# jyf588/SimGAN

Hardware: AMD Instinct MI355X
Metric: env-steps/sec of GAIL-dyn PPO update (higher is better)
Workload: dtype f32; 1 GPU; northstar: GAIL-dyn update, T=128 N=512/GPU obs=47 act=12 D-in=86 policy=mlp h64 D h100 ppo_epoch=10 num_mini_batch=1...; optimizer_steps_per_update=2720, parallelism=single GPU

## Files before the change

### include/simgan_hip.h

```cpp
#ifndef SIMGAN_HIP_H
#define SIMGAN_HIP_H

#include <stdint.h>

#define SG_API __attribute__((visibility("default")))

#ifdef __cplusplus
extern "C" {
#endif

typedef struct sg_ctx sg_ctx;
typedef struct sg_policy sg_policy;
typedef struct sg_rollout sg_rollout;
typedef struct sg_ppo sg_ppo;
typedef struct sg_disc sg_disc;

SG_API const char *sg_last_error(void);
SG_API const char *sg_version(void);
SG_API int sg_ctx_create(int device, sg_ctx **out);
SG_API int sg_ctx_destroy(sg_ctx *ctx);
SG_API int sg_ctx_synchronize(sg_ctx *ctx);
SG_API int sg_ctx_device_info(sg_ctx *ctx, char *name, int name_len, int *num_cu, int64_t *hbm_bytes);

SG_API int sg_comm_unique_id(uint8_t id[128]);
SG_API int sg_comm_loopback_id(uint8_t id[128]);
SG_API int sg_ctx_comm_init(sg_ctx *ctx, const uint8_t id[128], int rank, int world);
SG_API int sg_ctx_comm_kind(sg_ctx *ctx, int *kind);
SG_API int sg_ctx_comm_set_peer(sg_ctx *ctx, int enable);
SG_API int sg_ctx_comm_info(sg_ctx *ctx, int *rank, int *world);
SG_API int sg_ctx_set_disc_dp(sg_ctx *ctx, int sharded);

enum { SG_POLICY_MLP = 0, SG_POLICY_SPLIT = 1, SG_POLICY_GRU = 2 };
SG_API int sg_policy_create(sg_ctx *ctx, int kind, int obs_dim, int act_dim, int hidden, int num_feet,
                     sg_policy **out);
SG_API int sg_policy_create2(sg_ctx *ctx, int kind, int obs_dim, int act_dim, int hidden, int num_feet, int critic_hidden,
                             sg_policy **out);
SG_API int sg_policy_destroy(sg_policy *p);
SG_API int sg_policy_num_params(const sg_policy *p, int64_t *n);
SG_API int sg_policy_set_params(sg_policy *p, const float *flat, int64_t n);
SG_API int sg_policy_get_params(sg_policy *p, float *flat, int64_t n);
SG_API int sg_policy_act(sg_policy *p, const float *obs, int n, const float *noise, uint64_t seed,
                  int deterministic, float *value, float *action, float *logp);
SG_API int sg_policy_get_value(sg_policy *p, const float *obs, int n, float *value);
SG_API int sg_policy_evaluate(sg_policy *p, const float *obs, const float *action, int n, float *value,
                       float *logp, float *entropy);
SG_API int sg_policy_act_rnn(sg_policy *p, const float *obs, const float *hxs, const float *masks, int n, const float *noise,
                      uint64_t seed, int deterministic, float *value, float *action, float *logp, float *hxs_out);
SG_API int sg_policy_get_value_rnn(sg_policy *p, const float *obs, const float *hxs, const float *masks, int n, float *value);
SG_API int sg_policy_evaluate_rnn(sg_policy *p, const float *obs, const float *hxs, const float *masks, const float *action,
                           int T, int n, float *value, float *logp, float *entropy, float *hxs_out);
#define SG_ENSEMBLE_MAX 8
SG_API int sg_policy_act_ensemble(sg_policy *const *policies, int n_policies, const int32_t *idx, const float *obs,
                           int n, const float *noise, uint64_t seed, int deterministic, float *value,
                           float *action, float *logp);

enum {
    SG_F_OBS = 0,
    SG_F_OBS_FEAT = 1,
    SG_F_ACTIONS = 2,
    SG_F_REWARDS = 3,
    SG_F_VALUE_PREDS = 4,
    SG_F_RETURNS = 5,
    SG_F_LOGP = 6,
    SG_F_MASKS = 7,
    SG_F_BAD_MASKS = 8,
    SG_F_ADVANTAGES = 9,
    SG_F_COUNT = 10
};
SG_API int sg_rollout_create(sg_ctx *ctx, int T, int N, int obs_dim, int act_dim, int feat_dim,
                      sg_rollout **out);
SG_API int sg_rollout_destroy(sg_rollout *r);
SG_API int sg_rollout_upload(sg_rollout *r, int field, const float *host, int64_t count);
SG_API int sg_rollout_download(sg_rollout *r, int field, float *host, int64_t count);
SG_API int sg_rollout_upload_step(sg_rollout *r, int field, int t, const float *host, int64_t count);
SG_API int sg_rollout_download_step(sg_rollout *r, int field, int t, float *host, int64_t count);
SG_API int sg_rollout_after_update(sg_rollout *r);
SG_API int sg_rollout_compute_returns(sg_rollout *r, const float *next_value, int use_gae, float gamma,
                               float gae_lambda, int use_proper_time_limits);
SG_API int sg_rollout_compute_returns_policy(sg_rollout *r, sg_policy *p, int use_gae, float gamma,
                                      float gae_lambda, int use_proper_time_limits);
SG_API int sg_rollout_fill_synthetic(sg_rollout *r, sg_policy *p, uint64_t seed, float p_done);

typedef struct {
    float clip_param;
    int ppo_epoch;
    int num_mini_batch;
    float value_loss_coef;
    float entropy_coef;
    float lr;
    float eps;
    float max_grad_norm;
    int use_clipped_value_loss;
} sg_ppo_config;
SG_API int sg_ppo_create(sg_ctx *ctx, sg_policy *p, const sg_ppo_config *cfg, sg_ppo **out);
SG_API int sg_ppo_destroy(sg_ppo *a);
SG_API int sg_ppo_set_lr(sg_ppo *a, float lr);
SG_API int sg_ppo_update(sg_ppo *a, sg_rollout *r, const int64_t *perms, int64_t n_perms, uint64_t seed, float out3[3]);
SG_API int sg_results_publish(sg_ctx *ctx, sg_disc *d, sg_ppo *a, int slot);
SG_API int sg_results_fetch(sg_ctx *ctx, int slot, double out13[13]);
SG_API int sg_ppo_last_perms(sg_ppo *a, int64_t *perms, int64_t count);
SG_API int sg_ppo_get_adam(sg_ppo *a, float *m, float *v, int64_t n, int64_t *step);
SG_API int sg_ppo_set_adam(sg_ppo *a, const float *m, const float *v, int64_t n, int64_t step);
SG_API int sg_ppo_set_hidden_states(sg_ppo *a, const float *hxs0, int64_t count);
SG_API int sg_ppo_set_symmetry(sg_ppo *a, float coef, const float *m_obs, const float *m_act);
SG_API int sg_ppo_set_mirrored_obs(sg_ppo *a, const float *host, int64_t count);
SG_API int sg_ppo_last_symmetry_loss(sg_ppo *a, float *out);

typedef struct {
    float value_loss_coef;
    float entropy_coef;
    float lr;
    float eps;
    float alpha;
    float max_grad_norm;
} sg_a2c_config;
SG_API int sg_a2c_create(sg_ctx *ctx, sg_policy *p, const sg_a2c_config *cfg, sg_ppo **out);
SG_API int sg_a2c_get_rmsprop(sg_ppo *a, float *square_avg, int64_t n, int64_t *step);
SG_API int sg_a2c_set_rmsprop(sg_ppo *a, const float *square_avg, int64_t n, int64_t step);

typedef struct {
    float value_loss_coef;
    float entropy_coef;
    float lr;
    float momentum;
    float stat_decay;
    float kl_clip;
    float damping;
    int Tf;
} sg_acktr_config;
SG_API int sg_acktr_create(sg_ctx *ctx, sg_policy *p, const sg_acktr_config *cfg, sg_ppo **out);
SG_API int sg_acktr_set_value_noise(sg_ppo *a, const float *eps, int64_t n);
SG_API int sg_acktr_get_state(sg_ppo *a, float *m_aa, int64_t n_aa, float *m_gg, int64_t n_gg, float *momentum_buf, int64_t n,
                              int64_t *steps);

SG_API int sg_disc_create(sg_ctx *ctx, int input_dim, int hidden_dim, sg_disc **out);
SG_API int sg_disc_destroy(sg_disc *d);
SG_API int sg_disc_num_params(const sg_disc *d, int64_t *n);
SG_API int sg_disc_set_params(sg_disc *d, const float *flat, int64_t n);
SG_API int sg_disc_get_params(sg_disc *d, float *flat, int64_t n);
SG_API int sg_disc_get_adam(sg_disc *d, float *m, float *v, int64_t n, int64_t *step);
SG_API int sg_disc_set_adam(sg_disc *d, const float *m, const float *v, int64_t n, int64_t step);
SG_API int sg_disc_set_expert(sg_disc *d, const float *expert, int64_t n_rows);
SG_API int sg_disc_update_gail_dyn(sg_disc *d, sg_rollout *r, int batch_size, const int64_t *expert_perm, int64_t n_expert_perm,
                            const int64_t *policy_perm, int64_t n_policy_perm, const float *alpha, int64_t n_alpha,
                            uint64_t seed, float out3[3], int *n_steps);
SG_API int sg_disc_update_rows(sg_disc *d, const float *policy_rows, int64_t n_rows, int n_cols, int batch_size,
                        const int64_t *expert_perm, int64_t n_expert_perm, const int64_t *policy_perm, int64_t n_policy_perm,
                        const float *alpha, int64_t n_alpha, uint64_t seed, float out3[3], int *n_steps);
SG_API int sg_disc_predict_reward(sg_disc *d, const float *x, int n, float gamma, const float *masks,
                           float offset, float *reward, float *returns);
SG_API int sg_disc_predict_reward_steps(sg_disc *d, sg_rollout *r, float gamma, float offset, float *reward, float *returns);
SG_API int sg_disc_predict_prob(sg_disc *d, const float *x, int n, float *prob);
SG_API int sg_disc_grad_pen(sg_disc *d, const float *expert_rows, const float *policy_rows, const float *alpha, int n,
                     uint64_t seed, float *pen);
SG_API int sg_disc_last_draws(sg_disc *d, int64_t *expert_perm, int64_t *policy_perm, float *alpha, int64_t counts3[3]);
SG_API int sg_disc_reset_returns(sg_disc *d);
SG_API int sg_disc_get_returns(sg_disc *d, float *returns, int n, int *is_none);
SG_API int sg_disc_set_returns(sg_disc *d, const float *returns, int n);
SG_API int sg_disc_relabel_rewards(sg_disc *d, sg_rollout *r, float gamma, float offset,
                            double rms_state[3]);
SG_API int sg_disc_relabel_rewards_auto(sg_disc *d, sg_rollout *r, float gamma, double gail_tar_length, int no_alive_bonus);
SG_API int sg_disc_set_rms(sg_disc *d, const double rms_state[3]);
SG_API int sg_disc_get_scalars(sg_disc *d, double out5[5]);
SG_API int sg_rollout_count_dones(sg_rollout *r, double *dones);

SG_API int sg_host_alloc(int64_t bytes, void **out);
SG_API int sg_host_free(void *p);

SG_API int sg_ctx_profile(sg_ctx *ctx, int enable);
SG_API int sg_ctx_profile_read(sg_ctx *ctx, int which, double *total_ms, int64_t *launches);
SG_API int sg_ctx_profile_reset(sg_ctx *ctx);
SG_API int sg_ctx_mark(sg_ctx *ctx, int *id);
SG_API int sg_ctx_mark_elapsed(sg_ctx *ctx, int from, int to, double *ms);

#ifdef __cplusplus
}
#endif
#endif
```

### simgan_amd/_lib.py

```python
import ctypes as C
import os

import numpy as np

_HERE = os.path.dirname(os.path.abspath(__file__))
LIB_PATH = os.path.join(_HERE, "libsimgan_hip.so")

c_float_p = C.POINTER(C.c_float)
c_i64_p = C.POINTER(C.c_int64)
c_double_p = C.POINTER(C.c_double)
c_u8_p = C.POINTER(C.c_uint8)
c_int_p = C.POINTER(C.c_int)
H = C.c_void_p

F_OBS, F_OBS_FEAT, F_ACTIONS, F_REWARDS, F_VALUE_PREDS, F_RETURNS, F_LOGP, F_MASKS, F_BAD_MASKS, \
    F_ADVANTAGES = range(10)
POLICY_MLP, POLICY_SPLIT, POLICY_GRU = 0, 1, 2
PROF_DISC_CHAIN, PROF_DISC_WGRAD, PROF_PPO_FWD, PROF_PPO_BWD, PROF_PPO_REDUCE, PROF_RELABEL, PROF_PPO_ADAM = range(7)


class PPOConfig(C.Structure):
    _fields_ = [("clip_param", C.c_float), ("ppo_epoch", C.c_int), ("num_mini_batch", C.c_int),
                ("value_loss_coef", C.c_float), ("entropy_coef", C.c_float), ("lr", C.c_float),
                ("eps", C.c_float), ("max_grad_norm", C.c_float),
                ("use_clipped_value_loss", C.c_int)]


class A2CConfig(C.Structure):
    _fields_ = [("value_loss_coef", C.c_float), ("entropy_coef", C.c_float), ("lr", C.c_float), ("eps", C.c_float),
                ("alpha", C.c_float), ("max_grad_norm", C.c_float)]


class ACKTRConfig(C.Structure):
    _fields_ = [("value_loss_coef", C.c_float), ("entropy_coef", C.c_float), ("lr", C.c_float), ("momentum", C.c_float),
                ("stat_decay", C.c_float), ("kl_clip", C.c_float), ("damping", C.c_float), ("Tf", C.c_int)]


PROTOTYPES = {
    "sg_last_error": (C.c_char_p, []),
    "sg_version": (C.c_char_p, []),
    "sg_ctx_create": (C.c_int, [C.c_int, C.POINTER(H)]),
    "sg_ctx_destroy": (C.c_int, [H]),
    "sg_ctx_synchronize": (C.c_int, [H]),
    "sg_ctx_device_info": (C.c_int, [H, C.c_char_p, C.c_int, c_int_p, c_i64_p]),
    "sg_comm_unique_id": (C.c_int, [c_u8_p]),
    "sg_comm_loopback_id": (C.c_int, [c_u8_p]),
    "sg_ctx_comm_init": (C.c_int, [H, c_u8_p, C.c_int, C.c_int]),
    "sg_ctx_comm_kind": (C.c_int, [H, c_int_p]),
    "sg_ctx_comm_set_peer": (C.c_int, [H, C.c_int]),
    "sg_ctx_comm_info": (C.c_int, [H, c_int_p, c_int_p]),
    "sg_ctx_set_disc_dp": (C.c_int, [H, C.c_int]),
    "sg_policy_create": (C.c_int, [H, C.c_int, C.c_int, C.c_int, C.c_int, C.c_int, C.POINTER(H)]),
    "sg_policy_create2": (C.c_int, [H, C.c_int, C.c_int, C.c_int, C.c_int, C.c_int, C.c_int, C.POINTER(H)]),
    "sg_policy_destroy": (C.c_int, [H]),
    "sg_policy_num_params": (C.c_int, [H, c_i64_p]),
    "sg_policy_set_params": (C.c_int, [H, c_float_p, C.c_int64]),
    "sg_policy_get_params": (C.c_int, [H, c_float_p, C.c_int64]),
    "sg_policy_act": (C.c_int, [H, c_float_p, C.c_int, c_float_p, C.c_uint64, C.c_int, c_float_p, c_float_p, c_float_p]),
    "sg_policy_get_value": (C.c_int, [H, c_float_p, C.c_int, c_float_p]),
    "sg_policy_evaluate": (C.c_int, [H, c_float_p, c_float_p, C.c_int, c_float_p, c_float_p, c_float_p]),
    "sg_policy_act_rnn": (C.c_int, [H, c_float_p, c_float_p, c_float_p, C.c_int, c_float_p, C.c_uint64, C.c_int, c_float_p, c_float_p,
                                    c_float_p, c_float_p]),
    "sg_policy_get_value_rnn": (C.c_int, [H, c_float_p, c_float_p, c_float_p, C.c_int, c_float_p]),
    "sg_policy_evaluate_rnn": (C.c_int, [H, c_float_p, c_float_p, c_float_p, c_float_p, C.c_int, C.c_int, c_float_p, c_float_p,
                                         c_float_p, c_float_p]),
    "sg_policy_act_ensemble": (C.c_int, [C.POINTER(H), C.c_int, C.POINTER(C.c_int32), c_float_p, C.c_int, c_float_p, C.c_uint64,
                                         C.c_int, c_float_p, c_float_p, c_float_p]),
    "sg_rollout_create": (C.c_int, [H, C.c_int, C.c_int, C.c_int, C.c_int, C.c_int, C.POINTER(H)]),
    "sg_rollout_destroy": (C.c_int, [H]),
    "sg_rollout_upload": (C.c_int, [H, C.c_int, c_float_p, C.c_int64]),
    "sg_rollout_download": (C.c_int, [H, C.c_int, c_float_p, C.c_int64]),
    "sg_rollout_upload_step": (C.c_int, [H, C.c_int, C.c_int, c_float_p, C.c_int64]),
    "sg_rollout_download_step": (C.c_int, [H, C.c_int, C.c_int, c_float_p, C.c_int64]),
    "sg_rollout_after_update": (C.c_int, [H]),
    "sg_rollout_compute_returns": (C.c_int, [H, c_float_p, C.c_int, C.c_float, C.c_float, C.c_int]),
    "sg_rollout_compute_returns_policy": (C.c_int, [H, H, C.c_int, C.c_float, C.c_float, C.c_int]),
    "sg_rollout_fill_synthetic": (C.c_int, [H, H, C.c_uint64, C.c_float]),
    "sg_rollout_count_dones": (C.c_int, [H, c_double_p]),
    "sg_ppo_create": (C.c_int, [H, H, C.POINTER(PPOConfig), C.POINTER(H)]),
    "sg_ppo_destroy": (C.c_int, [H]),
    "sg_ppo_set_lr": (C.c_int, [H, C.c_float]),
    "sg_ppo_update": (C.c_int, [H, H, c_i64_p, C.c_int64, C.c_uint64, c_float_p]),
    "sg_ppo_last_perms": (C.c_int, [H, c_i64_p, C.c_int64]),
    "sg_ppo_set_hidden_states": (C.c_int, [H, c_float_p, C.c_int64]),
    "sg_ppo_get_adam": (C.c_int, [H, c_float_p, c_float_p, C.c_int64, c_i64_p]),
    "sg_ppo_set_adam": (C.c_int, [H, c_float_p, c_float_p, C.c_int64, C.c_int64]),
    "sg_ppo_set_symmetry": (C.c_int, [H, C.c_float, c_float_p, c_float_p]),
    "sg_ppo_set_mirrored_obs": (C.c_int, [H, c_float_p, C.c_int64]),
    "sg_ppo_last_symmetry_loss": (C.c_int, [H, c_float_p]),
    "sg_a2c_create": (C.c_int, [H, H, C.POINTER(A2CConfig), C.POINTER(H)]),
    "sg_a2c_get_rmsprop": (C.c_int, [H, c_float_p, C.c_int64, c_i64_p]),
    "sg_a2c_set_rmsprop": (C.c_int, [H, c_float_p, C.c_int64, C.c_int64]),
    "sg_acktr_create": (C.c_int, [H, H, C.POINTER(ACKTRConfig), C.POINTER(H)]),
    "sg_acktr_set_value_noise": (C.c_int, [H, c_float_p, C.c_int64]),
    "sg_acktr_get_state": (C.c_int, [H, c_float_p, C.c_int64, c_float_p, C.c_int64, c_float_p, C.c_int64, c_i64_p]),
    "sg_disc_create": (C.c_int, [H, C.c_int, C.c_int, C.POINTER(H)]),
    "sg_disc_destroy": (C.c_int, [H]),
    "sg_disc_num_params": (C.c_int, [H, c_i64_p]),
    "sg_disc_set_params": (C.c_int, [H, c_float_p, C.c_int64]),
    "sg_disc_get_params": (C.c_int, [H, c_float_p, C.c_int64]),
    "sg_disc_get_adam": (C.c_int, [H, c_float_p, c_float_p, C.c_int64, c_i64_p]),
    "sg_disc_set_adam": (C.c_int, [H, c_float_p, c_float_p, C.c_int64, C.c_int64]),
    "sg_disc_set_expert": (C.c_int, [H, c_float_p, C.c_int64]),
    "sg_disc_update_gail_dyn": (C.c_int, [H, H, C.c_int, c_i64_p, C.c_int64, c_i64_p, C.c_int64, c_float_p, C.c_int64, C.c_uint64,
                                          c_float_p, c_int_p]),
    "sg_disc_update_rows": (C.c_int, [H, c_float_p, C.c_int64, C.c_int, C.c_int, c_i64_p, C.c_int64, c_i64_p, C.c_int64, c_float_p,
                                      C.c_int64, C.c_uint64, c_float_p, c_int_p]),
    "sg_disc_predict_reward": (C.c_int, [H, c_float_p, C.c_int, C.c_float, c_float_p, C.c_float, c_float_p, c_float_p]),
    "sg_disc_predict_prob": (C.c_int, [H, c_float_p, C.c_int, c_float_p]),
    "sg_disc_predict_reward_steps": (C.c_int, [H, H, C.c_float, C.c_float, c_float_p, c_float_p]),
    "sg_disc_grad_pen": (C.c_int, [H, c_float_p, c_float_p, c_float_p, C.c_int, C.c_uint64, c_float_p]),
    "sg_disc_last_draws": (C.c_int, [H, c_i64_p, c_i64_p, c_float_p, c_i64_p]),
    "sg_disc_reset_returns": (C.c_int, [H]),
    "sg_disc_get_returns": (C.c_int, [H, c_float_p, C.c_int, c_int_p]),
    "sg_disc_set_returns": (C.c_int, [H, c_float_p, C.c_int]),
    "sg_disc_relabel_rewards": (C.c_int, [H, H, C.c_float, C.c_float, c_double_p]),
    "sg_disc_relabel_rewards_auto": (C.c_int, [H, H, C.c_float, C.c_double, C.c_int]),
    "sg_disc_set_rms": (C.c_int, [H, c_double_p]),
    "sg_disc_get_scalars": (C.c_int, [H, c_double_p]),
    "sg_results_publish": (C.c_int, [H, H, H, C.c_int]),
    "sg_results_fetch": (C.c_int, [H, C.c_int, c_double_p]),
    "sg_ctx_profile": (C.c_int, [H, C.c_int]),
    "sg_ctx_profile_read": (C.c_int, [H, C.c_int, c_double_p, c_i64_p]),
    "sg_ctx_profile_reset": (C.c_int, [H]),
    "sg_host_alloc": (C.c_int, [C.c_int64, C.POINTER(C.c_void_p)]),
    "sg_host_free": (C.c_int, [C.c_void_p]),
    "sg_ctx_mark": (C.c_int, [H, c_int_p]),
    "sg_ctx_mark_elapsed": (C.c_int, [H, C.c_int, C.c_int, c_double_p]),
}

TEST_LIB_PATH = os.path.join(_HERE, "libsimgan_hip_test.so")
c_ll_p = C.POINTER(C.c_longlong)
TEST_PROTOTYPES = {
    "sg_test_last_error": (C.c_char_p, []),
    "sg_test_gemm": (C.c_int, [H, C.c_int, C.c_int, C.c_int, C.c_int, c_float_p, c_float_p, c_float_p]),
    "sg_test_gemm_bench": (C.c_int, [H, C.c_int, C.c_int, C.c_int, C.c_int, C.c_int, C.c_int, C.c_int, c_ll_p]),
    "sg_test_mfma_probe": (C.c_int, [H, C.c_int, c_float_p, c_float_p, c_float_p]),
    "sg_test_flag_probe": (C.c_int, [H, C.c_int, C.c_int, C.c_int, C.c_int, c_ll_p, c_float_p]),
    "sg_test_fetch_probe": (C.c_int, [H, C.c_int, C.c_int, C.c_int, c_ll_p]),
    "sg_test_pmc_calibrate": (C.c_int, [H, C.c_int64]),
    "sg_test_pstep_probe": (C.c_int, [H, C.c_int, C.c_int, C.c_int, C.c_int, C.c_int, c_ll_p, c_int_p]),
    "sg_test_graph_state": (C.c_int, [H, H, c_int_p]),
    "sg_test_disc_phase_times": (C.c_int, [H, C.c_int, c_ll_p, C.c_int]),
    "sg_test_disc_step4_times": (C.c_int, [H, C.c_int, c_ll_p, C.c_int]),
    "sg_test_disc_gathers": (C.c_int, [H, c_ll_p]),
    "sg_test_ppo_phase_times": (C.c_int, [H, C.c_int, c_ll_p, C.c_int]),
    "sg_test_rng": (C.c_int, [H, C.c_int, C.c_int64, C.c_uint64, C.c_void_p]),
    "sg_test_kfac_eig": (C.c_int, [H, C.c_int, c_float_p, c_float_p, c_float_p, C.POINTER(C.c_int)]),
    "sg_test_acktr_noise": (C.c_int, [H, C.c_int64, C.c_uint64, C.c_int64, c_float_p]),
    "sg_test_raise_kfac_error": (C.c_int, [H]),
    "sg_test_tear_probe": (C.c_int, [H, C.c_int, C.c_int, C.c_int, c_ll_p]),
    "sg_test_raise_handoff_error": (C.c_int, [H, H]),
}
_TEST_LIB = None

_LIB = None


class SimganHipError(RuntimeError):
    pass


def load():
    global _LIB
    if _LIB is not None:
        return _LIB
    if not os.path.exists(LIB_PATH):
        raise SimganHipError(
            f"{LIB_PATH} not found: the HIP extension is not built. There is no CPU fallback; "
            "run `make -C simgan_amd/csrc` (hipcc, gfx950).")
    lib = C.CDLL(LIB_PATH)
    for name, (res, args) in PROTOTYPES.items():
        fn = getattr(lib, name)
        fn.restype = res
        fn.argtypes = args
    _LIB = lib
    return lib


def check(rc):
    if rc != 0:
        raise SimganHipError(load().sg_last_error().decode(errors="replace"))


def load_test():
    global _TEST_LIB
    if _TEST_LIB is not None:
        return _TEST_LIB
    load()
    if not os.path.exists(TEST_LIB_PATH):
        raise SimganHipError(f"{TEST_LIB_PATH} not found: run `make -C simgan_amd/csrc`")
    lib = C.CDLL(TEST_LIB_PATH)
    for name, (res, args) in TEST_PROTOTYPES.items():
        fn = getattr(lib, name)
        fn.restype = res
        fn.argtypes = args
    _TEST_LIB = lib
    return lib


def check_test(rc):
    if rc != 0:
        raise SimganHipError(load_test().sg_test_last_error().decode(errors="replace"))


def fptr(a):
    assert isinstance(a, np.ndarray) and a.dtype == np.float32 and a.flags["C_CONTIGUOUS"], (type(a), getattr(a, "dtype", None))
    return a.ctypes.data_as(c_float_p)


def i64ptr(a):
    assert isinstance(a, np.ndarray) and a.dtype == np.int64 and a.flags["C_CONTIGUOUS"]
    return a.ctypes.data_as(c_i64_p)


def as_f32(x):
    if hasattr(x, "detach"):
        x = x.detach().cpu().numpy()
    return np.ascontiguousarray(x, dtype=np.float32)


def as_i64(x):
    if hasattr(x, "detach"):
        x = x.detach().cpu().numpy()
    return np.ascontiguousarray(x, dtype=np.int64)


class _PinnedBlock(object):

    def __init__(self, nbytes):
        self.lib = load()
        p = C.c_void_p()
        check(self.lib.sg_host_alloc(int(nbytes), C.byref(p)))
        self.ptr = p.value

    def __del__(self):
        try:
            if self.ptr:
                self.lib.sg_host_free(C.c_void_p(self.ptr))
                self.ptr = None
        except Exception:
            pass


_PINNED_WARNED = False


def pinned_array(shape, fill=0.0):
    n = int(np.prod(shape)) * 4
    if n == 0:
        return np.full(shape, fill, np.float32)
    try:
        blk = _PinnedBlock(n)
    except SimganHipError as exc:
        global _PINNED_WARNED
        if not _PINNED_WARNED:
            _PINNED_WARNED = True
            import warnings
            warnings.warn(f"simgan_amd: page-locked host allocation of {n} bytes failed ({exc}); the rollout's host tensors fall back to "
                          "pageable memory (uploads are staged and slower)", RuntimeWarning, stacklevel=3)
        return np.full(shape, fill, np.float32)
    buf = (C.c_char * n).from_address(blk.ptr)
    buf._owner = blk
    a = np.frombuffer(buf, dtype=np.float32).reshape(shape)
    a[...] = fill
    return a


_CTX = {}


class Context:

    def __init__(self, device=0):
        self.lib = load()
        h = H()
        check(self.lib.sg_ctx_create(int(device), C.byref(h)))
        self.h = h
        self.device = int(device)
        self.rank, self.world = 0, 1
        self.disc_sharded = False

    @staticmethod
    def default():
        dev = int(os.environ.get("LOCAL_RANK", "0"))
        if dev not in _CTX:
            try:
                _CTX[dev] = Context(dev)
            except SimganHipError as exc:
                if dev == 0 or "out of range (1 visible)" not in str(exc):
                    raise
                _CTX[dev] = Context(0)
        return _CTX[dev]

    def make_default(self):
        _CTX[int(os.environ.get("LOCAL_RANK", "0"))] = self
        return self

    def synchronize(self):
# ... 74 lines not shown
```

### simgan_amd/csrc/sg_common.h

```cpp
#pragma once
#include <hip/hip_runtime.h>
#include <stdint.h>

#include <string>
#include <atomic>
#include <vector>
#include <mutex>
inline std::recursive_mutex& sg_capture_mutex() { static std::recursive_mutex m; return m; }
struct SgDeviceWideGuard {
    std::lock_guard<std::recursive_mutex> l{sg_capture_mutex()};
    ~SgDeviceWideGuard() { (void)hipGetLastError(); }
};
#define SG_DEVICE_WIDE() SgDeviceWideGuard _sg_device_wide_guard
static inline hipError_t sg_dev_malloc(void** p, size_t n) { std::lock_guard<std::recursive_mutex> l(sg_capture_mutex()); return hipMalloc(p, n); }
static inline hipError_t sg_dev_free(void* p) { std::lock_guard<std::recursive_mutex> l(sg_capture_mutex()); return hipFree(p); }
static inline hipError_t sg_host_malloc(void** p, size_t n) { std::lock_guard<std::recursive_mutex> l(sg_capture_mutex()); return hipHostMalloc(p, n, hipHostMallocDefault); }
static inline hipError_t sg_host_release(void* p) { std::lock_guard<std::recursive_mutex> l(sg_capture_mutex()); return hipHostFree(p); }

#include "../../include/simgan_hip.h"
#include "sg_gemm.hpp"

void sg_set_error(const char* fmt, ...);

#define SG_CHECK(expr)                                                                      \
// ... 45 lines not shown
    int total;
    int nc, na;
};

struct SgDiscDesc {
    int F, Hd, Fp, ldF, Hp, ldH;
    int w1, b1, w2, b2, w3, b3;
    int total;
};

SgPolicyDesc sg_make_policy_desc(int kind, int O, int A, int H, int num_feet, int Hc = 0);
int64_t sg_policy_flat_count(const SgPolicyDesc& d);
void sg_policy_pad(const SgPolicyDesc& d, const float* flat, float* padded);
void sg_policy_unpad(const SgPolicyDesc& d, const float* padded, float* flat);
struct sg_ctx;
bool sg_policy_needs_gw(const sg_ctx* ctx, const SgPolicyDesc& d);
SgDiscDesc sg_make_disc_desc(int F, int Hd);
int64_t sg_disc_flat_count(const SgDiscDesc& d);
void sg_disc_pad(const SgDiscDesc& d, const float* flat, float* padded);
void sg_disc_unpad(const SgDiscDesc& d, const float* padded, float* flat);

enum { SG_PROF_DISC_CHAIN = 0, SG_PROF_DISC_WGRAD, SG_PROF_PPO_FWD, SG_PROF_PPO_BWD,
       SG_PROF_PPO_REDUCE, SG_PROF_RELABEL, SG_PROF_PPO_ADAM, SG_PROF_DISC_STEP, SG_PROF_COMM_F32, SG_PROF_COUNT };

struct SgProfSlot {
    double total_ms = 0.0;
    int64_t launches = 0;
    std::vector<std::pair<hipEvent_t, hipEvent_t>> pending;
};

struct SgComm;

struct sg_ctx {
    int device = 0;
    hipStream_t stream = nullptr;
    int num_cu = 0;
    int lds_bytes = 0;
    bool profile = false;
    SgProfSlot prof[SG_PROF_COUNT];
    std::vector<hipEvent_t> event_pool;
    std::vector<hipEvent_t> marks;
    SgComm* comm = nullptr;
    int rank = 0, world = 1;
    bool disc_sharded = false;
    bool use_comm = false;
    std::atomic<int> n_learners{0};
    float* d_scratch = nullptr;
    size_t scratch_bytes = 0;
    void* h_pinned = nullptr;
    size_t pinned_bytes = 0;
    double* mailbox = nullptr;
    double* results = nullptr;
    hipEvent_t res_ev[8] = {nullptr};
    struct sg_disc* res_d[8] = {nullptr};
    struct sg_ppo* res_a[8] = {nullptr};
};
#define SG_RESULT_SLOTS 8

bool sg_ctx_exclusive(const sg_ctx* ctx);
void sg_ctx_learner_born(sg_ctx* ctx);
void sg_ctx_learner_gone(sg_ctx* ctx);
int sg_ctx_scratch(sg_ctx* ctx, size_t bytes, float** out);
int sg_ctx_pinned(sg_ctx* ctx, size_t bytes, void** out);
int sg_ctx_fetch_f64(sg_ctx* ctx, const double* dev, double* host, int n);
int sg_ctx_put_f64(sg_ctx* ctx, double* dev, const double* host, int n);
struct SgEv { hipEvent_t a = nullptr, b = nullptr; };
SgEv sg_prof_events(sg_ctx* ctx, int which);
#ifdef __HIPCC__
#include <hip/hip_ext.h>
#define SG_LAUNCH(ctx, which, kernel, grid, block, lds, ...)                                                  \
    do {                                                                                                      \
        if ((ctx)->profile) {                                                                                 \
            SgEv _ev = sg_prof_events(ctx, which);                                                            \
            hipExtLaunchKernelGGL(kernel, grid, block, lds, (ctx)->stream, _ev.a, _ev.b, 0, __VA_ARGS__);     \
        } else {                                                                                              \
            hipLaunchKernelGGL(kernel, grid, block, lds, (ctx)->stream, __VA_ARGS__);                         \
        }                                                                                                     \
    } while (0)
#endif

struct SgGruDesc {
    int O, H, Op, ldO, Hp, ldH;
    int off;
    int wih, whh, bih, bhh;
    int total;
};
SgGruDesc sg_make_gru_desc(int O, int H, int off);
int64_t sg_gru_flat_count(const SgGruDesc& g);
void sg_gru_pad(const SgGruDesc& g, const float* flat, float* padded);
void sg_gru_unpad(const SgGruDesc& g, const float* padded, float* flat);

struct sg_policy {
    sg_ctx* ctx;
    SgPolicyDesc desc;
    bool recurrent = false;
    SgGruDesc gru;
    float* d_params = nullptr;
    float* d_io = nullptr;
    size_t io_bytes = 0;
};

size_t sg_policy_padded_count(const sg_policy* p);
bool sg_gru_fits(const sg_ctx* ctx, const SgGruDesc& g);

#define SG_STEP4_FLAG_WORD0 64
#define SG_STEP4_MAX_FLAGS 1024
#ifndef SG_STEP4_FLAG_STRIDE
#define SG_STEP4_FLAG_STRIDE 32
#endif
#define SG_STEP4_ERR_WORD (SG_STEP4_FLAG_WORD0 + SG_STEP4_MAX_FLAGS * SG_STEP4_FLAG_STRIDE)
#define SG_STEP4_STATE_BYTES (4 * (SG_STEP4_ERR_WORD + 16))
#define SG_PAIR_ERR_WORD 0
unsigned* sg_comm_peer_err_word(struct sg_ctx* ctx);
bool sg_comm_peer_on(const struct sg_ctx* ctx);
uint32_t sg_comm_peer_generation(const struct sg_ctx* ctx);
unsigned* sg_disc_err_word(struct sg_disc* d);
uint64_t sg_next_feat_version();
struct sg_rollout {
    sg_ctx* ctx;
    int T, N, O, A, F;
    float* d_field[SG_F_COUNT] = {nullptr};
    int64_t field_count[SG_F_COUNT] = {0};
    int field_slots[SG_F_COUNT] = {0};
    int field_width[SG_F_COUNT] = {0};
    int64_t* d_perm = nullptr;
    uint64_t feat_version = sg_next_feat_version();
};

#define SG_H0_SLOTS 8
struct sg_ppo {
    int64_t opt_t = 0;
    uint64_t scratch_key = 0;
    hipGraphExec_t steps_graph = nullptr;
    bool graph_refused = false;
    uint64_t steps_graph_key[18] = {0};
    sg_ctx* ctx;
    sg_policy* policy;
    sg_ppo_config cfg;
    float *d_m = nullptr, *d_v = nullptr, *d_grad = nullptr;
    float* d_slabs = nullptr;
    size_t slabs_cap = 0;
    float* d_stacks = nullptr;
    size_t stacks_cap = 0;
    float* d_state = nullptr;
    int64_t* d_perms = nullptr;
    int64_t perms_cap = 0;
    int64_t last_perm_count = 0;
    double* d_loss_acc = nullptr;
    float* d_part = nullptr;
    long long* d_dbg = nullptr;
    unsigned* d_pair = nullptr;
    bool self_wait_failed = false;
    bool pair_primed = false;
    float sym_coef = 0.f;
    float* d_mobs_mat = nullptr;
    float* d_mact = nullptr;
    float* d_mrows = nullptr;
    int64_t mrows_cap = 0;
    int64_t mrows_host = 0;
    float* d_h0 = nullptr;
    int64_t h0_cap = 0, h0_count = 0;
    float* h_h0 = nullptr;
    hipEvent_t h0_ev[8] = {nullptr};
    uint64_t h0_calls = 0;
    float* d_gru = nullptr;
    size_t gru_cap = 0;
    int64_t gru_layout[8] = {0};
    bool a2c = false;
    float alpha = 0.f;
    struct SgKfac* kfac = nullptr;
};

struct sg_disc {
    sg_ctx* ctx;
    SgDiscDesc desc;
    bool self_wait_failed = false;
    float *d_params = nullptr, *d_m = nullptr, *d_v = nullptr;
    float* d_slabs = nullptr;
    int n_slabs = 0;
    float* d_state = nullptr;
    float* d_expert = nullptr;
    int64_t n_expert = 0;
    int64_t *d_eperm = nullptr, *d_pperm = nullptr;
    int64_t eperm_cap = 0, pperm_cap = 0;
    float* d_alpha = nullptr;
    int64_t alpha_cap = 0;
    int64_t last_draws[3] = {0, 0, 0};
    float* d_feat_all = nullptr;
    int64_t feat_all_cap = 0;
    const float* gather_src = nullptr;
    int64_t gather_rows = 0;
    uint64_t gather_version = 0;
    int64_t n_gathers = 0;
    int64_t opt_t = 0;
    hipGraphExec_t epoch_graph = nullptr;
    bool graph_refused = false;
    uint64_t epoch_graph_key[12] = {0};
    float* d_wT = nullptr;
    float *d_erows = nullptr, *d_prows = nullptr;
    int64_t erows_cap = 0, prows_cap = 0;
    float* d_rows = nullptr;
    int64_t rows_cap = 0;
    double* d_loss_acc = nullptr;
    double* d_scal = nullptr;
    int last_n_d = 0;
    float* d_returns = nullptr;
    int returns_n = 0;
    bool returns_none = true;
    uint64_t rng_calls = 0;
    long long* d_dbg_step4 = nullptr;
    long long* d_dbg = nullptr;
};

struct SgOptState {
    float lr;
    float reserved[3];
    float step_size2[2];
    float bc2_sqrt2[2];
    int t0;
    int pad[3];
};

#ifdef __HIPCC__
__attribute__((unused)) static __global__ void k_zero_f64(double* p, int n) {
    if ((int)threadIdx.x < n) p[threadIdx.x] = 0.0;
}
__attribute__((unused)) static __global__ void k_opt_commit(SgOptState* st, int n_steps) { st->t0 += n_steps; }
__device__ __forceinline__ void sg_opt_prepare(SgOptState* st, int t) {
    const double bc1 = 1.0 - pow(0.9, (double)t), bc2 = 1.0 - pow(0.999, (double)t);
    st->step_size2[t & 1] = (float)((double)st->lr / bc1);
    st->bc2_sqrt2[t & 1] = (float)sqrt(bc2);
}
#endif

#include <stdio.h>

template <typename F>
static inline int sg_try_capture(sg_ctx* ctx, hipGraphExec_t* exec, F&& enqueue) {
    std::lock_guard<std::recursive_mutex> lock(sg_capture_mutex());
    hipGraph_t graph = nullptr;
    auto refuse = [&](const char* what, hipError_t e, int rc) {
        static bool told = false;
        if (!told) {
            fprintf(stderr, "[simgan_hip] graph capture not used (%s: %s%s); falling back to direct launches\n", what,
                    e != hipSuccess ? hipGetErrorString(e) : "no HIP error", rc != 0 ? ", enqueue reported an error" : "");
            told = true;
        }
        (void)hipGetLastError();
        return 1;
    };
    hipError_t e = hipStreamBeginCapture(ctx->stream, hipStreamCaptureModeRelaxed);
    if (e != hipSuccess) return refuse("hipStreamBeginCapture", e, 0);
    const int rc = enqueue();
    e = hipStreamEndCapture(ctx->stream, &graph);
    if (rc != 0 || e != hipSuccess || !graph) {
        if (graph) (void)hipGraphDestroy(graph);
        return refuse("hipStreamEndCapture", e, rc);
    }
    e = hipGraphInstantiate(exec, graph, nullptr, nullptr, 0);
    (void)hipGraphDestroy(graph);
    if (e != hipSuccess) { *exec = nullptr; return refuse("hipGraphInstantiate", e, 0); }
    return 0;
}

int sg_comm_graph_ok(const sg_ctx* ctx);
void sg_comm_destroy(sg_ctx* ctx);
int sg_rollout_count_dones_dev(sg_rollout* r, double* d_out);
int sg_comm_allreduce_f32(sg_ctx* ctx, float* dev, int64_t n);
int sg_comm_allreduce_f64(sg_ctx* ctx, double* dev, int64_t n);
int sg_comm_allgather_f32(sg_ctx* ctx, const float* dev_in, float* dev_out, int64_t n_per_rank);
```

### simgan_amd/csrc/sg_gemm.hpp

```cpp
#pragma once
#include <hip/hip_runtime.h>

typedef float f32x4 __attribute__((ext_vector_type(4)));

#define SG_PAD16(x) (((x) + 15) & ~15)
#define SG_LD(x) (SG_PAD16(x) + 4)

__device__ __forceinline__ f32x4 sg_mfma(float a, float b, f32x4 c) {
    return __builtin_amdgcn_mfma_f32_16x16x4f32(a, b, c, 0, 0, 0);
}

__device__ __forceinline__ float2 sg_lds_read_b64(const float* p) {
    typedef float v2f __attribute__((ext_vector_type(2)));
    typedef const volatile v2f __attribute__((address_space(3))) * lds_v2f_ptr;
    const v2f v = *(lds_v2f_ptr)(p);
    return float2{v.x, v.y};
}

__device__ __forceinline__ float sg_tanh(float x) {
    const float x2 = x * x;
    const float poly = x * (1.f + x2 * (-0.33333334f + x2 * (0.13333334f + x2 * (-0.053968254f + x2 * 0.021869488f))));
    const float t = __expf(2.f * x);
    const float big = 1.f - 2.f * __builtin_amdgcn_rcpf(t + 1.f);
    return fabsf(x) < 0.1f ? poly : big;
// ... 129 lines not shown
    for (int c = 0; c < KC; ++c)
#pragma unroll
        for (int s = 0; s < 4; ++s)
#pragma unroll
            for (int i = 0; i < MT; ++i) {
                const float av = s == 0 ? a[c][i].x : s == 1 ? a[c][i].y : s == 2 ? a[c][i].z : a[c][i].w;
#pragma unroll
                for (int j = 0; j < NT; ++j) {
                    if (DUAL && (s & 1)) alt = sg_mfma(av, b[c][s][j], alt);
                    else acc[i][j] = sg_mfma(av, b[c][s][j], acc[i][j]);
                }
            }
    ap += 16 * KC;
    bp += 16 * KC * ldb;
}

template <int MT, int NT>
__device__ __forceinline__ void sg_mma_nn(const float* A, int lda, const float* B, int ldb, int K,
                                          f32x4 (&acc)[MT][NT]) {
    const int lane = threadIdx.x & 63, li = lane & 15, lq = lane >> 4;
    const float* ap = A + li * lda + 4 * lq;
    const float* bp = B + (4 * lq) * ldb + li;
    f32x4 alt = f32x4{0.f, 0.f, 0.f, 0.f};
#define SG_BODY(N) sg_mma_nn_blk<MT, NT, N>(ap, lda, bp, ldb, acc, alt)
    SG_KC_DISPATCH(K >> 4, SG_BODY);
#undef SG_BODY
    if (MT * NT == 1) acc[0][0] += alt;
}

template <int MT, int NT, int KC>
__device__ __forceinline__ void sg_mma_tn_blk(const float*& ap, int lda, const float*& bp, int ldb,
                                              f32x4 (&acc)[MT][NT], f32x4& alt) {
    constexpr bool DUAL = (MT * NT == 1);
    float a[KC][4][MT], b[KC][4][NT];
#pragma unroll
    for (int c = 0; c < KC; ++c)
#pragma unroll
        for (int s = 0; s < 4; ++s) {
#pragma unroll
            for (int i = 0; i < MT; ++i) a[c][s][i] = ap[(16 * c + s) * lda + i * 16];
#pragma unroll
            for (int j = 0; j < NT; ++j) b[c][s][j] = bp[(16 * c + s) * ldb + j * 16];
        }
#pragma unroll
    for (int c = 0; c < KC; ++c)
#pragma unroll
        for (int s = 0; s < 4; ++s)
#pragma unroll
            for (int i = 0; i < MT; ++i)
#pragma unroll
                for (int j = 0; j < NT; ++j) {
                    if (DUAL && (s & 1)) alt = sg_mfma(a[c][s][i], b[c][s][j], alt);
                    else acc[i][j] = sg_mfma(a[c][s][i], b[c][s][j], acc[i][j]);
                }
    ap += 16 * KC * lda;
    bp += 16 * KC * ldb;
}

template <int MT, int NT>
__device__ __forceinline__ void sg_mma_tn(const float* A, int lda, const float* B, int ldb, int K,
                                          f32x4 (&acc)[MT][NT]) {
    const int lane = threadIdx.x & 63, li = lane & 15, lq = lane >> 4;
    const float* ap = A + (4 * lq) * lda + li;
    const float* bp = B + (4 * lq) * ldb + li;
    f32x4 alt = f32x4{0.f, 0.f, 0.f, 0.f};
#define SG_BODY(N) sg_mma_tn_blk<MT, NT, N>(ap, lda, bp, ldb, acc, alt)
    SG_KC_DISPATCH(K >> 4, SG_BODY);
#undef SG_BODY
    if (MT * NT == 1) acc[0][0] += alt;
}

template <typename F>
__device__ __forceinline__ void sg_tile_foreach(const f32x4& acc, int row0, int col0, F&& f) {
    const int lane = threadIdx.x & 63, li = lane & 15, lq = lane >> 4;
#pragma unroll
    for (int r = 0; r < 4; ++r) f(row0 + 4 * lq + r, col0 + li, acc[r]);
}

template <int MT>
__device__ __forceinline__ float sg_tile_colsum(const float (&v)[MT][4]) {
    float s = 0.f;
#pragma unroll
    for (int i = 0; i < MT; ++i) s += (v[i][0] + v[i][1]) + (v[i][2] + v[i][3]);
    s += __shfl_xor(s, 16);
    s += __shfl_xor(s, 32);
    return s;
}


template <int MT, bool GW = false, typename EP>
__device__ __forceinline__ void sg_layer_nt_t(const float* in, int ldi, const float* W, int ldw,
                                              int K, int Np, EP&& ep) {
    const int wave = threadIdx.x >> 6, nw = blockDim.x >> 6;
    for (int tn = wave; tn * 16 < Np; tn += nw) {
        f32x4 acc[MT][1];
        sg_acc_zero(acc);
        if (GW) sg_mma_nt_g<MT, 1>(in, ldi, W + (size_t)tn * 16 * ldw, ldw, K, acc);
        else sg_mma_nt<MT, 1>(in, ldi, W + tn * 16 * ldw, ldw, K, acc);
        ep(tn, acc);
    }
}

template <int MT, typename EP>
__device__ __forceinline__ void sg_layer_nn_t(const float* dY, int ldy, const float* W, int ldw,
                                              int K, int Np, EP&& ep) {
    const int wave = threadIdx.x >> 6, nw = blockDim.x >> 6;
    for (int tn = wave; tn * 16 < Np; tn += nw) {
        f32x4 acc[MT][1];
        sg_acc_zero(acc);
        sg_mma_nn<MT, 1>(dY, ldy, W + tn * 16, ldw, K, acc);
        ep(tn, acc);
    }
}

template <int MT, bool GW = false, typename EP>
__device__ __forceinline__ void sg_layer_nt(const float* in, int ldi, const float* W, int ldw,
                                            int K, int Np, EP&& ep) {
    sg_layer_nt_t<MT, GW>(in, ldi, W, ldw, K, Np, [&](int tn, f32x4 (&acc)[MT][1]) {
#pragma unroll
        for (int i = 0; i < MT; ++i) sg_tile_foreach(acc[i][0], i * 16, tn * 16, ep);
    });
}

template <int MT, typename EP>
__device__ __forceinline__ void sg_layer_nn(const float* dY, int ldy, const float* W, int ldw,
                                            int K, int Np, EP&& ep) {
    sg_layer_nn_t<MT>(dY, ldy, W, ldw, K, Np, [&](int tn, f32x4 (&acc)[MT][1]) {
#pragma unroll
        for (int i = 0; i < MT; ++i) sg_tile_foreach(acc[i][0], i * 16, tn * 16, ep);
    });
}

template <int MT, bool GW = false, typename EP>
__device__ __forceinline__ void sg_layer_nt_u(const float* in, int ldi, const float* W, int ldw, int K, int Np, EP&& ep) {
    const int wave = threadIdx.x >> 6, nw = blockDim.x >> 6, ntl = Np >> 4;
    for (int u = wave; u < MT * ntl; u += nw) {
        const int i = u / ntl, tn = u - i * ntl;
        f32x4 acc[1][1];
        sg_acc_zero(acc);
        if (GW) sg_mma_nt_g<1, 1>(in + i * 16 * ldi, ldi, W + (size_t)tn * 16 * ldw, ldw, K, acc);
        else sg_mma_nt<1, 1>(in + i * 16 * ldi, ldi, W + tn * 16 * ldw, ldw, K, acc);
        sg_tile_foreach(acc[0][0], i * 16, tn * 16, ep);
    }
}
template <int MT, typename EP>
__device__ __forceinline__ void sg_layer_nn_u(const float* dY, int ldy, const float* W, int ldw, int K, int Np, EP&& ep) {
    const int wave = threadIdx.x >> 6, nw = blockDim.x >> 6, ntl = Np >> 4;
    for (int u = wave; u < MT * ntl; u += nw) {
        const int i = u / ntl, tn = u - i * ntl;
        f32x4 acc[1][1];
        sg_acc_zero(acc);
        sg_mma_nn<1, 1>(dY + i * 16 * ldy, ldy, W + tn * 16, ldw, K, acc);
        sg_tile_foreach(acc[0][0], i * 16, tn * 16, ep);
    }
}

template <int KC, int NTN, bool TWO, bool NT = true>
__device__ __forceinline__ void sg_tn_panel(const float* ap, const float* ap2, int lda, const float* bp,
                                            const float* bp2, int ldb, float* G, int ldg, bool accumulate) {
    float a[TWO ? 2 : 1][KC][4], b[TWO ? 2 : 1][KC][4][NTN];
#pragma unroll
    for (int c = 0; c < KC; ++c)
#pragma unroll
        for (int s = 0; s < 4; ++s) {
            a[0][c][s] = ap[(16 * c + s) * lda];
#pragma unroll
            for (int j = 0; j < NTN; ++j) b[0][c][s][j] = bp[(16 * c + s) * ldb + 16 * j];
            if (TWO) {
                a[TWO ? 1 : 0][c][s] = ap2[(16 * c + s) * lda];
#pragma unroll
                for (int j = 0; j < NTN; ++j) b[TWO ? 1 : 0][c][s][j] = bp2[(16 * c + s) * ldb + 16 * j];
            }
        }
    f32x4 acc[NTN];
#pragma unroll
    for (int j = 0; j < NTN; ++j) acc[j] = f32x4{0.f, 0.f, 0.f, 0.f};
#pragma unroll
    for (int src = 0; src < (TWO ? 2 : 1); ++src)
#pragma unroll
        for (int c = 0; c < KC; ++c)
#pragma unroll
            for (int s = 0; s < 4; ++s)
#pragma unroll
                for (int j = 0; j < NTN; ++j) acc[j] = sg_mfma(b[src][c][s][j], a[src][c][s], acc[j]);
    const int lane = threadIdx.x & 63, li = lane & 15, lq = lane >> 4;
    typedef float sg_f4 __attribute__((ext_vector_type(4)));
#pragma unroll
    for (int j = 0; j < NTN; ++j) {
        sg_f4* p = reinterpret_cast<sg_f4*>(G + li * ldg + 16 * j + 4 * lq);
        sg_f4 v = sg_f4{acc[j][0], acc[j][1], acc[j][2], acc[j][3]};
        if (accumulate) *p = *p + v;
        else if (NT) __builtin_nontemporal_store(v, p);
        else {
            float* q = G + li * ldg + 16 * j + 4 * lq;
            q[0] = acc[j][0]; q[1] = acc[j][1]; q[2] = acc[j][2]; q[3] = acc[j][3];
        }
    }
}

template <int KC, int NW_HINT = 0, bool NT = true>
__device__ __forceinline__ void sg_grad_tn2(const float* dY, int ldy, const float* X, int ldx,
                                            const float* dY2, const float* X2, int Mp, int Np,
                                            float* G, int ldg, bool accumulate) {
    const int wave = threadIdx.x >> 6, nw = blockDim.x >> 6;
    const int lane = threadIdx.x & 63, li = lane & 15, lq = lane >> 4;
    const int tm_n = Mp >> 4, tn_n = Np >> 4;
    int bw = 8;
    if (NW_HINT > 4) while (bw > 1 && tm_n * ((tn_n + bw - 1) / bw) < NW_HINT) bw >>= 1;
    const int blocks_n = (tn_n + bw - 1) / bw;
    for (int t = wave; t < tm_n * blocks_n; t += nw) {
        const int tm = t / blocks_n, tb = t % blocks_n;
        const int ntn = tn_n - bw * tb < bw ? tn_n - bw * tb : bw;
        const float* ap = dY + (4 * lq) * ldy + tm * 16 + li;
        const float* bp = X + (4 * lq) * ldx + tb * bw * 16 + li;
        const float* ap2 = dY2 ? dY2 + (4 * lq) * ldy + tm * 16 + li : ap;
        const float* bp2 = X2 ? X2 + (4 * lq) * ldx + tb * bw * 16 + li : bp;
        float* g = G + (size_t)(tm * 16) * ldg + tb * bw * 16;
#define SG_PANEL(N)                                                                              \
    do {                                                                                         \
        if (dY2) sg_tn_panel<KC, N, true, NT>(ap, ap2, ldy, bp, bp2, ldx, g, ldg, accumulate);   \
        else sg_tn_panel<KC, N, false, NT>(ap, ap2, ldy, bp, bp2, ldx, g, ldg, accumulate);      \
    } while (0)
        switch (ntn) {
            case 8: SG_PANEL(8); break; case 7: SG_PANEL(7); break; case 6: SG_PANEL(6); break;
            case 5: SG_PANEL(5); break; case 4: SG_PANEL(4); break; case 3: SG_PANEL(3); break;
            case 2: SG_PANEL(2); break; case 1: SG_PANEL(1); break; default: break;
        }
#undef SG_PANEL
    }
}

template <int KC, int NW_HINT = 0, bool NT = true>
__device__ __forceinline__ void sg_grad_tn(const float* dY, int ldy, const float* X, int ldx, int Mp,
                                           int Np, float* G, int ldg, bool accumulate) {
    sg_grad_tn2<KC, NW_HINT, NT>(dY, ldy, X, ldx, nullptr, nullptr, Mp, Np, G, ldg, accumulate);
}

template <int CTRL>
__device__ __forceinline__ float sg_dpp_add(float v) {
    return v + __int_as_float(__builtin_amdgcn_update_dpp(0, __float_as_int(v), CTRL, 0xF, 0xF, true));
}
__device__ __forceinline__ float sg_rowsum16(float v) {
    v = sg_dpp_add<0xB1>(v);
    v = sg_dpp_add<0x4E>(v);
    v = sg_dpp_add<0x141>(v);
    v = sg_dpp_add<0x140>(v);
    return v;
}

__device__ __forceinline__ void sg_colsum(const float* M, int ldm, int R, int Np, float* g,
                                          bool accumulate) {
    const int sub = threadIdx.x & 15;
    for (int c = threadIdx.x >> 4; c < Np; c += blockDim.x >> 4) {
        float s = 0.f;
        for (int r = sub; r < R; r += 16) s += M[r * ldm + c];
        s = sg_rowsum16(s);
        if (sub == 0) g[c] = accumulate ? g[c] + s : s;
    }
}

typedef unsigned int sg_u32x4 __attribute__((ext_vector_type(4)));
__device__ __forceinline__ float4 sg_buffer_load4(__amdgpu_buffer_rsrc_t rsrc, int byte_offset) {
    const sg_u32x4 r = __builtin_amdgcn_raw_buffer_load_b128(rsrc, byte_offset, 0, 0);
    return float4{__uint_as_float(r.x), __uint_as_float(r.y), __uint_as_float(r.z), __uint_as_float(r.w)};
}
__device__ __forceinline__ void sg_stage(float* lds, const float* __restrict__ g, int n4) {
    const __amdgpu_buffer_rsrc_t rsrc = __builtin_amdgcn_make_buffer_rsrc(const_cast<float*>(g), 0, n4 * 16, 0x00020000);
    float4* dst = reinterpret_cast<float4*>(lds);
    const int nt = blockDim.x;
#pragma unroll 2
    for (int base = threadIdx.x; base < n4; base += 8 * nt) {
        float4 v[8];
#pragma unroll
        for (int u = 0; u < 8; ++u) v[u] = sg_buffer_load4(rsrc, (base + u * nt) * 16);
#pragma unroll
        for (int u = 0; u < 8; ++u) {
            const int i = base + u * nt;
            if (i < n4) dst[i] = v[u];
        }
    }
}

template <int U>
__device__ __forceinline__ void sg_stage_issue(float4 (&v)[U], const float* __restrict__ g, int n4) {
    const __amdgpu_buffer_rsrc_t rsrc = __builtin_amdgcn_make_buffer_rsrc(const_cast<float*>(g), 0, n4 * 16, 0x00020000);
#pragma unroll
    for (int u = 0; u < U; ++u) v[u] = sg_buffer_load4(rsrc, (int)(threadIdx.x + u * blockDim.x) * 16);
}
template <int U>
__device__ __forceinline__ void sg_stage_commit(float* lds, const float4 (&v)[U], const float* __restrict__ g, int n4) {
    float4* dst = reinterpret_cast<float4*>(lds);
#pragma unroll
    for (int u = 0; u < U; ++u) {
        const int i = threadIdx.x + u * blockDim.x;
        if (i < n4) dst[i] = v[u];
    }
    const int done = U * blockDim.x;
    if (n4 > done) sg_stage(lds + 4 * done, g + 4 * done, n4 - done);
}

__device__ __forceinline__ float sg_wave_sum(float v) {
#pragma unroll
    for (int o = 32; o > 0; o >>= 1) v += __shfl_xor(v, o);
    return v;
}
__device__ __forceinline__ double sg_wave_sum(double v) {
// ... 5 lines not shown
```

### simgan_amd/csrc/sg_layout.cpp

```cpp
#include <string.h>

#include <functional>

#include "sg_common.h"

static SgTrunk make_trunk(int& cursor, int H, int ldO, int P, int EX) {
    SgTrunk t;
    const int Hp = SG_PAD16(H), ldH = SG_LD(H);
    t.H = H; t.Hp = Hp; t.ldH = ldH;
    t.off = cursor;
    int o = 0;
    t.w1 = o; o += Hp * ldO;
    t.b1 = o; o += Hp;
    t.w2 = o; o += Hp * ldH;
    t.b2 = o; o += Hp;
    t.P = P;
    t.Pp = SG_PAD16(P);
    t.ldP = SG_LD(P);
    t.wh = o; o += t.Pp * ldH;
    t.bh = o; o += t.Pp;
    t.EX = EX;
    t.ex = o; o += EX ? SG_PAD16(EX) : 0;
    t.size = o;
    cursor += o;
    return t;
}

SgPolicyDesc sg_make_policy_desc(int kind, int O, int A, int H, int num_feet, int Hc) {
    SgPolicyDesc d;
    memset(&d, 0, sizeof d);
    if (Hc <= 0) Hc = H;
    d.kind = kind; d.O = O; d.A = A; d.H = H; d.num_feet = num_feet; d.Hc = Hc;
    d.Op = SG_PAD16(O); d.ldO = SG_LD(O);
    const int Hmax = H > Hc ? H : Hc;
    d.Hp = SG_PAD16(Hmax); d.ldH = SG_LD(Hmax);
    int cur = 0;
    if (kind == SG_POLICY_MLP) {
        d.n_trunks = 2;
        d.trunk[0] = make_trunk(cur, H, d.ldO, A, A);
        d.trunk[1] = make_trunk(cur, Hc, d.ldO, 1, 0);
    } else {
        d.n_trunks = 3;
        d.nc = 4 * num_feet; d.na = 3 * num_feet;
        d.trunk[0] = make_trunk(cur, H, d.ldO, 2 * d.nc, 0);
        d.trunk[1] = make_trunk(cur, H, d.ldO, 2 * d.na, 0);
        d.trunk[2] = make_trunk(cur, Hc, d.ldO, 1, 0);
    }
    d.total = cur;
    return d;
}

typedef std::function<void(int64_t, int64_t, int, int, int)> SegFn;

static int64_t policy_segments(const SgPolicyDesc& d, const SegFn& f) {
    int64_t fo = 0;
    const int O = d.O, H = d.H, A = d.A;
    auto mat = [&](int64_t po, int rows, int cols, int ld) { f(fo, po, rows, cols, ld); fo += (int64_t)rows * cols; };
    for (int t = 0; t < d.n_trunks; ++t) {
        const SgTrunk& tr = d.trunk[t];
        mat(tr.off + tr.w1, tr.H, O, d.ldO);
        mat(tr.off + tr.b1, 1, tr.H, tr.H);
        mat(tr.off + tr.w2, tr.H, tr.H, tr.ldH);
        mat(tr.off + tr.b2, 1, tr.H, tr.H);
    }
    const SgTrunk& cr = d.trunk[d.n_trunks - 1];
    mat(cr.off + cr.wh, 1, cr.H, cr.ldH);
    mat(cr.off + cr.bh, 1, 1, 1);
    if (d.kind == SG_POLICY_MLP) {
        const SgTrunk& ac = d.trunk[0];
        mat(ac.off + ac.wh, A, H, ac.ldH);
        mat(ac.off + ac.bh, 1, A, A);
        mat(ac.off + ac.ex, 1, A, A);
    } else {
        const SgTrunk& c = d.trunk[0];
        const SgTrunk& a = d.trunk[1];
        mat(c.off + c.wh, d.nc, H, c.ldH);
        mat(c.off + c.bh, 1, d.nc, d.nc);
        mat(a.off + a.wh, d.na, H, a.ldH);
        mat(a.off + a.bh, 1, d.na, d.na);
        mat(c.off + c.wh + d.nc * c.ldH, d.nc, H, c.ldH);
        mat(c.off + c.bh + d.nc, 1, d.nc, d.nc);
        mat(a.off + a.wh + d.na * a.ldH, d.na, H, a.ldH);
        mat(a.off + a.bh + d.na, 1, d.na, d.na);
    }
    return fo;
}

int64_t sg_policy_flat_count(const SgPolicyDesc& d) {
    return policy_segments(d, [](int64_t, int64_t, int, int, int) {});
}

void sg_policy_pad(const SgPolicyDesc& d, const float* flat, float* padded) {
    policy_segments(d, [&](int64_t fo, int64_t po, int rows, int cols, int ld) {
        for (int r = 0; r < rows; ++r) memcpy(padded + po + (int64_t)r * ld, flat + fo + (int64_t)r * cols, sizeof(float) * cols);
    });
}

void sg_policy_unpad(const SgPolicyDesc& d, const float* padded, float* flat) {
    policy_segments(d, [&](int64_t fo, int64_t po, int rows, int cols, int ld) {
        for (int r = 0; r < rows; ++r) memcpy(flat + fo + (int64_t)r * cols, padded + po + (int64_t)r * ld, sizeof(float) * cols);
    });
}

SgGruDesc sg_make_gru_desc(int O, int H, int off) {
    SgGruDesc g;
    memset(&g, 0, sizeof g);
    g.O = O; g.H = H; g.Op = SG_PAD16(O); g.ldO = SG_LD(O); g.Hp = SG_PAD16(H); g.ldH = SG_LD(H);
    g.off = off;
    int o = 0;
    g.wih = o; o += 3 * g.Hp * g.ldO;
    g.whh = o; o += 3 * g.Hp * g.ldH;
    g.bih = o; o += 3 * g.Hp;
    g.bhh = o; o += 3 * g.Hp;
    g.total = o;
    return g;
}

static int64_t gru_segments(const SgGruDesc& g, const SegFn& f) {
    int64_t fo = 0;
    auto mat = [&](int64_t po, int rows, int cols, int ld) { f(fo, po, rows, cols, ld); fo += (int64_t)rows * cols; };
    for (int k = 0; k < 3; ++k) mat(g.wih + (int64_t)k * g.Hp * g.ldO, g.H, g.O, g.ldO);
    for (int k = 0; k < 3; ++k) mat(g.whh + (int64_t)k * g.Hp * g.ldH, g.H, g.H, g.ldH);
    for (int k = 0; k < 3; ++k) mat(g.bih + k * g.Hp, 1, g.H, g.H);
    for (int k = 0; k < 3; ++k) mat(g.bhh + k * g.Hp, 1, g.H, g.H);
    return fo;
}

int64_t sg_gru_flat_count(const SgGruDesc& g) {
    return gru_segments(g, [](int64_t, int64_t, int, int, int) {});
}

void sg_gru_pad(const SgGruDesc& g, const float* flat, float* padded) {
    gru_segments(g, [&](int64_t fo, int64_t po, int rows, int cols, int ld) {
        for (int r = 0; r < rows; ++r) memcpy(padded + po + (int64_t)r * ld, flat + fo + (int64_t)r * cols, sizeof(float) * cols);
    });
}

void sg_gru_unpad(const SgGruDesc& g, const float* padded, float* flat) {
    gru_segments(g, [&](int64_t fo, int64_t po, int rows, int cols, int ld) {
        for (int r = 0; r < rows; ++r) memcpy(flat + fo + (int64_t)r * cols, padded + po + (int64_t)r * ld, sizeof(float) * cols);
    });
}

SgDiscDesc sg_make_disc_desc(int F, int Hd) {
    SgDiscDesc d;
    d.F = F; d.Hd = Hd;
    d.Fp = SG_PAD16(F); d.ldF = SG_LD(F);
    d.Hp = SG_PAD16(Hd); d.ldH = SG_LD(Hd);
    int o = 0;
    d.w1 = o; o += d.Hp * d.ldF;
    d.b1 = o; o += d.Hp;
    d.w2 = o; o += d.Hp * d.ldH;
    d.b2 = o; o += d.Hp;
    d.w3 = o; o += d.Hp;
    d.b3 = o; o += 16;
    d.total = o;
    return d;
}

static int64_t disc_segments(const SgDiscDesc& d, const SegFn& f) {
    int64_t fo = 0;
    auto mat = [&](int64_t po, int rows, int cols, int ld) { f(fo, po, rows, cols, ld); fo += (int64_t)rows * cols; };
    mat(d.w1, d.Hd, d.F, d.ldF);
    mat(d.b1, 1, d.Hd, d.Hd);
    mat(d.w2, d.Hd, d.Hd, d.ldH);
    mat(d.b2, 1, d.Hd, d.Hd);
    mat(d.w3, 1, d.Hd, d.Hd);
    mat(d.b3, 1, 1, 1);
    return fo;
}

int64_t sg_disc_flat_count(const SgDiscDesc& d) {
    return disc_segments(d, [](int64_t, int64_t, int, int, int) {});
}

void sg_disc_pad(const SgDiscDesc& d, const float* flat, float* padded) {
    disc_segments(d, [&](int64_t fo, int64_t po, int rows, int cols, int ld) {
        for (int r = 0; r < rows; ++r) memcpy(padded + po + (int64_t)r * ld, flat + fo + (int64_t)r * cols, sizeof(float) * cols);
    });
}

void sg_disc_unpad(const SgDiscDesc& d, const float* padded, float* flat) {
    disc_segments(d, [&](int64_t fo, int64_t po, int rows, int cols, int ld) {
        for (int r = 0; r < rows; ++r) memcpy(flat + fo + (int64_t)r * cols, padded + po + (int64_t)r * ld, sizeof(float) * cols);
    });
}
```

### simgan_amd/csrc/sg_ppo.hip

```cpp
#include <math.h>
#include <stdlib.h>
#include <string.h>

#include <algorithm>
#include <vector>

#include "sg_common.h"
#include "sg_rng.hpp"
#include "sg_ppo_kernels.hpp"
#include "sg_kfac.hpp"
#include "sg_gru_kernels.hpp"

__global__ void k_fill_perm(int64_t* perm, int64_t n, int half_bits, uint64_t key) {
    const int64_t i = (int64_t)blockIdx.x * blockDim.x + threadIdx.x;
    if (i < n) perm[i] = sg_perm_at(i, n, half_bits, key);
}

int sg_fill_perm(sg_ctx* ctx, int64_t* d_perm, int64_t n, uint64_t seed, uint64_t stream_id) {
    const uint64_t key = sg_key(seed, 0x5045524Dull, stream_id);
    hipLaunchKernelGGL(k_fill_perm, dim3((unsigned)((n + 255) / 256)), dim3(256), 0, ctx->stream, d_perm, n,
                       sg_perm_half_bits((uint64_t)n), key);
    SG_CHECK(hipGetLastError());
    return 0;
}

static int max_trunk_floats(const SgPolicyDesc& d) {
    int m = 0;
    for (int t = 0; t < d.n_trunks; ++t) m = d.trunk[t].size > m ? d.trunk[t].size : m;
    return m;
}
static int max_bwd_floats(const SgPolicyDesc& d) {
    int m = 0;
    for (int t = 0; t < d.n_trunks; ++t) { const int s = d.trunk[t].size - d.trunk[t].w2; m = s > m ? s : m; }
    return m;
}
static int stack_ldP(const SgPolicyDesc& d) {
    int m = 0;
    for (int t = 0; t < d.n_trunks; ++t) m = d.trunk[t].ldP > m ? d.trunk[t].ldP : m;
    return m;
}
static size_t ppo_fwd_lds(const SgPolicyDesc& d, int MT, bool gw) {
    const int R = 16 * MT;
    return sizeof(float) * ((gw ? 0 : (size_t)max_trunk_floats(d)) + R * d.ldO + 2 * R * d.ldH);
}
static bool ppo_fused(const SgPolicyDesc& d, int MT) {
    const char* e = getenv("SG_PPO_FUSED");
    return d.kind == SG_POLICY_MLP && MT <= 2 && !(e && !strcmp(e, "0"));
}
static size_t ppo_bwd_lds(const SgPolicyDesc& d, int MT, bool gw) {
    const int R = 16 * MT;
    return sizeof(float) * ((gw ? 0 : (size_t)(ppo_fused(d, MT) ? max_trunk_floats(d) : max_bwd_floats(d))) + R * d.ldO + 2 * R * d.ldH + 2 * R * stack_ldP(d) +
                            ((R * d.A + 3) & ~3) + 7 * R);
}
static size_t ppo_bwd_sym_lds(const SgPolicyDesc& d, int MT, bool gw) {
    const int R = 16 * MT;
    return sizeof(float) * ((gw ? 0 : (size_t)max_bwd_floats(d)) + R * d.ldO + 2 * R * d.ldH + 3 * R * stack_ldP(d) +
                            ((R * d.A + 3) & ~3) + 7 * R + ((d.A * d.A + 3) & ~3));
}

static size_t a2c_bwd_lds(const SgPolicyDesc& d, int MT, bool gw) {
    const int R = 16 * MT;
    return sizeof(float) * ((gw ? 0 : (size_t)max_bwd_floats(d)) + R * d.ldO + 2 * R * d.ldH + 2 * R * stack_ldP(d) +
                            ((R * d.A + 3) & ~3) + 7 * R);
}
#define SG_A2C_CHUNK_ROWS 4096

#define SG_PPO_SHAPES(X) X(1, 3, 4) X(2, 3, 4)  X(2, 1, 7)  \
                         X(2, 4, 7)  X(2, 7, 4)

static int ppo_block_threads(int MT) {
    const char* we = getenv("SG_PPO_WAVES");
    return (MT >= 2 && !(we && atoi(we) == 4)) ? 512 : 256;
}

static void launch_ppo_fwd(sg_ctx* ctx, int MT, const SgPolicyDesc& d, dim3 grid, size_t lds, const PpoArgs& pa, bool gw) {
    const int ko = d.Op / 16, kh = d.Hc == d.H ? d.Hp / 16 : 0;
    const dim3 block(ppo_block_threads(MT));
    if (gw) {
        if (MT == 2) SG_LAUNCH(ctx, SG_PROF_PPO_FWD, (k_ppo_fwd<2, 0, 0, true>), grid, block, lds, pa);
        else SG_LAUNCH(ctx, SG_PROF_PPO_FWD, (k_ppo_fwd<1, 0, 0, true>), grid, block, lds, pa);
        return;
    }
#define SG_CASE(mt, o, h) \
    if (MT == mt && ko == o && kh == h) { SG_LAUNCH(ctx, SG_PROF_PPO_FWD, (k_ppo_fwd<mt, o, h>), grid, block, lds, pa); return; }
    SG_PPO_SHAPES(SG_CASE)
#undef SG_CASE
    if (MT == 4) SG_LAUNCH(ctx, SG_PROF_PPO_FWD, (k_ppo_fwd<4, 0, 0>), grid, block, lds, pa);
    else if (MT == 2) SG_LAUNCH(ctx, SG_PROF_PPO_FWD, (k_ppo_fwd<2, 0, 0>), grid, block, lds, pa);
    else SG_LAUNCH(ctx, SG_PROF_PPO_FWD, (k_ppo_fwd<1, 0, 0>), grid, block, lds, pa);
}
static void launch_ppo_fwd_critic(sg_ctx* ctx, int MT, const SgPolicyDesc& d, dim3 grid, size_t lds, const PpoArgs& pa) {
    const int ko = d.Op / 16, kh = d.Hc == d.H ? d.Hp / 16 : 0;
    const dim3 block(ppo_block_threads(MT));
    if (MT == 2 && ko == 4 && kh == 7) { SG_LAUNCH(ctx, SG_PROF_PPO_FWD, (k_ppo_fwd_critic<2, 4, 7>), grid, block, lds, pa); return; }
    if (MT == 2 && ko == 1 && kh == 7) { SG_LAUNCH(ctx, SG_PROF_PPO_FWD, (k_ppo_fwd_critic<2, 1, 7>), grid, block, lds, pa); return; }
    if (MT == 2) SG_LAUNCH(ctx, SG_PROF_PPO_FWD, (k_ppo_fwd_critic<2, 0, 0>), grid, block, lds, pa);
    else SG_LAUNCH(ctx, SG_PROF_PPO_FWD, (k_ppo_fwd_critic<1, 0, 0>), grid, block, lds, pa);
}
static void launch_ppo_pair(sg_ctx* ctx, int MT, const SgPolicyDesc& d, int G, size_t lds, const PpoArgs& pa) {
    const int ko = d.Op / 16, kh = d.Hc == d.H ? d.Hp / 16 : 0;
    const dim3 block(ppo_block_threads(MT)), grid(3 * G);
    if (MT == 2 && ko == 1 && kh == 7) { SG_LAUNCH(ctx, SG_PROF_PPO_BWD, (k_ppo_pair<2, 1, 7>), grid, block, lds, pa); return; }
    if (MT == 2 && ko == 4 && kh == 7) { SG_LAUNCH(ctx, SG_PROF_PPO_BWD, (k_ppo_pair<2, 4, 7>), grid, block, lds, pa); return; }
    if (MT == 2) SG_LAUNCH(ctx, SG_PROF_PPO_BWD, (k_ppo_pair<2, 0, 0>), grid, block, lds, pa);
    else SG_LAUNCH(ctx, SG_PROF_PPO_BWD, (k_ppo_pair<1, 0, 0>), grid, block, lds, pa);
}
static void launch_ppo_bwd(sg_ctx* ctx, int MT, const SgPolicyDesc& d, dim3 grid, size_t lds, const PpoArgs& pa, bool fused, bool gw) {
    const int ko = d.Op / 16, kh = d.Hc == d.H ? d.Hp / 16 : 0;
    const dim3 block(ppo_block_threads(MT));
    if (gw) {
        if (fused && MT == 2) SG_LAUNCH(ctx, SG_PROF_PPO_BWD, (k_ppo_bwd<2, 0, 0, true, true>), grid, block, lds, pa);
        else if (fused) SG_LAUNCH(ctx, SG_PROF_PPO_BWD, (k_ppo_bwd<1, 0, 0, true, true>), grid, block, lds, pa);
        else if (MT == 2) SG_LAUNCH(ctx, SG_PROF_PPO_BWD, (k_ppo_bwd<2, 0, 0, false, true>), grid, block, lds, pa);
        else SG_LAUNCH(ctx, SG_PROF_PPO_BWD, (k_ppo_bwd<1, 0, 0, false, true>), grid, block, lds, pa);
        return;
    }
    if (fused) {
        if (MT == 1 && ko == 3 && kh == 4) { SG_LAUNCH(ctx, SG_PROF_PPO_BWD, (k_ppo_bwd<1, 3, 4, true>), grid, block, lds, pa); return; }
        if (MT == 2 && ko == 3 && kh == 4) { SG_LAUNCH(ctx, SG_PROF_PPO_BWD, (k_ppo_bwd<2, 3, 4, true>), grid, block, lds, pa); return; }
        if (MT == 2 && ko == 7 && kh == 4) { SG_LAUNCH(ctx, SG_PROF_PPO_BWD, (k_ppo_bwd<2, 7, 4, true>), grid, block, lds, pa); return; }
        if (MT == 2) SG_LAUNCH(ctx, SG_PROF_PPO_BWD, (k_ppo_bwd<2, 0, 0, true>), grid, block, lds, pa);
        else SG_LAUNCH(ctx, SG_PROF_PPO_BWD, (k_ppo_bwd<1, 0, 0, true>), grid, block, lds, pa);
        return;
    }
#define SG_CASE(mt, o, h) \
    if (MT == mt && ko == o && kh == h) { SG_LAUNCH(ctx, SG_PROF_PPO_BWD, (k_ppo_bwd<mt, o, h>), grid, block, lds, pa); return; }
    SG_PPO_SHAPES(SG_CASE)
#undef SG_CASE
    if (MT == 4) SG_LAUNCH(ctx, SG_PROF_PPO_BWD, (k_ppo_bwd<4, 0, 0>), grid, block, lds, pa);
    else if (MT == 2) SG_LAUNCH(ctx, SG_PROF_PPO_BWD, (k_ppo_bwd<2, 0, 0>), grid, block, lds, pa);
    else SG_LAUNCH(ctx, SG_PROF_PPO_BWD, (k_ppo_bwd<1, 0, 0>), grid, block, lds, pa);
}

static void launch_ppo_fwd_sym(sg_ctx* ctx, int MT, const SgPolicyDesc& d, dim3 grid, size_t lds, const PpoArgs& pa, bool gw) {
    const int ko = d.Op / 16, kh = d.Hc == d.H ? d.Hp / 16 : 0;
    const dim3 block(ppo_block_threads(MT));
    if (gw) {
        if (MT == 2) SG_LAUNCH(ctx, SG_PROF_PPO_FWD, (k_ppo_fwd_sym<2, 0, 0, true>), grid, block, lds, pa);
        else SG_LAUNCH(ctx, SG_PROF_PPO_FWD, (k_ppo_fwd_sym<1, 0, 0, true>), grid, block, lds, pa);
    } else if (MT == 2 && ko == 7 && kh == 4) {
        SG_LAUNCH(ctx, SG_PROF_PPO_FWD, (k_ppo_fwd_sym<2, 7, 4>), grid, block, lds, pa);
    } else if (MT == 2) {
        SG_LAUNCH(ctx, SG_PROF_PPO_FWD, (k_ppo_fwd_sym<2, 0, 0>), grid, block, lds, pa);
    } else {
        SG_LAUNCH(ctx, SG_PROF_PPO_FWD, (k_ppo_fwd_sym<1, 0, 0>), grid, block, lds, pa);
    }
}
static void launch_ppo_bwd_sym(sg_ctx* ctx, int MT, const SgPolicyDesc& d, dim3 grid, size_t lds, const PpoArgs& pa, bool gw) {
    const int ko = d.Op / 16, kh = d.Hc == d.H ? d.Hp / 16 : 0;
    const dim3 block(ppo_block_threads(MT));
    if (gw) {
        if (MT == 2) SG_LAUNCH(ctx, SG_PROF_PPO_BWD, (k_ppo_bwd_sym<2, 0, 0, true>), grid, block, lds, pa);
        else SG_LAUNCH(ctx, SG_PROF_PPO_BWD, (k_ppo_bwd_sym<1, 0, 0, true>), grid, block, lds, pa);
    } else if (MT == 2 && ko == 7 && kh == 4) {
        SG_LAUNCH(ctx, SG_PROF_PPO_BWD, (k_ppo_bwd_sym<2, 7, 4>), grid, block, lds, pa);
    } else if (MT == 2) {
        SG_LAUNCH(ctx, SG_PROF_PPO_BWD, (k_ppo_bwd_sym<2, 0, 0>), grid, block, lds, pa);
    } else {
        SG_LAUNCH(ctx, SG_PROF_PPO_BWD, (k_ppo_bwd_sym<1, 0, 0>), grid, block, lds, pa);
    }
}

static void launch_a2c_bwd(sg_ctx* ctx, int MT, const SgPolicyDesc& d, dim3 grid, size_t lds, const PpoArgs& pa, bool gw) {
    const int ko = d.Op / 16, kh = d.Hc == d.H ? d.Hp / 16 : 0;
    const dim3 block(ppo_block_threads(MT));
    if (gw) {
        if (MT == 2) SG_LAUNCH(ctx, SG_PROF_PPO_BWD, (k_a2c_bwd<2, 0, 0, true>), grid, block, lds, pa);
        else SG_LAUNCH(ctx, SG_PROF_PPO_BWD, (k_a2c_bwd<1, 0, 0, true>), grid, block, lds, pa);
    } else if (MT == 2 && ko == 3 && kh == 4) {
        SG_LAUNCH(ctx, SG_PROF_PPO_BWD, (k_a2c_bwd<2, 3, 4>), grid, block, lds, pa);
    } else if (MT == 1 && ko == 3 && kh == 4) {
        SG_LAUNCH(ctx, SG_PROF_PPO_BWD, (k_a2c_bwd<1, 3, 4>), grid, block, lds, pa);
    } else if (MT == 2) {
        SG_LAUNCH(ctx, SG_PROF_PPO_BWD, (k_a2c_bwd<2, 0, 0>), grid, block, lds, pa);
    } else {
        SG_LAUNCH(ctx, SG_PROF_PPO_BWD, (k_a2c_bwd<1, 0, 0>), grid, block, lds, pa);
    }
}

static void kfac_free(sg_ppo* a) {
    SgKfac* k = a->kfac;
    if (!k) return;
    void* ptrs[] = {k->d_acc, k->d_m, k->d_Q, k->d_d, k->d_work, k->d_ks, k->d_vec, k->d_t0, k->d_t1, k->d_one, k->d_vpart,
                    k->d_jobs, k->d_tiles, k->d_eps, k->d_fish};
    for (void* q : ptrs) if (q) (void)sg_dev_free(q);
    delete k;
    a->kfac = nullptr;
}

static int kfac_setup(sg_ctx* ctx, SgKfac* k, const SgPolicyDesc& d, float* d_grad) {
    const SgTrunk& ac = d.trunk[0];
    const SgTrunk& cr = d.trunk[1];
    const int O = d.O, A = d.A, H = ac.H, Hc = cr.H;
    const int nf[SG_KFAC_NF] = {O, H, H, Hc, Hc, H, H, Hc, Hc, 1, A, A};
    int fo = 0, vo = 0;
    int64_t wo = 0;
    k->lds_n = 0;
    while (16 * (k->lds_n + 1) * (k->lds_n + 1) + 8192 <= ctx->lds_bytes) ++k->lds_n;
    for (int f = 0; f < SG_KFAC_NF; ++f) {
        if (f == SG_KFAC_NA) k->g_start = fo;
        k->n[f] = nf[f]; k->off[f] = fo; k->voff[f] = vo; k->woff[f] = wo;
        fo += nf[f] * nf[f]; vo += nf[f];
        if (nf[f] > k->lds_n) wo += 2 * (int64_t)nf[f] * nf[f];
        SG_REQUIRE(nf[f] <= 512, "sg_acktr_create: a %d-wide Kronecker factor is larger than the eigensolver's 512", nf[f]);
    }
    k->fac_total = fo; k->vec_total = vo; k->work_doubles = wo;
    const KfacModule mods[SG_KFAC_MODULES] = {
        {0, 5, ac.off + ac.w1, d.ldO, H, O, 0},     {-1, 5, ac.off + ac.b1, 1, H, 1, 0},
        {1, 6, ac.off + ac.w2, ac.ldH, H, H, 0},    {-1, 6, ac.off + ac.b2, 1, H, 1, 0},
        {0, 7, cr.off + cr.w1, d.ldO, Hc, O, 0},    {-1, 7, cr.off + cr.b1, 1, Hc, 1, 0},
        {3, 8, cr.off + cr.w2, cr.ldH, Hc, Hc, 0},  {-1, 8, cr.off + cr.b2, 1, Hc, 1, 0},
        {4, 9, cr.off + cr.wh, cr.ldH, 1, Hc, 0},   {-1, 9, cr.off + cr.bh, 1, 1, 1, 0},
        {2, 10, ac.off + ac.wh, ac.ldH, A, H, 0},   {-1, 10, ac.off + ac.bh, 1, A, 1, 0},
        {-1, 11, ac.off + ac.ex, 1, A, 1, 0}};
    int to = 0;
    k->max_tiles = 0;
    for (int m = 0; m < SG_KFAC_MODULES; ++m) {
        k->mod[m] = mods[m];
        k->mod[m].toff = to;
        to += mods[m].out * mods[m].in;
        k->max_tiles = std::max(k->max_tiles, ((mods[m].out + 31) / 32) * ((mods[m].in + 31) / 32));
    }
    k->tmp_total = to;
    SG_CHECK(sg_dev_malloc((void**)&k->d_acc, sizeof(float) * fo));
    SG_CHECK(sg_dev_malloc((void**)&k->d_m, sizeof(float) * fo));
    SG_CHECK(sg_dev_malloc((void**)&k->d_Q, sizeof(float) * fo));
    SG_CHECK(sg_dev_malloc((void**)&k->d_d, sizeof(float) * vo));
    if (wo) SG_CHECK(sg_dev_malloc((void**)&k->d_work, sizeof(double) * wo));
    SG_CHECK(sg_dev_malloc((void**)&k->d_ks, sizeof(KfacDevState)));
    SG_CHECK(sg_dev_malloc((void**)&k->d_vec, sizeof(float) * (d.total + 8)));
    SG_CHECK(sg_dev_malloc((void**)&k->d_t0, sizeof(float) * to));
    SG_CHECK(sg_dev_malloc((void**)&k->d_t1, sizeof(float) * to));
    SG_CHECK(sg_dev_malloc((void**)&k->d_one, sizeof(float) * 4));
    SG_CHECK(sg_dev_malloc((void**)&k->d_vpart, sizeof(float) * SG_KFAC_MODULES * k->max_tiles));
    SG_CHECK(hipMemsetAsync(k->d_m, 0, sizeof(float) * fo, ctx->stream));
    SG_CHECK(hipMemsetAsync(k->d_Q, 0, sizeof(float) * fo, ctx->stream));
    SG_CHECK(hipMemsetAsync(k->d_d, 0, sizeof(float) * vo, ctx->stream));
    SG_CHECK(hipMemsetAsync(k->d_ks, 0, sizeof(KfacDevState), ctx->stream));
    SG_CHECK(hipMemsetAsync(k->d_vec, 0, sizeof(float) * (d.total + 8), ctx->stream));
    const float one[4] = {1.f, 1.f, 1.f, 1.f};
    SG_COPY_SYNC(ctx, k->d_one, one, sizeof one, hipMemcpyHostToDevice);
    std::vector<KfacJob> jobs(4 * SG_KFAC_MODULES);
    for (int m = 0; m < SG_KFAC_MODULES; ++m) {
        const KfacModule& md = k->mod[m];
        const float* Qa = md.a_f >= 0 ? k->d_Q + k->off[md.a_f] : k->d_one;
        const float* da = md.a_f >= 0 ? k->d_d + k->voff[md.a_f] : k->d_one;
        const float* Qg = k->d_Q + k->off[md.g_f];
        const float* dg = k->d_d + k->voff[md.g_f];
        float* t0 = k->d_t0 + md.toff;
        float* t1 = k->d_t1 + md.toff;
        const int M = md.out, N = md.in;
        KfacJob j;
        memset(&j, 0, sizeof j);
        j.M = M; j.N = N;
        KfacJob s1 = j, s2 = j, s3 = j, s4 = j;
        s1.K = M; s1.A = Qg; s1.lda = M; s1.ta = 1; s1.B = d_grad + md.goff; s1.ldb = md.gld; s1.C = t0; s1.ldc = N;
        s2.K = N; s2.A = t0; s2.lda = N; s2.B = Qa; s2.ldb = N; s2.C = t1; s2.ldc = N; s2.epi = 1; s2.dg = dg; s2.da = da;
        s3.K = M; s3.A = Qg; s3.lda = M; s3.B = t1; s3.ldb = N; s3.C = t0; s3.ldc = N;
        s4.K = N; s4.A = t0; s4.lda = N; s4.B = Qa; s4.ldb = N; s4.tb = 1; s4.C = k->d_vec + md.goff; s4.ldc = md.gld; s4.epi = 2;
        s4.G = d_grad + md.goff; s4.ldg = md.gld;
        jobs[0 * SG_KFAC_MODULES + m] = s1;
        jobs[1 * SG_KFAC_MODULES + m] = s2;
        jobs[2 * SG_KFAC_MODULES + m] = s3;
        jobs[3 * SG_KFAC_MODULES + m] = s4;
    }
    SG_CHECK(sg_dev_malloc((void**)&k->d_jobs, sizeof(KfacJob) * jobs.size()));
    SG_COPY_SYNC(ctx, k->d_jobs, jobs.data(), sizeof(KfacJob) * jobs.size(), hipMemcpyHostToDevice);
    std::vector<int4> tiles;
    for (int f = 0; f < SG_KFAC_NF; ++f) {
        const int T = (k->n[f] + 15) / 16;
        for (int ti = 0; ti < T; ++ti)
            for (int tj = ti; tj < T; ++tj) tiles.push_back(make_int4(f, ti, tj, 0));
    }
    k->n_tiles = (int)tiles.size();
    SG_CHECK(sg_dev_malloc((void**)&k->d_tiles, sizeof(int4) * tiles.size()));
    SG_COPY_SYNC(ctx, k->d_tiles, tiles.data(), sizeof(int4) * tiles.size(), hipMemcpyHostToDevice);
    return 0;
}

static KfacEigArgs kfac_eig_args(const SgKfac* k) {
    KfacEigArgs e;
    memset(&e, 0, sizeof e);
    e.m = k->d_m; e.Q = k->d_Q; e.dv = k->d_d; e.work = k->d_work;
    for (int f = 0; f < SG_KFAC_NF; ++f) { e.n[f] = k->n[f]; e.off[f] = k->off[f]; e.voff[f] = k->voff[f]; e.woff[f] = k->woff[f]; }
    e.lds_n = k->lds_n; e.tf = k->cfg.Tf; e.ks = k->d_ks;
    return e;
}

static size_t kfac_eig_lds(const SgKfac* k) {
    int nl = 0;
    for (int f = 0; f < SG_KFAC_NF; ++f) if (k->n[f] <= k->lds_n) nl = std::max(nl, k->n[f]);
    return sizeof(double) * 2 * (size_t)nl * nl;
}

extern "C" int sg_ppo_create(sg_ctx* ctx, sg_policy* p, const sg_ppo_config* cfg, sg_ppo** out) {
    SG_DEVICE_WIDE();
    SG_REQUIRE(ctx && p && cfg && out, "sg_ppo_create: NULL argument");
    SG_REQUIRE(!(p->recurrent && ctx->use_comm && ctx->world > 1), "sg_ppo_create: PPO with a recurrent policy runs on one rank: this "
               "context has a communicator of world %d (data-parallel PPO through time is not implemented)", ctx->world);
    SG_REQUIRE(cfg->ppo_epoch > 0 && cfg->num_mini_batch > 0, "sg_ppo_create: ppo_epoch and num_mini_batch must be positive");
    SG_REQUIRE(ppo_fwd_lds(p->desc, 1, true) <= (size_t)ctx->lds_bytes && ppo_bwd_lds(p->desc, 1, true) <= (size_t)ctx->lds_bytes,
               "sg_ppo_create: the 16-row activation tiles of this policy do not fit LDS (%zu / %zu > %d bytes)",
               ppo_fwd_lds(p->desc, 1, true), ppo_bwd_lds(p->desc, 1, true), ctx->lds_bytes);
    SG_CHECK(hipSetDevice(ctx->device));
    sg_ppo* a = new sg_ppo();
    a->ctx = ctx; a->policy = p; a->cfg = *cfg;
    const size_t tot = sg_policy_padded_count(p) + 8;
    SG_CHECK(sg_dev_malloc((void**)&a->d_m, sizeof(float) * tot));
    SG_CHECK(sg_dev_malloc((void**)&a->d_v, sizeof(float) * tot));
    SG_CHECK(sg_dev_malloc((void**)&a->d_grad, sizeof(float) * tot));
    SG_CHECK(sg_dev_malloc((void**)&a->d_state, sizeof(SgOptState)));
    SG_CHECK(sg_dev_malloc((void**)&a->d_loss_acc, sizeof(double) * 8));
    SG_CHECK(sg_dev_malloc((void**)&a->d_part, sizeof(float) * ((tot + 8 + SG_PPO_REDUCE_PARAMS - 1) / SG_PPO_REDUCE_PARAMS + 8 +
                                                                 (p->recurrent ? (p->gru.total + 255) / 256 : 0))));
    SG_CHECK(hipMemsetAsync(a->d_m, 0, sizeof(float) * tot, ctx->stream));
    SG_CHECK(hipMemsetAsync(a->d_v, 0, sizeof(float) * tot, ctx->stream));
    SG_CHECK(hipMemsetAsync(a->d_loss_acc, 0, sizeof(double) * 8, ctx->stream));
    SG_CHECK(sg_dev_malloc((void**)&a->d_pair, SG_PAIR_BYTES));
    SG_CHECK(hipMemsetAsync(a->d_pair, 0, SG_PAIR_BYTES, ctx->stream));
    SgOptState st;
    memset(&st, 0, sizeof st);
    st.lr = cfg->lr;
    SG_CHECK(hipMemcpyAsync(a->d_state, &st, sizeof st, hipMemcpyHostToDevice, ctx->stream));
    SG_CHECK(hipStreamSynchronize(ctx->stream));
    sg_ctx_learner_born(ctx);
    *out = a;
    return 0;
}

extern "C" int sg_a2c_create(sg_ctx* ctx, sg_policy* p, const sg_a2c_config* cfg, sg_ppo** out) {
    SG_REQUIRE(ctx && p && cfg && out, "sg_a2c_create: NULL argument");
    SG_REQUIRE(!p->recurrent, "sg_a2c_create: A2C is implemented for feed-forward policies only, not for a recurrent Policy");
    SG_REQUIRE(p->desc.kind == SG_POLICY_MLP, "sg_a2c_create: A2C is implemented for Policy (MLP) only, not for SplitPolicy");
    SG_REQUIRE(!(ctx->use_comm && ctx->world > 1), "sg_a2c_create: A2C runs on one rank: this context has a communicator of "
               "world %d (data-parallel A2C is not implemented)", ctx->world);
    SG_REQUIRE(cfg->alpha >= 0.f && cfg->alpha <= 1.f && cfg->eps >= 0.f && cfg->max_grad_norm > 0.f,
               "sg_a2c_create: alpha must lie in [0, 1], eps >= 0 and max_grad_norm > 0 (got %g, %g, %g)", (double)cfg->alpha,
               (double)cfg->eps, (double)cfg->max_grad_norm);
    sg_ppo_config pc;
    memset(&pc, 0, sizeof pc);
    pc.ppo_epoch = 1; pc.num_mini_batch = 1;
    pc.value_loss_coef = cfg->value_loss_coef; pc.entropy_coef = cfg->entropy_coef;
    pc.lr = cfg->lr; pc.eps = cfg->eps; pc.max_grad_norm = cfg->max_grad_norm;
    sg_ppo* a = nullptr;
    SG_TRY(sg_ppo_create(ctx, p, &pc, &a));
    a->a2c = true;
    a->alpha = cfg->alpha;
    *out = a;
    return 0;
}

extern "C" int sg_acktr_create(sg_ctx* ctx, sg_policy* p, const sg_acktr_config* cfg, sg_ppo** out) {
    SG_DEVICE_WIDE();
    SG_REQUIRE(ctx && p && cfg && out, "sg_acktr_create: NULL argument");
    SG_REQUIRE(!p->recurrent, "sg_acktr_create: ACKTR is not defined for a recurrent Policy (the reference refuses it too: "
               "a2c/arguments.py:253-255)");
    SG_REQUIRE(p->desc.kind == SG_POLICY_MLP, "sg_acktr_create: ACKTR is implemented for Policy (MLP) only, not for SplitPolicy");
    SG_REQUIRE(!(ctx->use_comm && ctx->world > 1), "sg_acktr_create: ACKTR runs on one rank: this context has a communicator of "
               "world %d (data-parallel ACKTR is not implemented)", ctx->world);
    SG_REQUIRE(cfg->lr > 0.f && cfg->momentum >= 0.f && cfg->momentum < 1.f && cfg->stat_decay > 0.f && cfg->stat_decay < 1.f &&
               cfg->kl_clip > 0.f && cfg->damping >= 0.f && cfg->Tf >= 1,
               "sg_acktr_create: need lr > 0, momentum in [0, 1), stat_decay in (0, 1), kl_clip > 0, damping >= 0 and Tf >= 1");
    sg_a2c_config ac;
    memset(&ac, 0, sizeof ac);
    ac.value_loss_coef = cfg->value_loss_coef; ac.entropy_coef = cfg->entropy_coef;
    ac.lr = cfg->lr; ac.eps = 1.f; ac.alpha = 0.f; ac.max_grad_norm = 1.f;
    sg_ppo* a = nullptr;
    SG_TRY(sg_a2c_create(ctx, p, &ac, &a));
    a->kfac = new SgKfac();
    a->kfac->cfg = *cfg;
    const int rc = kfac_setup(ctx, a->kfac, p->desc, a->d_grad);
    if (rc != 0) {
        const std::string err = sg_last_error();
        sg_ppo_destroy(a);
        sg_set_error("%s", err.c_str());
        return rc;
    }
    *out = a;
    return 0;
}

extern "C" int sg_acktr_set_value_noise(sg_ppo* a, const float* eps, int64_t n) {
    SG_REQUIRE(a, "sg_acktr_set_value_noise: NULL argument");
    SG_REQUIRE(a->kfac, "sg_acktr_set_value_noise: not an ACKTR handle");
    SgKfac* k = a->kfac;
    if (!eps) {
        k->eps_pending = false;
        k->eps_host.clear();
        return 0;
    }
    SG_REQUIRE(n > 0 && n < (1ll << 30), "sg_acktr_set_value_noise: %lld values", (long long)n);
    k->eps_host.assign(eps, eps + n);
    k->eps_pending = true;
    return 0;
}

extern "C" int sg_acktr_get_state(sg_ppo* a, float* m_aa, int64_t n_aa, float* m_gg, int64_t n_gg, float* momentum_buf,
                                  int64_t n, int64_t* steps) {
    SG_REQUIRE(a && m_aa && m_gg && momentum_buf && steps, "sg_acktr_get_state: NULL argument");
    SG_REQUIRE(a->kfac, "sg_acktr_get_state: not an ACKTR handle");
    const SgKfac* k = a->kfac;
    const SgPolicyDesc& d = a->policy->desc;
    SG_REQUIRE(n == sg_policy_flat_count(d), "sg_acktr_get_state: bad momentum length");
    int64_t want_aa = 0, want_gg = 0;
    for (int m = 0; m < SG_KFAC_MODULES; ++m) {
        want_aa += (int64_t)k->mod[m].in * k->mod[m].in;
        want_gg += (int64_t)k->mod[m].out * k->mod[m].out;
    }
    SG_REQUIRE(n_aa == want_aa && n_gg == want_gg, "sg_acktr_get_state: m_aa / m_gg take %lld / %lld floats", (long long)want_aa,
               (long long)want_gg);
    std::vector<float> fac(k->fac_total), buf(d.total);
    KfacDevState ks;
    SG_CHECK(hipSetDevice(a->ctx->device));
    SG_CHECK(hipStreamSynchronize(a->ctx->stream));
    SG_COPY_SYNC(a->ctx, fac.data(), k->d_m, sizeof(float) * k->fac_total, hipMemcpyDeviceToHost);
    SG_COPY_SYNC(a->ctx, buf.data(), a->d_m, sizeof(float) * d.total, hipMemcpyDeviceToHost);
    SG_COPY_SYNC(a->ctx, &ks, k->d_ks, sizeof ks, hipMemcpyDeviceToHost);
    SG_REQUIRE(!ks.err, "sg_acktr_get_state: k_kfac_eig hit its sweep cap (%d) on an earlier update", SG_KFAC_SWEEPS);
    float *pa = m_aa, *pg = m_gg;
    for (int m = 0; m < SG_KFAC_MODULES; ++m) {
        const KfacModule& md = k->mod[m];
        if (md.a_f >= 0) {
            memcpy(pa, fac.data() + k->off[md.a_f], sizeof(float) * md.in * md.in);
        } else {
            pa[0] = ks.steps > 0 ? 1.f : 0.f;
        }
        pa += (int64_t)md.in * md.in;
        memcpy(pg, fac.data() + k->off[md.g_f], sizeof(float) * md.out * md.out);
        pg += (int64_t)md.out * md.out;
    }
    sg_policy_unpad(d, buf.data(), momentum_buf);
    *steps = ks.steps;
    return 0;
}

extern "C" int sg_ppo_destroy(sg_ppo* a) {
    SG_DEVICE_WIDE();
    if (!a) return 0;
    (void)hipStreamSynchronize(a->ctx->stream);
    sg_ctx_learner_gone(a->ctx);
    for (auto& q : a->ctx->res_a) if (q == a) q = nullptr;
    float* ptrs[] = {a->d_m, a->d_v, a->d_grad, a->d_slabs, a->d_state, a->d_part, a->d_stacks, a->d_mobs_mat, a->d_mact, a->d_mrows,
                     a->d_h0, a->d_gru};
    for (float* q : ptrs) if (q) (void)sg_dev_free(q);
    if (a->d_perms) (void)sg_dev_free(a->d_perms);
    if (a->d_loss_acc) (void)sg_dev_free(a->d_loss_acc);
    if (a->d_dbg) (void)sg_dev_free(a->d_dbg);
    if (a->d_pair) (void)sg_dev_free(a->d_pair);
    if (a->h_h0) (void)sg_host_release(a->h_h0);
    for (hipEvent_t ev : a->h0_ev) if (ev) (void)hipEventDestroy(ev);
    if (a->steps_graph) (void)hipGraphExecDestroy(a->steps_graph);
    kfac_free(a);
    delete a;
    return 0;
}

__global__ void k_set_lr(SgOptState* st, float lr) { st->lr = lr; }

extern "C" int sg_ppo_set_lr(sg_ppo* a, float lr) {
    SG_REQUIRE(a, "sg_ppo_set_lr: NULL argument");
    SG_CHECK(hipSetDevice(a->ctx->device));
    a->cfg.lr = lr;
    hipLaunchKernelGGL(k_set_lr, dim3(1), dim3(1), 0, a->ctx->stream, reinterpret_cast<SgOptState*>(a->d_state), lr);
    SG_CHECK(hipGetLastError());
    return 0;
}

extern "C" int sg_ppo_set_symmetry(sg_ppo* a, float coef, const float* m_obs, const float* m_act) {
    SG_REQUIRE(a, "sg_ppo_set_symmetry: NULL argument");
    SG_REQUIRE(!a->a2c, "sg_ppo_set_symmetry: the mirror-symmetry loss is a PPO option; this is an A2C / ACKTR handle");
    SG_REQUIRE(coef >= 0.f && coef < INFINITY, "sg_ppo_set_symmetry: symmetry_coef must be finite and >= 0 (got %g)", (double)coef);
    sg_ctx* ctx = a->ctx;
    const SgPolicyDesc& d = a->policy->desc;
    SG_CHECK(hipSetDevice(ctx->device));
    SG_CHECK(hipStreamSynchronize(ctx->stream));
    if (coef == 0.f) { a->sym_coef = 0.f; return 0; }
    SG_REQUIRE(m_act, "sg_ppo_set_symmetry: symmetry_coef > 0 needs the action mirror m_act");
    SG_REQUIRE(d.kind == SG_POLICY_MLP, "sg_ppo_set_symmetry: the mirror-symmetry loss is implemented for Policy (MLP) only, "
               "not for SplitPolicy");
    SG_REQUIRE(!a->policy->recurrent, "sg_ppo_set_symmetry: the mirror-symmetry loss is implemented for feed-forward policies only, "
               "not for a recurrent Policy");
    SG_REQUIRE(ppo_bwd_sym_lds(d, 1, true) <= (size_t)ctx->lds_bytes,
               "sg_ppo_set_symmetry: the 16-row tiles of the symmetric step do not fit LDS (%zu > %d bytes)", ppo_bwd_sym_lds(d, 1, true),
               ctx->lds_bytes);
    if (!a->d_mact) SG_CHECK(sg_dev_malloc((void**)&a->d_mact, sizeof(float) * d.A * d.A));
    SG_COPY_SYNC(ctx, a->d_mact, m_act, sizeof(float) * d.A * d.A, hipMemcpyHostToDevice);
    if (m_obs) {
        if (!a->d_mobs_mat) SG_CHECK(sg_dev_malloc((void**)&a->d_mobs_mat, sizeof(float) * d.O * d.O));
        SG_COPY_SYNC(ctx, a->d_mobs_mat, m_obs, sizeof(float) * d.O * d.O, hipMemcpyHostToDevice);
    } else if (a->d_mobs_mat) {
        SG_CHECK(sg_dev_free(a->d_mobs_mat));
        a->d_mobs_mat = nullptr;
    }
    a->sym_coef = coef;
    return 0;
}

extern "C" int sg_ppo_set_mirrored_obs(sg_ppo* a, const float* host, int64_t count) {
    SG_REQUIRE(a && host, "sg_ppo_set_mirrored_obs: NULL argument");
    SG_REQUIRE(!a->a2c, "sg_ppo_set_mirrored_obs: the mirror-symmetry loss is a PPO option; this is an A2C / ACKTR handle");
    SG_REQUIRE(count > 0 && count % a->policy->desc.O == 0, "sg_ppo_set_mirrored_obs: %lld floats is not a whole number of %d-float rows",
               (long long)count, a->policy->desc.O);
    sg_ctx* ctx = a->ctx;
    SG_CHECK(hipSetDevice(ctx->device));
    SG_CHECK(hipStreamSynchronize(ctx->stream));
    if (a->mrows_cap < count) {
        if (a->d_mrows) SG_CHECK(sg_dev_free(a->d_mrows));
        SG_CHECK(sg_dev_malloc((void**)&a->d_mrows, sizeof(float) * count));
        a->mrows_cap = count;
    }
    SG_COPY_SYNC(ctx, a->d_mrows, host, sizeof(float) * count, hipMemcpyHostToDevice);
    a->mrows_host = count;
    return 0;
}

extern "C" int sg_ppo_last_symmetry_loss(sg_ppo* a, float* out) {
    SG_REQUIRE(a && out, "sg_ppo_last_symmetry_loss: NULL argument");
    SG_CHECK(hipSetDevice(a->ctx->device));
    double acc = 0.0;
    SG_TRY(sg_ctx_fetch_f64(a->ctx, a->d_loss_acc + 3, &acc, 1));
    *out = (float)(acc / ((double)a->cfg.ppo_epoch * a->cfg.num_mini_batch));
    return 0;
}

extern "C" int sg_ppo_last_perms(sg_ppo* a, int64_t* perms, int64_t count) {
    SG_REQUIRE(a && perms, "sg_ppo_last_perms: NULL argument");
    SG_REQUIRE(a->last_perm_count > 0, "sg_ppo_last_perms: no update has run on this agent");
    SG_REQUIRE(count == a->last_perm_count, "sg_ppo_last_perms: the last update used %lld indices, asked for %lld",
               (long long)a->last_perm_count, (long long)count);
    SG_CHECK(hipSetDevice(a->ctx->device));
    SG_CHECK(hipStreamSynchronize(a->ctx->stream));
    SG_COPY_SYNC(a->ctx, perms, a->d_perms, sizeof(int64_t) * count, hipMemcpyDeviceToHost);
    return 0;
}

extern "C" int sg_ppo_get_adam(sg_ppo* a, float* m, float* v, int64_t n, int64_t* step) {
    SG_REQUIRE(a && m && v && step, "sg_ppo_get_adam: NULL argument");
    SG_REQUIRE(!a->kfac, "sg_ppo_get_adam: an ACKTR handle has K-FAC state, not Adam's (sg_acktr_get_state)");
    SG_REQUIRE(!a->a2c, "sg_ppo_get_adam: an A2C handle has RMSprop state, not Adam's (sg_a2c_get_rmsprop)");
    const SgPolicyDesc& d = a->policy->desc;
    const sg_policy* pol = a->policy;
    const int64_t n_gru = pol->recurrent ? sg_gru_flat_count(pol->gru) : 0;
    SG_REQUIRE(n == sg_policy_flat_count(d) + n_gru, "sg_ppo_get_adam: bad length");
    const size_t ptot = sg_policy_padded_count(pol);
    std::vector<float> pm(ptot), pv(ptot);
    SG_CHECK(hipStreamSynchronize(a->ctx->stream));
    SG_COPY_SYNC(a->ctx, pm.data(), a->d_m, sizeof(float) * ptot, hipMemcpyDeviceToHost);
    SG_COPY_SYNC(a->ctx, pv.data(), a->d_v, sizeof(float) * ptot, hipMemcpyDeviceToHost);
    if (pol->recurrent) {
        sg_gru_unpad(pol->gru, pm.data() + pol->gru.off, m);
        sg_gru_unpad(pol->gru, pv.data() + pol->gru.off, v);
    }
    sg_policy_unpad(d, pm.data(), m + n_gru);
    sg_policy_unpad(d, pv.data(), v + n_gru);
    *step = a->opt_t;
    return 0;
}

extern "C" int sg_ppo_set_adam(sg_ppo* a, const float* m, const float* v, int64_t n, int64_t step) {
    SG_REQUIRE(a && m && v, "sg_ppo_set_adam: NULL argument");
    SG_REQUIRE(!a->kfac, "sg_ppo_set_adam: an ACKTR handle has K-FAC state, not Adam's (sg_acktr_get_state)");
    SG_REQUIRE(!a->a2c, "sg_ppo_set_adam: an A2C handle has RMSprop state, not Adam's (sg_a2c_set_rmsprop)");
    const SgPolicyDesc& d = a->policy->desc;
    const sg_policy* pol = a->policy;
    const int64_t n_gru = pol->recurrent ? sg_gru_flat_count(pol->gru) : 0;
    SG_REQUIRE(n == sg_policy_flat_count(d) + n_gru, "sg_ppo_set_adam: bad length");
    const size_t ptot = sg_policy_padded_count(pol);
    std::vector<float> pm(ptot, 0.f), pv(ptot, 0.f);
    if (pol->recurrent) {
        sg_gru_pad(pol->gru, m, pm.data() + pol->gru.off);
        sg_gru_pad(pol->gru, v, pv.data() + pol->gru.off);
    }
    sg_policy_pad(d, m + n_gru, pm.data());
    sg_policy_pad(d, v + n_gru, pv.data());
    SG_REQUIRE(step >= 0 && step < (1ll << 30), "sg_ppo_set_adam: step out of range");
    const int t0 = (int)step;
    SG_CHECK(hipStreamSynchronize(a->ctx->stream));
    SG_COPY_SYNC(a->ctx, a->d_m, pm.data(), sizeof(float) * ptot, hipMemcpyHostToDevice);
    SG_COPY_SYNC(a->ctx, a->d_v, pv.data(), sizeof(float) * ptot, hipMemcpyHostToDevice);
    SG_COPY_SYNC(a->ctx, &reinterpret_cast<SgOptState*>(a->d_state)->t0, &t0, sizeof t0, hipMemcpyHostToDevice);
    a->scratch_key = 0;
    a->pair_primed = false;
    a->opt_t = step;
    return 0;
}

extern "C" int sg_a2c_get_rmsprop(sg_ppo* a, float* square_avg, int64_t n, int64_t* step) {
    SG_REQUIRE(a && square_avg && step, "sg_a2c_get_rmsprop: NULL argument");
    SG_REQUIRE(!a->kfac, "sg_a2c_get_rmsprop: an ACKTR handle has K-FAC state, not RMSprop's (sg_acktr_get_state)");
    SG_REQUIRE(a->a2c, "sg_a2c_get_rmsprop: not an A2C handle (sg_ppo_get_adam)");
    const SgPolicyDesc& d = a->policy->desc;
    SG_REQUIRE(n == sg_policy_flat_count(d), "sg_a2c_get_rmsprop: bad length");
    std::vector<float> pv(d.total);
    SG_CHECK(hipSetDevice(a->ctx->device));
    SG_CHECK(hipStreamSynchronize(a->ctx->stream));
    SG_COPY_SYNC(a->ctx, pv.data(), a->d_v, sizeof(float) * d.total, hipMemcpyDeviceToHost);
    sg_policy_unpad(d, pv.data(), square_avg);
    *step = a->opt_t;
    return 0;
}

extern "C" int sg_a2c_set_rmsprop(sg_ppo* a, const float* square_avg, int64_t n, int64_t step) {
    SG_REQUIRE(a && square_avg, "sg_a2c_set_rmsprop: NULL argument");
    SG_REQUIRE(!a->kfac, "sg_a2c_set_rmsprop: an ACKTR handle has K-FAC state, not RMSprop's (sg_acktr_get_state)");
    SG_REQUIRE(a->a2c, "sg_a2c_set_rmsprop: not an A2C handle (sg_ppo_set_adam)");
    const SgPolicyDesc& d = a->policy->desc;
// ... 529 lines not shown
                step_off[(size_t)e * M + k] = (int)n_own;
                for (int64_t i = 0; i < mb_global; ++i) {
                    const int64_t g = perms[(size_t)e * TN_perm + (size_t)k * mb_global + i];
                    const int64_t t = g / Ng, c = g - t * Ng, owner = c / r->N;
                    if (owner == ctx->rank) {
                        SG_REQUIRE(n_own < TN, "sg_ppo_update: epoch %d hands this rank more than its %lld rows", e, (long long)TN);
                        own_perm[(size_t)e * TN + n_own++] = t * r->N + (c - owner * r->N);
                    }
                }
                const int cnt = (int)n_own - step_off[(size_t)e * M + k];
                step_cnt[(size_t)e * M + k] = cnt;
                if (cnt > mb) mb = cnt;
            }
            epoch_rows[e] = n_own;
        }
    } else {
        for (int e = 0; e < E; ++e)
            for (int k = 0; k < M; ++k) { step_cnt[(size_t)e * M + k] = mb; step_off[(size_t)e * M + k] = k * mb; }
    }

    const bool sym = a->sym_coef > 0.f;
    if (sym) {
        if (a->d_mobs_mat) {
            if (a->mrows_cap < TN * d.O) {
                SG_CHECK(hipStreamSynchronize(ctx->stream));
                if (a->d_mrows) SG_CHECK(sg_dev_free(a->d_mrows));
                SG_CHECK(sg_dev_malloc((void**)&a->d_mrows, sizeof(float) * TN * d.O));
                a->mrows_cap = TN * d.O;
            }
            hipLaunchKernelGGL(k_mirror_rows, dim3((unsigned)((TN * d.O + 255) / 256)), dim3(256), 0, ctx->stream,
                               r->d_field[SG_F_OBS], a->d_mobs_mat, a->d_mrows, TN, d.O);
            SG_CHECK(hipGetLastError());
        } else {
            SG_REQUIRE(a->mrows_host == TN * d.O, "sg_ppo_update: the symmetry loss takes its mirrored observations from the host: "
                       "sg_ppo_set_mirrored_obs must hand over %lld floats (T*N rows of %d) before every update (pending: %lld)",
                       (long long)(TN * d.O), d.O, (long long)a->mrows_host);
            a->mrows_host = 0;
        }
    }

    float* adv = r->d_field[SG_F_ADVANTAGES];
    double* stats = a->d_loss_acc + 4;
    hipLaunchKernelGGL(k_adv_stats, dim3(1), dim3(1024), 0, ctx->stream, r->d_field[SG_F_RETURNS],
                       r->d_field[SG_F_VALUE_PREDS], TN, adv, stats, 0);
    if (ctx->use_comm) SG_TRY(sg_comm_allreduce_f64(ctx, stats, 3));
    hipLaunchKernelGGL(k_adv_stats, dim3(1), dim3(1024), 0, ctx->stream, r->d_field[SG_F_RETURNS],
                       r->d_field[SG_F_VALUE_PREDS], TN, adv, stats, 1);
    if (ctx->use_comm) SG_TRY(sg_comm_allreduce_f64(ctx, stats + 1, 1));
    hipLaunchKernelGGL(k_adv_stats, dim3(64), dim3(1024), 0, ctx->stream, r->d_field[SG_F_RETURNS],
                       r->d_field[SG_F_VALUE_PREDS], TN, adv, stats, 2);
    SG_CHECK(hipGetLastError());

    if (a->perms_cap < (int64_t)E * TN) {
        SG_CHECK(hipStreamSynchronize(ctx->stream));
        if (a->d_perms) SG_CHECK(sg_dev_free(a->d_perms));
        SG_CHECK(sg_dev_malloc((void**)&a->d_perms, sizeof(int64_t) * (size_t)E * TN));
        a->perms_cap = (int64_t)E * TN;
    }
    a->last_perm_count = owned ? 0 : (int64_t)E * TN;
    if (owned) {
        SG_CHECK(hipMemcpyAsync(a->d_perms, own_perm.data(), sizeof(int64_t) * (size_t)E * TN, hipMemcpyHostToDevice, ctx->stream));
        SG_CHECK(hipStreamSynchronize(ctx->stream));
    } else if (perms) {
        SG_CHECK(hipMemcpyAsync(a->d_perms, perms, sizeof(int64_t) * (size_t)E * TN, hipMemcpyHostToDevice, ctx->stream));
        if (!out3) SG_CHECK(hipStreamSynchronize(ctx->stream));
    } else {
        for (int e = 0; e < E; ++e)
            SG_TRY(sg_fill_perm(ctx, a->d_perms + (size_t)e * TN, TN, seed, (uint64_t)e * 2654435761ull + (uint64_t)ctx->rank));
    }

    const int ncols = d.n_trunks + (sym ? 1 : 0);
    int MT = ((size_t)((mb + 15) / 16) * (size_t)(d.total + 8) * sizeof(float) > ((size_t)24 << 20) ||
              ((mb + 31) / 32) * ncols >= ctx->num_cu) ? 2 : 1;
    if (const char* e = getenv("SG_PPO_ROWS")) {
        const int v = atoi(e);
        if (v == 16 || v == 32 || v == 64) MT = v / 16;
    }
    const bool gw = sg_policy_needs_gw(ctx, d) || ppo_fwd_lds(d, 1, false) > (size_t)ctx->lds_bytes ||
                    ppo_bwd_lds(d, 1, false) > (size_t)ctx->lds_bytes || (sym && ppo_bwd_sym_lds(d, 1, false) > (size_t)ctx->lds_bytes);
    if ((gw || sym) && MT > 2) MT = 2;
    while (MT > 1 && (ppo_fwd_lds(d, MT, gw) > (size_t)ctx->lds_bytes || ppo_bwd_lds(d, MT, gw) > (size_t)ctx->lds_bytes ||
                      (sym && ppo_bwd_sym_lds(d, MT, gw) > (size_t)ctx->lds_bytes))) MT /= 2;
    const int R = 16 * MT;
    const int G = (mb + R - 1) / R;
    const int mbp = G * R;
    const int ldP = stack_ldP(d);
    const int slab_stride = (d.total + 8 + 63) & ~63;
    const int TNp = (int)TN + 64 + (owned ? mbp : 0);

    const size_t slab_f = (size_t)(sym ? 2 : 1) * G * slab_stride;
    const size_t xm_off = ((size_t)TNp * (d.ldO + d.A + 4) + 3) & ~(size_t)3;
    const size_t epoch_f = sym ? xm_off + (size_t)TNp * d.ldO : (size_t)TNp * (d.ldO + d.A + 4);
    const size_t stack_f = (size_t)ncols * mbp * (2 * (size_t)d.ldH + ldP);
    if (a->slabs_cap < slab_f || a->stacks_cap < epoch_f + stack_f) {
        SG_CHECK(hipStreamSynchronize(ctx->stream));
        if (a->d_slabs) SG_CHECK(sg_dev_free(a->d_slabs));
        if (a->d_stacks) SG_CHECK(sg_dev_free(a->d_stacks));
        SG_CHECK(sg_dev_malloc((void**)&a->d_slabs, sizeof(float) * slab_f));
        SG_CHECK(sg_dev_malloc((void**)&a->d_stacks, sizeof(float) * (epoch_f + stack_f)));
        a->slabs_cap = slab_f;
        a->stacks_cap = epoch_f + stack_f;
        a->scratch_key = 0;
    }
    const uint64_t key = ((uint64_t)G << 40) ^ ((uint64_t)slab_stride << 20) ^ ((uint64_t)mbp << 8) ^ (uint64_t)TNp ^ ((uint64_t)MT << 60) ^
                         ((uint64_t)sym << 63);
    if (a->scratch_key != key) {
        SG_CHECK(hipMemsetAsync(a->d_slabs, 0, sizeof(float) * slab_f, ctx->stream));
        SG_CHECK(hipMemsetAsync(a->d_stacks, 0, sizeof(float) * (epoch_f + stack_f), ctx->stream));
        a->scratch_key = key;
    }
    hipLaunchKernelGGL(k_zero_f64, dim3(1), dim3(64), 0, ctx->stream, a->d_loss_acc, 4);

    float* epX = a->d_stacks;
    float* epACT = epX + (size_t)TNp * d.ldO;
    float* epSC = epACT + (size_t)TNp * d.A;
    float* epXm = sym ? a->d_stacks + xm_off : nullptr;
    float* stk = a->d_stacks + epoch_f;

    EpochGatherArgs ga;
    ga.obs = r->d_field[SG_F_OBS]; ga.actions = r->d_field[SG_F_ACTIONS]; ga.old_logp = r->d_field[SG_F_LOGP];
    ga.adv = adv; ga.vpred = r->d_field[SG_F_VALUE_PREDS]; ga.ret = r->d_field[SG_F_RETURNS];
    ga.TN = TN; ga.O = d.O; ga.Op = d.Op; ga.ldO = d.ldO; ga.A = d.A; ga.sc_stride = TNp;
    ga.X = epX; ga.ACT = epACT; ga.SC = epSC;
    ga.mobs = sym ? a->d_mrows : nullptr; ga.Xm = epXm;

    PpoArgs pa;
    pa.d = d; pa.params = a->policy->d_params;
    pa.sc_stride = TNp; pa.mb = mb; pa.mbp = mbp; pa.inv_B = 1.0f / (float)mb_global;
    pa.clip = a->cfg.clip_param; pa.vcoef = a->cfg.value_loss_coef; pa.ecoef = a->cfg.entropy_coef;
    pa.use_clipped = a->cfg.use_clipped_value_loss;
    pa.slabs = a->d_slabs; pa.slab_stride = slab_stride; pa.ldP = ldP; pa.dbg = a->d_dbg;
    pa.st = reinterpret_cast<SgOptState*>(a->d_state); pa.G = G; pa.k1 = 0;
    pa.pair = a->d_pair;
    pa.Xm = nullptr; pa.MA = a->d_mact;
    pa.sym_c = sym ? (float)(2.0 * a->sym_coef / ((double)mb_global * d.A)) : 0.f;
    for (int t = 0; t < 3; ++t) {
        const bool on = t < ncols;
        pa.H1[t] = on ? stk : nullptr; if (on) stk += (size_t)mbp * d.ldH;
        pa.H2[t] = on ? stk : nullptr; if (on) stk += (size_t)mbp * d.ldH;
        pa.OUT[t] = on ? stk : nullptr; if (on) stk += (size_t)mbp * ldP;
    }
    const int wb_f = gw ? 0 : max_trunk_floats(d), wb_b = gw ? 0 : max_bwd_floats(d);
    const bool fused = !sym && ppo_fused(d, MT);
    const size_t lds_fc = sizeof(float) * ((size_t)wb_f + R * d.ldO + 2 * R * d.ldH + 2 * R * ldP + ((R * d.A + 3) & ~3) + 7 * R);
    const char* cfenv = getenv("SG_PPO_CRITIC_FIRST");
    const bool crit_first = !gw && !fused && d.kind == SG_POLICY_SPLIT && MT <= 2 && lds_fc <= (size_t)ctx->lds_bytes &&
                            (cfenv ? cfenv[0] == '1' : G * d.n_trunks > ctx->num_cu);
    const char* penv = getenv("SG_PPO_PAIR");
    const bool pair = !gw && !fused && !crit_first && d.kind == SG_POLICY_SPLIT && d.n_trunks == 3 && MT <= 2 &&
                      lds_fc <= (size_t)ctx->lds_bytes && 3 * G <= ctx->num_cu && 2 * ldP + 2 <= std::min(d.trunk[0].ldH, d.trunk[1].ldH) && !a->d_dbg &&
                      !a->self_wait_failed && (penv ? strcmp(penv, "0") != 0 : sg_ctx_exclusive(ctx));
    if (pair && !a->pair_primed) SG_CHECK(hipMemsetAsync(a->d_stacks, 0, sizeof(float) * (epoch_f + stack_f), ctx->stream));
    a->pair_primed = pair;
    const size_t lds_f = ppo_fwd_lds(d, MT, gw), lds_b = sym ? ppo_bwd_sym_lds(d, MT, gw) : ppo_bwd_lds(d, MT, gw);
    const int nblk = (d.total + 8 + 255) / 256;
    const int nblk_r = (d.total + 8 + SG_PPO_REDUCE_PARAMS - 1) / SG_PPO_REDUCE_PARAMS;
    SgOptState* st = reinterpret_cast<SgOptState*>(a->d_state);

    auto enqueue_steps = [&]() -> int {
        hipLaunchKernelGGL(k_opt_prepare_first, dim3(1), dim3(1), 0, ctx->stream, st);
        for (int e = 0; e < E; ++e) {
            ga.perm = a->d_perms + (size_t)e * TN;
            ga.TN = epoch_rows[e];
            if (ga.TN) hipLaunchKernelGGL(sym ? k_ppo_epoch_gather_sym : k_ppo_epoch_gather, dim3((unsigned)((ga.TN + 63) / 64)), dim3(256), 0,
                                          ctx->stream, ga);
            for (int k = 0; k < M; ++k) {
                const size_t rb = (size_t)step_off[(size_t)e * M + k];
                pa.mb = step_cnt[(size_t)e * M + k];
                pa.X = epX + rb * d.ldO; pa.ACT = epACT + rb * d.A; pa.SC = epSC + rb;
                if (sym) pa.Xm = epXm + rb * d.ldO;
                pa.k1 = e * M + k + 1;
                if (sym) {
                    pa.wbuf_floats = wb_f;
                    launch_ppo_fwd_sym(ctx, MT, d, dim3(G, 3), lds_f, pa, gw);
                    pa.wbuf_floats = wb_b;
                    launch_ppo_bwd_sym(ctx, MT, d, dim3(G, 3), lds_b, pa, gw);
                } else if (pair) {
                    pa.wbuf_floats = wb_f;
                    launch_ppo_pair(ctx, MT, d, G, lds_fc, pa);
                } else if (crit_first) {
                    pa.wbuf_floats = wb_f;
                    launch_ppo_fwd_critic(ctx, MT, d, dim3(G, d.n_trunks), lds_fc > lds_f ? lds_fc : lds_f, pa);
                    pa.wbuf_floats = wb_b;
                    launch_ppo_bwd(ctx, MT, d, dim3(G, d.n_trunks - 1), lds_b, pa, false, false);
                } else {
                    if (!fused) {
                        pa.wbuf_floats = wb_f;
                        launch_ppo_fwd(ctx, MT, d, dim3(G, d.n_trunks), lds_f, pa, gw);
                    }
                    pa.wbuf_floats = fused ? wb_f : wb_b;
                    launch_ppo_bwd(ctx, MT, d, dim3(G, d.n_trunks), lds_b, pa, fused, gw);
                }
                if (sym) SG_LAUNCH(ctx, SG_PROF_PPO_REDUCE, k_ppo_reduce_sym, dim3(nblk_r), dim3(256), 0, a->d_slabs, G, slab_stride,
                                   d.total, a->d_grad, a->d_part, d.trunk[0].off, d.trunk[0].off + d.trunk[0].ex);
                else SG_LAUNCH(ctx, SG_PROF_PPO_REDUCE, k_ppo_reduce, dim3(nblk_r), dim3(256), 0, a->d_slabs, G, slab_stride,
                               d.total, a->d_grad, a->d_part);
                if (ctx->use_comm) {
                    SG_TRY(sg_comm_allreduce_f32(ctx, a->d_grad, d.total + 8));
                    hipLaunchKernelGGL(k_sumsq, dim3(nblk), dim3(256), 0, ctx->stream, a->d_grad, d.total, a->d_part);
                }
                SG_LAUNCH(ctx, SG_PROF_PPO_ADAM, sym ? k_ppo_adam_sym : k_ppo_adam, dim3(nblk), dim3(256), 0, a->policy->d_params, a->d_m,
                          a->d_v, a->d_grad, a->d_part, ctx->use_comm ? nblk : nblk_r, d.total, st, e * M + k + 1, a->cfg.eps,
                          a->cfg.max_grad_norm, pa.inv_B, a->d_loss_acc);
            }
        }
        hipLaunchKernelGGL(k_opt_commit, dim3(1), dim3(1), 0, ctx->stream, st, E * M);
        return 0;
    };
    const char* genv = getenv("SG_PPO_GRAPH");
    const char* gcenv = getenv("SG_PPO_GRAPH_COMM");
    const bool comm_ok = !a->graph_refused && (!ctx->use_comm || (sg_comm_graph_ok(ctx) && !(gcenv && !strcmp(gcenv, "0"))));
    bool use_graph = comm_ok && !owned && !ctx->profile && !a->d_dbg && !(genv && !strcmp(genv, "0"));
    if (use_graph) {
        uint32_t fbits[6];
        const float fv[6] = {a->cfg.clip_param, a->cfg.value_loss_coef, a->cfg.entropy_coef, a->cfg.eps, a->cfg.max_grad_norm, pa.inv_B};
        memcpy(fbits, fv, sizeof fbits);
        uint32_t cbits;
        memcpy(&cbits, &a->sym_coef, sizeof cbits);
        const uint64_t key[18] = {(uint64_t)(uintptr_t)a->d_slabs, (uint64_t)(uintptr_t)a->d_stacks, (uint64_t)(uintptr_t)a->d_perms,
                                  (uint64_t)(uintptr_t)r->d_field[SG_F_OBS], (uint64_t)(uintptr_t)r->d_field[SG_F_ACTIONS],
                                  (uint64_t)(uintptr_t)r->d_field[SG_F_RETURNS], (uint64_t)(uintptr_t)a->policy->d_params,
                                  (uint64_t)TN, ((uint64_t)E << 32) | (uint64_t)M, ((uint64_t)MT << 32) | (uint64_t)G,
                                  ((uint64_t)fbits[0] << 32) | fbits[1], ((uint64_t)fbits[2] << 32) | fbits[3],
                                  ((uint64_t)fbits[4] << 32) | fbits[5], (uint64_t)a->cfg.use_clipped_value_loss,
                                  (uint64_t)(uintptr_t)r->d_field[SG_F_LOGP], 0x50504full + (fused ? 1 : 0) + (ctx->use_comm ? 2 : 0) + (crit_first ? 4 : 0) + (gw ? 8 : 0) + (pair ? 16 : 0) + (sg_comm_peer_on(ctx) ? 32 : 0) + (sym ? 64 : 0) + ((uint64_t)sg_comm_peer_generation(ctx) << 32),
                                  sym ? (uint64_t)(uintptr_t)a->d_mrows : 0, sym ? (uint64_t)cbits : 0};
        if (!a->steps_graph || memcmp(key, a->steps_graph_key, sizeof key) != 0) {
            if (a->steps_graph) { SG_CHECK(hipGraphExecDestroy(a->steps_graph)); a->steps_graph = nullptr; }
            if (sg_try_capture(ctx, &a->steps_graph, enqueue_steps) != 0) {
                a->graph_refused = true;
                use_graph = false;
            } else {
                memcpy(a->steps_graph_key, key, sizeof key);
            }
        }
        if (use_graph) SG_CHECK(hipGraphLaunch(a->steps_graph, ctx->stream));
    }
    if (!use_graph) SG_TRY(enqueue_steps());
    SG_CHECK(hipGetLastError());
    a->opt_t += (int64_t)E * M;
    if (!out3) return 0;
    double acc[3];
    SG_TRY(sg_ctx_fetch_f64(ctx, a->d_loss_acc, acc, 3));
    if (pair && (acc[0] != acc[0] || acc[1] != acc[1] || acc[2] != acc[2])) {
        unsigned err = 0;
        SG_COPY_SYNC(ctx, &err, a->d_pair + SG_PAIR_ERR_WORD, sizeof err, hipMemcpyDeviceToHost);
        if (err) {
            SG_CHECK(hipMemsetAsync(a->d_pair + SG_PAIR_ERR_WORD, 0, sizeof err, ctx->stream));
            a->self_wait_failed = true;
            SG_REQUIRE(false, "sg_ppo_update: a workgroup of k_ppo_pair waited %d s for its partner's words and gave "
                       "up (the policy's state is undefined; SG_PPO_PAIR=0 runs the multi-launch step)", (int)(SG_PAIR_TIMEOUT_TICKS / 100000000ll));
        }
    }
    const double nu = (double)E * M;
    for (int i = 0; i < 3; ++i) out3[i] = (float)(acc[i] / nu);
    return 0;
}

__global__ void k_publish(double* dst, const double* d_acc, const double* d_scal, const double* p_acc, double n_d, double n_p,
                          const unsigned* d_err, const unsigned* a_err, const unsigned* peer_err) {
    const int t = threadIdx.x;
    if (t < 3) dst[t] = d_acc ? d_acc[t] : 0.0;
    else if (t < 8) dst[t] = d_scal ? d_scal[t - 3] : 0.0;
    else if (t < 11) dst[t] = p_acc ? p_acc[t - 8] : 0.0;
    else if (t == 11) dst[t] = n_d;
    else if (t == 12) dst[t] = n_p;
    else if (t == 13) dst[t] = d_err ? (double)*d_err : 0.0;
    else if (t == 14) dst[t] = a_err ? (double)*a_err : 0.0;
    else if (t == 15) dst[t] = peer_err ? (double)__hip_atomic_load(peer_err, __ATOMIC_RELAXED, __HIP_MEMORY_SCOPE_AGENT) : 0.0;
}

extern "C" int sg_results_publish(sg_ctx* ctx, sg_disc* d, sg_ppo* a, int slot) {
    SG_REQUIRE(ctx && slot >= 0 && slot < SG_RESULT_SLOTS, "sg_results_publish: bad argument");
    SG_REQUIRE((!d || d->ctx == ctx) && (!a || a->ctx == ctx), "sg_results_publish: objects of another context");
    SG_CHECK(hipSetDevice(ctx->device));
    hipLaunchKernelGGL(k_publish, dim3(1), dim3(64), 0, ctx->stream, ctx->results + 16 * slot, d ? d->d_loss_acc : nullptr,
                       d ? d->d_scal : nullptr, a ? a->d_loss_acc : nullptr, d ? (double)d->last_n_d : 1.0,
                       a ? (double)a->cfg.ppo_epoch * a->cfg.num_mini_batch : 1.0,
                       d ? sg_disc_err_word(d) : nullptr,
                       (a && a->kfac) ? reinterpret_cast<const unsigned*>(&a->kfac->d_ks->err)
                                      : (a && a->d_pair) ? a->d_pair + SG_PAIR_ERR_WORD : nullptr,
                       sg_comm_peer_err_word(ctx));
    SG_CHECK(hipGetLastError());
    SG_CHECK(hipEventRecord(ctx->res_ev[slot], ctx->stream));
    ctx->res_d[slot] = d;
    ctx->res_a[slot] = a;
    return 0;
}

extern "C" int sg_results_fetch(sg_ctx* ctx, int slot, double out13[13]) {
    SG_REQUIRE(ctx && out13 && slot >= 0 && slot < SG_RESULT_SLOTS, "sg_results_fetch: bad argument");
    SG_CHECK(hipEventSynchronize(ctx->res_ev[slot]));
    const double* src = ctx->results + 16 * slot;
    memcpy(out13, src, sizeof(double) * 13);
    const bool d_err = src[13] != 0.0;
    const bool k_err = src[14] != 0.0 && ctx->res_a[slot] && ctx->res_a[slot]->kfac;
    const bool a_err = src[14] != 0.0 && !k_err;
    if (src[15] != 0.0) {
        SG_CHECK(hipSetDevice(ctx->device));
        if (unsigned* w = sg_comm_peer_err_word(ctx)) SG_CHECK(hipMemsetAsync(w, 0, sizeof(unsigned), ctx->stream));
        SG_REQUIRE(false, "sg_results_fetch: rank %d: a peer-mesh all-reduce (SG_COMM_PEER) waited 20 s for a peer's flags and gave up "
                   "during or before the update this slot reports; that step's gradient was NaN on this rank", ctx->rank);
    }
    if (d_err || a_err) {
        SG_CHECK(hipSetDevice(ctx->device));
        sg_disc* d = ctx->res_d[slot];
        sg_ppo* a = ctx->res_a[slot];
        if (d_err && d) {
            d->self_wait_failed = true;
            SG_CHECK(hipMemsetAsync(sg_disc_err_word(d), 0, sizeof(unsigned), ctx->stream));
        }
        if (a_err && a && a->d_pair) {
            a->self_wait_failed = true;
            SG_CHECK(hipMemsetAsync(a->d_pair + SG_PAIR_ERR_WORD, 0, sizeof(unsigned), ctx->stream));
        }
        SG_REQUIRE(false, "sg_results_fetch: %s%s%s waited for workgroups of its own launch and gave up during the update this slot reports "
                   "(another process on this GPU?): the %s undefined and the slot's losses are NaN; later updates of the object run the "
                   "multi-launch form", d_err ? "k_disc_step4" : "", d_err && a_err ? " and " : "", a_err ? "k_ppo_pair" : "",
                   d_err && a_err ? "discriminator's and the policy's state are" : d_err ? "discriminator's state is" : "policy's state is");
    }
    SG_REQUIRE(!k_err, "sg_results_fetch: k_kfac_eig hit its sweep cap (%d) during or before the ACKTR update this slot reports: "
               "the K-FAC eigenbases are not valid and the update stepped with them", SG_KFAC_SWEEPS);
    return 0;
}
```

### simgan_amd/csrc/sg_ppo_kernels.hpp

```cpp
#pragma once
#include "sg_common.h"
#include "sg_thin.hpp"

#define HALF_LOG_2PI 0.91893853320467274178f

struct PpoArgs {
    SgPolicyDesc d;
    const float* params;
    const float* X;
    const float* ACT;
    const float* SC;
    int sc_stride;
    int mb, mbp;
    float inv_B;
    float clip, vcoef, ecoef;
    int use_clipped;
    float* H1[3];
    float* H2[3];
    float* OUT[3];
    float* slabs;
    int slab_stride;
    int ldP;
    int wbuf_floats;
    long long* dbg;
    SgOptState* st;
    int k1, G;
    unsigned* pair;
    const float* Xm;
    const float* MA;
    float sym_c;
    float* DX[2] = {nullptr, nullptr};
};

#define SG_PAIR_BYTES 64
#define SG_PAIR_TIMEOUT_TICKS 300000000ll



#define SG_LDS_SYNC() asm volatile("s_waitcnt lgkmcnt(0)\n\ts_barrier" ::: "memory")

#define SG_PPO_STAMP(n) do { if (a.dbg && threadIdx.x == 0 && blockIdx.y == 0) a.dbg[blockIdx.x * 16 + (n)] = clock64(); } while (0)
#define SG_PPO_WALL(n) do { if (a.dbg && threadIdx.x == 0 && blockIdx.y < 2) a.dbg[(blockIdx.x + 512 * blockIdx.y) * 16 + (n)] = wall_clock64(); } while (0)

struct EpochGatherArgs {
    const float *obs, *actions, *old_logp, *adv, *vpred, *ret;
    const int64_t* perm;
    int64_t TN;
    int O, Op, ldO, A, sc_stride;
    float *X, *ACT, *SC;
    const float* mobs;
    float* Xm;
};

template <bool SYM = false, bool ROLLOUT_ORDER = false>
__device__ __forceinline__ void sg_ppo_epoch_gather_body(const EpochGatherArgs& a) {
    __shared__ int IDX[64];
    const int tid = threadIdx.x;
    const int64_t row0 = (int64_t)blockIdx.x * 64;
    if (tid < 64) {
        const int64_t rr = row0 + tid;
        const int idx = rr < a.TN ? (ROLLOUT_ORDER ? (int)rr : (int)a.perm[rr]) : -1;
        IDX[tid] = idx;
        if (ROLLOUT_ORDER) {
            if (idx >= 0) a.SC[3 * (size_t)a.sc_stride + rr] = a.ret[idx];
        } else if (idx >= 0) {
            a.SC[0 * (size_t)a.sc_stride + rr] = a.old_logp[idx];
            a.SC[1 * (size_t)a.sc_stride + rr] = a.adv[idx];
            a.SC[2 * (size_t)a.sc_stride + rr] = a.vpred[idx];
            a.SC[3 * (size_t)a.sc_stride + rr] = a.ret[idx];
        }
    }
    __syncthreads();
    for (int base = tid; base < 64 * a.Op; base += 8 * blockDim.x) {
        float v[8];
#pragma unroll
        for (int u = 0; u < 8; ++u) {
            const int i = base + u * blockDim.x;
            const int r = i / a.Op, c = i - r * a.Op;
            v[u] = (i < 64 * a.Op && IDX[r] >= 0 && c < a.O) ? a.obs[(size_t)IDX[r] * a.O + c] : 0.f;
        }
#pragma unroll
        for (int u = 0; u < 8; ++u) {
            const int i = base + u * blockDim.x;
            if (i < 64 * a.Op && IDX[i / a.Op] >= 0) a.X[(size_t)(row0 + i / a.Op) * a.ldO + (i % a.Op)] = v[u];
        }
        if (SYM) {
#pragma unroll
            for (int u = 0; u < 8; ++u) {
                const int i = base + u * blockDim.x;
                const int r = i / a.Op, c = i - r * a.Op;
                v[u] = (i < 64 * a.Op && IDX[r] >= 0 && c < a.O) ? a.mobs[(size_t)IDX[r] * a.O + c] : 0.f;
            }
#pragma unroll
            for (int u = 0; u < 8; ++u) {
                const int i = base + u * blockDim.x;
                if (i < 64 * a.Op && IDX[i / a.Op] >= 0) a.Xm[(size_t)(row0 + i / a.Op) * a.ldO + (i % a.Op)] = v[u];
            }
        }
    }
    for (int i = tid; i < 64 * a.A; i += blockDim.x) {
        const int r = i / a.A, c = i - r * a.A;
        if (IDX[r] >= 0) a.ACT[(size_t)(row0 + r) * a.A + c] = a.actions[(size_t)IDX[r] * a.A + c];
    }
}

__global__ __launch_bounds__(256) void k_ppo_epoch_gather(EpochGatherArgs a) { sg_ppo_epoch_gather_body<false>(a); }
__global__ __launch_bounds__(256) void k_ppo_epoch_gather_sym(EpochGatherArgs a) { sg_ppo_epoch_gather_body<true>(a); }
__global__ __launch_bounds__(256) void k_a2c_gather(EpochGatherArgs a) { sg_ppo_epoch_gather_body<false, true>(a); }

__global__ __launch_bounds__(256) void k_mirror_rows(const float* obs, const float* m, float* out, int64_t rows, int O) {
    const int64_t idx = (int64_t)blockIdx.x * blockDim.x + threadIdx.x;
    if (idx >= rows * O) return;
    const int64_t r = idx / O;
    const int i = (int)(idx - r * O);
    const float* x = obs + r * O;
    const float* mi = m + (size_t)i * O;
    double s = 0.0;
    for (int j = 0; j < O; ++j) {
        const float w = mi[j];
        if (w != 0.f) s += (double)w * (double)x[j];
    }
    out[idx] = (float)s;
}

template <int MT, int KO, int KH, bool GW = false, bool SYM = false>
__device__ __forceinline__ void sg_ppo_fwd_body(const PpoArgs& a, const int t, const int bx) {
    extern __shared__ __attribute__((aligned(16))) float smem[];
    constexpr int R = 16 * MT;
    const SgPolicyDesc& d = a.d;
    const int tid = threadIdx.x;
    const bool mirror = SYM && t == 2;
    const SgTrunk tr = d.trunk[mirror ? 0 : t];
    const int Op = (KO > 0 && KH > 0) ? 16 * KO : d.Op, Hp = (KO > 0 && KH > 0) ? 16 * KH : tr.Hp;
    const int ldO = Op + 4, ldH = Hp + 4, ldP = a.ldP;
    const float* W = GW ? a.params + tr.off : smem;
    float* X = smem + a.wbuf_floats;
    float* H1 = X + R * ldO;
    float* H2 = H1 + R * ldH;
    const int row0 = bx * R;

    SG_PPO_STAMP(0);
    float4 wv[12];
    if (!GW) sg_stage_issue<12>(wv, a.params + tr.off, tr.size / 4);
    {
        const float4* gx = reinterpret_cast<const float4*>((mirror ? a.Xm : a.X) + (size_t)row0 * ldO);
        float4* lx = reinterpret_cast<float4*>(X);
        for (int i = tid; i < R * ldO / 4; i += blockDim.x) lx[i] = gx[i];
    }
    SG_PPO_STAMP(1);
    if (!GW) sg_stage_commit<12>(smem, wv, a.params + tr.off, tr.size / 4);
    __syncthreads();
    SG_PPO_STAMP(2);
    const float* b1 = W + tr.b1;
    const float* b2 = W + tr.b2;
    const float* bh = W + tr.bh;
    float* gH1 = a.H1[t] + (size_t)row0 * ldH;
    float* gH2 = a.H2[t] + (size_t)row0 * ldH;
    float* gOUT = a.OUT[t] + (size_t)row0 * ldP;
    sg_layer_nt_u<MT, GW>(X, ldO, W + tr.w1, ldO, Op, Hp, [&](int r, int c, float v) {
        const float h = sg_tanh(v + b1[c]);
        H1[r * ldH + c] = h;
        gH1[r * ldH + c] = h;
    });
    __syncthreads();
    SG_PPO_STAMP(3);
    sg_layer_nt_u<MT, GW>(H1, ldH, W + tr.w2, ldH, Hp, Hp, [&](int r, int c, float v) {
        const float h = sg_tanh(v + b2[c]);
        H2[r * ldH + c] = h;
        gH2[r * ldH + c] = h;
    });
    __syncthreads();
    SG_PPO_STAMP(4);
    sg_layer_nt_u<MT, GW>(H2, ldH, W + tr.wh, ldH, Hp, tr.Pp, [&](int r, int c, float v) { gOUT[r * ldP + c] = v + bh[c]; });
    __syncthreads();
    SG_PPO_STAMP(5);
}

template <int MT, int KO, int KH, bool GW = false>
__global__ __launch_bounds__(512) void k_ppo_fwd(PpoArgs a) {
    sg_ppo_fwd_body<MT, KO, KH, GW>(a, blockIdx.y, blockIdx.x);
}
template <int MT, int KO, int KH, bool GW = false>
__global__ __launch_bounds__(512) void k_ppo_fwd_sym(PpoArgs a) {
    sg_ppo_fwd_body<MT, KO, KH, GW, true>(a, blockIdx.y, blockIdx.x);
}

template <int MT, int KO, int KH, bool FUSED, bool GW = false, bool PAIR = false, bool SYM = false, bool A2C = false, bool DX = false>
__device__ __forceinline__ void sg_ppo_bwd_body(const PpoArgs& a, const int t, const int bx) {
    static_assert(!(SYM && (FUSED || PAIR)), "the symmetric step runs the two-launch form");
    static_assert(!DX || ((FUSED || GW) && !PAIR && !SYM && !A2C), "d loss / d X needs w1 at hand: the fused or the global-weight form");
    static_assert(!(A2C && (FUSED || PAIR || SYM)), "the A2C step runs the two-launch form");
    extern __shared__ __attribute__((aligned(16))) float smem[];
    constexpr int R = 16 * MT;
    const SgPolicyDesc& d = a.d;
    const int tid = threadIdx.x;
    const bool mirror = SYM && t == 2;
    const SgTrunk tr = d.trunk[mirror ? 0 : t];
    const int Op = (KO > 0 && KH > 0) ? 16 * KO : d.Op, Hp = (KO > 0 && KH > 0) ? 16 * KH : tr.Hp;
    const bool critic = t == d.n_trunks - 1;
    const bool mlp = d.kind == SG_POLICY_MLP;
    const int ldO = Op + 4, ldH = Hp + 4, ldP = a.ldP, A = d.A;
    float* Wimg = smem;
    const int w_first = FUSED ? 0 : tr.w2;
    const float* W = GW ? a.params + tr.off : Wimg - w_first;
    const int wfl = tr.size - w_first;
    float* X = Wimg + a.wbuf_floats;
    float* H1 = X + R * ldO;
    float* H2 = H1 + R * ldH;
    float* O0 = H2 + R * ldH;
    float* O1 = O0 + R * ldP;
    float* ACT = O1 + R * ldP;
    float* SC = ACT + ((R * A + 3) & ~3);
    float* ROWL = SC + 4 * R;
    int* VALID = reinterpret_cast<int*>(ROWL + 2 * R);
    float* OM = reinterpret_cast<float*>(VALID + R);
    float* MA = OM + R * ldP;
    const int row0 = bx * R;
    float* slab = a.slabs + (size_t)(mirror ? a.G + bx : bx) * a.slab_stride;

    SG_PPO_STAMP(8);
    SG_PPO_WALL(6);
    unsigned pair_tag = 0;
    bool pair_failed = false;
    if (PAIR && !critic) pair_tag = (unsigned)(a.st->t0 + a.k1);
    float4 wv[12];
    if (!GW) sg_stage_issue<12>(wv, a.params + tr.off + w_first, wfl / 4);
    constexpr int UX = MT <= 2 ? 4 : 8;
    constexpr int UO = MT <= 2 ? 2 : 4;
    const int ta = critic ? t : (mirror ? 2 : 0);
    const bool two_heads = !critic && !mlp;
    const float* gX = (mirror ? a.Xm : a.X) + (size_t)row0 * ldO;
    const float* gH1 = a.H1[t] + (size_t)row0 * ldH;
    const float* gH2 = a.H2[t] + (size_t)row0 * ldH;
    const float* gO0 = a.OUT[ta] + (size_t)row0 * ldP;
    const float* gO1 = a.OUT[two_heads ? 1 : ta] + (size_t)row0 * ldP;
    const float* gOM = SYM ? a.OUT[mirror ? 0 : 2] + (size_t)row0 * ldP : nullptr;
    float4 xv[UX], h1v[UX], h2v[UX], o0v[UO], o1v[UO], omv[UO];
    sg_stage_issue<UX>(xv, gX, R * ldO / 4);
    if (!FUSED) {
        sg_stage_issue<UX>(h1v, gH1, R * ldH / 4);
        sg_stage_issue<UX>(h2v, gH2, R * ldH / 4);
        sg_stage_issue<UO>(o0v, gO0, R * ldP / 4);
        if (two_heads) sg_stage_issue<UO>(o1v, gO1, R * ldP / 4);
        if (SYM && !critic) sg_stage_issue<UO>(omv, gOM, R * ldP / 4);
    }
    float actv[2] = {0.f, 0.f}, scv[4] = {0.f, 0.f, 0.f, 0.f};
    if (!critic && !mirror) {
#pragma unroll
        for (int u = 0; u < 2; ++u) { const int i = tid + u * 256; actv[u] = a.ACT[(size_t)row0 * A + (i < R * A ? i : 0)]; }
    }
    {
        const int r = tid < R ? tid : 0;
        if (A2C) {
            scv[3] = a.SC[(size_t)3 * a.sc_stride + row0 + r];
            if (!critic) scv[0] = a.OUT[d.n_trunks - 1][(size_t)(row0 + r) * ldP];
        } else {
#pragma unroll
            for (int q = 0; q < 4; ++q) scv[q] = a.SC[(size_t)q * a.sc_stride + row0 + r];
        }
    }
    sg_stage_commit<UX>(X, xv, gX, R * ldO / 4);
    if (!FUSED) {
        sg_stage_commit<UX>(H1, h1v, gH1, R * ldH / 4);
        sg_stage_commit<UX>(H2, h2v, gH2, R * ldH / 4);
        sg_stage_commit<UO>(O0, o0v, gO0, R * ldP / 4);
        if (two_heads) sg_stage_commit<UO>(O1, o1v, gO1, R * ldP / 4);
        if (SYM && !critic) {
            sg_stage_commit<UO>(OM, omv, gOM, R * ldP / 4);
            for (int i = tid; i < A * A; i += blockDim.x) MA[i] = a.MA[i];
        }
    }
    if (!critic && !mirror) {
#pragma unroll
        for (int u = 0; u < 2; ++u) { const int i = tid + u * 256; if (i < R * A) ACT[i] = actv[u]; }
        for (int i = tid + 512; i < R * A; i += blockDim.x) ACT[i] = a.ACT[(size_t)row0 * A + i];
    }
    if (tid < R) {
        VALID[tid] = row0 + tid < a.mb;
#pragma unroll
        for (int q = 0; q < 4; ++q) SC[q * R + tid] = scv[q];
    }
    SG_PPO_STAMP(0);
    if (!GW) sg_stage_commit<12>(Wimg, wv, a.params + tr.off + w_first, wfl / 4);
    __syncthreads();
    SG_PPO_STAMP(1);
    if (FUSED) {
        const float* b1 = W + tr.b1;
        const float* b2 = W + tr.b2;
        const float* bh = W + tr.bh;
        sg_layer_nt_u<MT, GW>(X, ldO, W + tr.w1, ldO, Op, Hp, [&](int r, int c, float v) { H1[r * ldH + c] = sg_tanh(v + b1[c]); });
        __syncthreads();
        SG_PPO_STAMP(2);
        sg_layer_nt_u<MT, GW>(H1, ldH, W + tr.w2, ldH, Hp, Hp, [&](int r, int c, float v) { H2[r * ldH + c] = sg_tanh(v + b2[c]); });
        __syncthreads();
        SG_PPO_STAMP(3);
        float* Oown = (PAIR && t == 1) ? O1 : O0;
        sg_layer_nt_u<MT, GW>(H2, ldH, W + tr.wh, ldH, Hp, tr.Pp, [&](int r, int c, float v) { Oown[r * ldP + c] = v + bh[c]; });
        __syncthreads();
        SG_PPO_STAMP(4);
        if (PAIR && !critic) {
            float* Ooth = t == 1 ? O0 : O1;
            auto word_base = [](float* p) { return reinterpret_cast<unsigned long long*>((reinterpret_cast<uintptr_t>(p) + 7) & ~(uintptr_t)7); };
            unsigned long long* xown = word_base(a.H1[t] + (size_t)row0 * ldH);
            const unsigned long long* xoth = word_base(a.H1[1 - t] + (size_t)row0 * ldH);
            const int Pown = tr.Pp, Poth = d.trunk[1 - t].Pp;
            for (int i = tid; i < R * Pown; i += blockDim.x) {
                const int r = i / Pown, c = i - r * Pown;
                const unsigned long long w = ((unsigned long long)pair_tag << 32) | (unsigned long long)__float_as_uint(Oown[r * ldP + c]);
                __hip_atomic_store(xown + i, w, __ATOMIC_RELAXED, __HIP_MEMORY_SCOPE_AGENT);
            }
            bool ok = __hip_atomic_load(a.pair + SG_PAIR_ERR_WORD, __ATOMIC_RELAXED, __HIP_MEMORY_SCOPE_AGENT) == 0;
            const long long deadline = wall_clock64() + SG_PAIR_TIMEOUT_TICKS;
            for (int i = tid; ok && i < R * Poth; i += blockDim.x) {
                const int r = i / Poth, c = i - r * Poth;
                unsigned long long w = 0;
                for (int it = 0;; ++it) {
                    w = __hip_atomic_load(xoth + i, __ATOMIC_RELAXED, __HIP_MEMORY_SCOPE_AGENT);
                    if ((unsigned)(w >> 32) == pair_tag) break;
                    if ((it & 31) == 31 && wall_clock64() > deadline) { ok = false; break; }
                    __builtin_amdgcn_s_sleep(1);
                }
                Ooth[r * ldP + c] = __uint_as_float((unsigned)w);
            }
            pair_failed = __syncthreads_or(!ok) != 0;
        }
    }
    SG_PPO_STAMP(9);

    if (SYM && !critic) {
        float* own = mirror ? O0 : OM;
        const float* mu = mirror ? OM : O0;
        for (int i = tid; i < R * tr.Pp; i += blockDim.x) {
            const int r = i / tr.Pp, k = i - r * tr.Pp;
            float e = 0.f;
            if (k < A && VALID[r]) {
                float s = 0.f;
                for (int j = 0; j < A; ++j) s += MA[k * A + j] * mu[r * ldP + j];
                e = s - (mirror ? O0 : OM)[r * ldP + k];
            }
            own[r * ldP + k] = mirror ? -a.sym_c * e : e;
        }
        __syncthreads();
    }

    if (mirror) {
    } else if (critic) {
        if (tid < R) {
            const int r = tid;
            const float v = O0[r * ldP];
            float dv = 0.f, lv = 0.f;
            if (VALID[r]) {
                const float Rt = SC[3 * R + r], vo = SC[2 * R + r];
                if (A2C) {
                    dv = 2.f * a.inv_B * (v - Rt);
                    lv = (Rt - v) * (Rt - v);
                } else if (a.use_clipped) {
                    const float dvv = v - vo;
                    const float vc = vo + fminf(fmaxf(dvv, -a.clip), a.clip);
                    const float u = (v - Rt) * (v - Rt), w = (vc - Rt) * (vc - Rt);
                    const float m1 = u > w ? 1.f : (u < w ? 0.f : 0.5f);
                    const float pass = (dvv >= -a.clip && dvv <= a.clip) ? 1.f : 0.f;
                    dv = 0.5f * a.inv_B * (m1 * 2.f * (v - Rt) + (1.f - m1) * 2.f * (vc - Rt) * pass);
                    lv = 0.5f * fmaxf(u, w);
                } else {
                    dv = 0.5f * a.inv_B * (-2.f) * (Rt - v);
                    lv = 0.5f * (Rt - v) * (Rt - v);
                }
                dv *= a.vcoef;
            }
            O0[r * ldP] = dv;
            ROWL[r] = lv;
        }
    } else {
        const SgTrunk tra = d.trunk[0];
        const int L = blockDim.x / R;
        if (A <= 8 * L) {
            const int r = tid / L, sub = tid - r * L;
            float* o0 = O0 + r * ldP;
            float* o1 = O1 + r * ldP;
            float sig[8], dif[8];
            float* pmv[8];
            float* plv[8];
            float lp = 0.f, en = 0.f;
#pragma unroll
            for (int j = 0; j < 8; ++j) {
                const int k = sub + j * L;
                sig[j] = 1.f; dif[j] = 0.f; pmv[j] = nullptr; plv[j] = nullptr;
                if (k < A) {
                    float mean, ls;
                    if (mlp) { pmv[j] = o0 + k; plv[j] = o1 + k; mean = *pmv[j]; ls = W[tra.ex + k]; }
                    else if (k < d.nc) { pmv[j] = o0 + k; plv[j] = o0 + d.nc + k; mean = *pmv[j]; ls = *plv[j]; }
                    else { pmv[j] = o1 + (k - d.nc); plv[j] = o1 + (d.na + k - d.nc); mean = *pmv[j]; ls = *plv[j]; }
                    sig[j] = __expf(ls);
                    dif[j] = ACT[r * A + k] - mean;
                    const float lsig = ls;
                    sig[j] = __builtin_amdgcn_rcpf(sig[j] * sig[j]);
                    lp += -0.5f * (dif[j] * dif[j]) * sig[j] - lsig - HALF_LOG_2PI;
                    en += 0.5f + HALF_LOG_2PI + lsig;
                }
            }
            if (L <= 16) {
                lp = sg_dpp_add<0xB1>(lp); en = sg_dpp_add<0xB1>(en);
                lp = sg_dpp_add<0x4E>(lp); en = sg_dpp_add<0x4E>(en);
                if (L >= 8) { lp = sg_dpp_add<0x141>(lp); en = sg_dpp_add<0x141>(en); }
                if (L >= 16) { lp = sg_dpp_add<0x140>(lp); en = sg_dpp_add<0x140>(en); }
            } else {
                for (int o = 1; o < L; o <<= 1) { lp += __shfl_xor(lp, o); en += __shfl_xor(en, o); }
            }
            const float logp = lp, ent = en;
            const bool valid = VALID[r];
            float dlogp = 0.f, la = 0.f;
            if (valid && A2C) {
                const float adv = SC[3 * R + r] - SC[0 * R + r];
                dlogp = -a.inv_B * adv;
                la = -adv * logp;
            } else if (valid) {
                const float adv = SC[1 * R + r];
                const float ratio = __expf(logp - SC[0 * R + r]);
                const float surr1 = ratio * adv;
                const float surr2 = fminf(fmaxf(ratio, 1.f - a.clip), 1.f + a.clip) * adv;
                const float w1 = surr1 < surr2 ? 1.f : (surr1 > surr2 ? 0.f : 0.5f);
                const float inr = (ratio >= 1.f - a.clip && ratio <= 1.f + a.clip) ? 1.f : 0.f;
                dlogp = -a.inv_B * (w1 * adv + (1.f - w1) * adv * inr) * ratio;
                la = -fminf(surr1, surr2);
            }
            const float dent = valid ? a.ecoef * a.inv_B : 0.f;
#pragma unroll
            for (int j = 0; j < 8; ++j) {
                const int k = sub + j * L;
                if (k < A) {
                    const float rvar = sig[j];
                    *pmv[j] = dlogp * dif[j] * rvar;
                    *plv[j] = dlogp * (dif[j] * dif[j] * rvar - 1.f) - dent;
                } else if (mlp && k < tra.Pp) {
                    o1[k] = 0.f;
                }
            }
            if (sub == 0) { ROWL[r] = la; ROWL[R + r] = valid ? ent : 0.f; }
        } else {
        const int rows_per_pass = blockDim.x >> 5;
        for (int r = tid >> 5; r < R; r += rows_per_pass) {
            float* o0 = O0 + r * ldP;
            float* o1 = O1 + r * ldP;
            float logp = 0.f, ent = 0.f;
            for (int k0 = 0; k0 < A; k0 += 32) {
                const int k = k0 + (tid & 31);
                float lp = 0.f, en = 0.f;
                if (k < A) {
                    float mean, ls;
                    if (mlp) { mean = o0[k]; ls = W[tra.ex + k]; }
                    else if (k < d.nc) { mean = o0[k]; ls = o0[d.nc + k]; }
                    else { mean = o1[k - d.nc]; ls = o1[d.na + k - d.nc]; }
                    const float sigma = expf(ls), diff = ACT[r * A + k] - mean, lsig = logf(sigma);
                    lp = -(diff * diff) / (2.f * sigma * sigma) - lsig - HALF_LOG_2PI;
                    en = 0.5f + HALF_LOG_2PI + lsig;
                }
#pragma unroll
                for (int o = 1; o < 32; o <<= 1) { lp += __shfl_xor(lp, o); en += __shfl_xor(en, o); }
                logp += lp;
                ent += en;
            }
            const bool valid = VALID[r];
            float dlogp = 0.f, la = 0.f;
            if (valid && A2C) {
                const float adv = SC[3 * R + r] - SC[0 * R + r];
                dlogp = -a.inv_B * adv;
                la = -adv * logp;
            } else if (valid) {
                const float adv = SC[1 * R + r];
                const float ratio = expf(logp - SC[0 * R + r]);
                const float surr1 = ratio * adv;
                const float surr2 = fminf(fmaxf(ratio, 1.f - a.clip), 1.f + a.clip) * adv;
                const float w1 = surr1 < surr2 ? 1.f : (surr1 > surr2 ? 0.f : 0.5f);
                const float inr = (ratio >= 1.f - a.clip && ratio <= 1.f + a.clip) ? 1.f : 0.f;
                dlogp = -a.inv_B * (w1 * adv + (1.f - w1) * adv * inr) * ratio;
                la = -fminf(surr1, surr2);
            }
            const float dent = valid ? a.ecoef * a.inv_B : 0.f;
            for (int k0 = 0; k0 < A; k0 += 32) {
                const int k = k0 + (tid & 31);
                if (k < A) {
                    float mean, ls, *pm, *pl;
                    if (mlp) { mean = o0[k]; ls = W[tra.ex + k]; pm = o0 + k; pl = o1 + k; }
                    else if (k < d.nc) { pm = o0 + k; pl = o0 + d.nc + k; mean = *pm; ls = *pl; }
                    else { pm = o1 + (k - d.nc); pl = o1 + (d.na + k - d.nc); mean = *pm; ls = *pl; }
                    const float sigma = expf(ls), var = sigma * sigma, diff = ACT[r * A + k] - mean;
                    *pm = dlogp * diff / var;
                    *pl = dlogp * (diff * diff / var - 1.f) - dent;
                } else if (mlp && k < tra.Pp) {
                    o1[k] = 0.f;
                }
            }
            if ((tid & 31) == 0) { ROWL[r] = la; ROWL[R + r] = valid ? ent : 0.f; }
        }
        }
    }
    __syncthreads();
    SG_PPO_STAMP(10);
    float* dout = (critic || t == 0 || mirror) ? O0 : O1;
    if (tid < 64 && (critic || t == 0)) {
        float s0 = tid < R ? ROWL[tid] : 0.f, s1 = (tid < R && !critic) ? ROWL[R + tid] : 0.f;
        s0 = sg_wave_sum(s0); s1 = sg_wave_sum(s1);
        float s3 = 0.f;
        if (SYM) {
            if (tid < R && !critic)
                for (int k = 0; k < A; ++k) s3 += OM[tid * ldP + k] * OM[tid * ldP + k];
            s3 = sg_wave_sum(s3) / (float)A;
        }
        if (tid == 0) {
            float* ls = slab + d.total;
            if (critic) ls[0] = s0;
            else { ls[1] = s0; ls[2] = s1; if (SYM) ls[3] = s3; }
        }
    }
    float* g = slab + tr.off;
    sg_grad_tn<MT, (MT >= 2 ? 8 : 0), true>(dout, ldP, H2, ldH, tr.Pp, Hp, g + tr.wh, ldH, false);
    sg_colsum(dout, ldP, R, tr.Pp, g + tr.bh, false);
    if (tr.EX && !mirror) sg_colsum(O1, ldP, R, SG_PAD16(tr.EX), g + tr.ex, false);
    SG_LDS_SYNC();
    SG_PPO_STAMP(11);
    {
        auto dz_u = [&](float* h) { return [=](int r, int c, float v) { float* ph = h + r * ldH + c; const float hv = *ph; *ph = v * (1.f - hv * hv); }; };
        sg_layer_nn_u<MT>(dout, ldP, W + tr.wh, ldH, tr.Pp, Hp, dz_u(H2));
        SG_LDS_SYNC();
        SG_PPO_STAMP(12);
        sg_grad_tn<MT, (MT >= 2 ? 8 : 0), true>(H2, ldH, H1, ldH, Hp, Hp, g + tr.w2, ldH, false);
        SG_PPO_STAMP(5);
        sg_colsum(H2, ldH, R, Hp, g + tr.b2, false);
        SG_LDS_SYNC();
        SG_PPO_STAMP(13);
        sg_layer_nn_u<MT>(H2, ldH, W + tr.w2, ldH, Hp, Hp, dz_u(H1));
        SG_LDS_SYNC();
        SG_PPO_STAMP(14);
        sg_grad_tn<MT, (MT >= 2 ? 8 : 0), true>(H1, ldH, X, ldO, Hp, Op, g + tr.w1, ldO, false);
        sg_colsum(H1, ldH, R, Hp, g + tr.b1, false);
        SG_LDS_SYNC();
    }
    if (DX) {
        float* gdx = a.DX[t] + (size_t)row0 * ldO;
        sg_layer_nn_u<MT>(H1, ldH, W + tr.w1, ldO, Hp, Op, [&](int r, int c, float v) { gdx[r * ldO + c] = v; });
    }
    SG_PPO_STAMP(15);
    SG_PPO_WALL(7);
    if (PAIR && pair_failed && tid == 0) {
        atomicOr(a.pair + SG_PAIR_ERR_WORD, 1u);
        slab[d.total + 1] = __builtin_nanf("");
    }
}

template <int MT, int KO, int KH, bool FUSED = false, bool GW = false, bool DX = false>
__global__ __launch_bounds__(512) void k_ppo_bwd(PpoArgs a) {
    sg_ppo_bwd_body<MT, KO, KH, FUSED, GW, false, false, false, DX>(a, blockIdx.y, blockIdx.x);
}
template <int MT, int KO, int KH, bool GW = false>
__global__ __launch_bounds__(512) void k_ppo_bwd_sym(PpoArgs a) {
    sg_ppo_bwd_body<MT, KO, KH, false, GW, false, true>(a, blockIdx.y, blockIdx.x);
}

template <int MT, int KO, int KH, bool GW = false>
__global__ __launch_bounds__(512) void k_a2c_bwd(PpoArgs a) {
    sg_ppo_bwd_body<MT, KO, KH, false, GW, false, false, true>(a, blockIdx.y, blockIdx.x);
}

template <int MT, int KO, int KH>
__global__ __launch_bounds__(512) void k_ppo_pair(PpoArgs a) {
    const int bx = (int)blockIdx.x / 3, t = (int)blockIdx.x - 3 * bx;
    sg_ppo_bwd_body<MT, KO, KH, true, false, true>(a, t, bx);
}

template <int MT, int KO, int KH>
__global__ __launch_bounds__(512) void k_ppo_fwd_critic(PpoArgs a) {
    if (blockIdx.y == 0) sg_ppo_bwd_body<MT, KO, KH, true>(a, a.d.n_trunks - 1, blockIdx.x);
    else sg_ppo_fwd_body<MT, KO, KH>(a, blockIdx.y - 1, blockIdx.x);
}

#define SG_PPO_REDUCE_PARAMS 64
template <bool SYM, bool ACC = false>
__device__ __forceinline__ void sg_ppo_reduce_body(const float* slabs, int n_slabs_, int slab_stride, int total,
                                                   float* grad, float* part, int lo2, int hi2, int acc = 0) {
    __shared__ float red[4][64];
    const int lane = threadIdx.x & 63, wave = threadIdx.x >> 6;
    const int i = blockIdx.x * SG_PPO_REDUCE_PARAMS + lane;
    const int n_slabs = (SYM && i >= lo2 && i < hi2) ? 2 * n_slabs_ : n_slabs_;
    float g = 0.f;
    if (i < total + 8) {
        for (int s0 = wave; s0 < n_slabs; s0 += 64) {
            float t[16];
#pragma unroll
            for (int u = 0; u < 16; ++u) {
                const int sidx = s0 + 4 * u;
                t[u] = slabs[(size_t)(sidx < n_slabs ? sidx : s0) * slab_stride + i];
            }
#pragma unroll
            for (int u = 0; u < 16; ++u) g += (s0 + 4 * u < n_slabs) ? t[u] : 0.f;
        }
    }
    red[wave][lane] = g;
    __syncthreads();
    if (wave == 0) {
        g = (red[0][lane] + red[1][lane]) + (red[2][lane] + red[3][lane]);
        if (ACC && acc && i < total + 8) g += grad[i];
        if (i < total + 8) grad[i] = g;
        float sq = (i < total) ? g * g : 0.f;
        sq = sg_wave_sum(sq);
        if (lane == 0) part[blockIdx.x] = sq;
    }
}
__global__ __launch_bounds__(256) void k_ppo_reduce(const float* slabs, int n_slabs, int slab_stride, int total,
                                                    float* grad, float* part) {
    sg_ppo_reduce_body<false>(slabs, n_slabs, slab_stride, total, grad, part, 0, 0);
}
__global__ __launch_bounds__(256) void k_ppo_reduce_sym(const float* slabs, int n_slabs, int slab_stride, int total,
                                                        float* grad, float* part, int lo2, int hi2) {
    sg_ppo_reduce_body<true>(slabs, n_slabs, slab_stride, total, grad, part, lo2, hi2);
}
__global__ __launch_bounds__(256) void k_a2c_reduce(const float* slabs, int n_slabs, int slab_stride, int total,
                                                    float* grad, float* part, int acc) {
    sg_ppo_reduce_body<false, true>(slabs, n_slabs, slab_stride, total, grad, part, 0, 0, acc);
}

__global__ void k_opt_prepare_first(SgOptState* st) { sg_opt_prepare(st, st->t0 + 1); }

__global__ __launch_bounds__(256) void k_sumsq(const float* grad, int total, float* part) {
    const int i = blockIdx.x * blockDim.x + threadIdx.x;
    float sq = (i < total) ? grad[i] * grad[i] : 0.f;
    sq = sg_wave_sum(sq);
    __shared__ float ws[4];
    if ((threadIdx.x & 63) == 0) ws[threadIdx.x >> 6] = sq;
    __syncthreads();
    if (threadIdx.x == 0) part[blockIdx.x] = ws[0] + ws[1] + ws[2] + ws[3];
}

template <int NL>
__device__ __forceinline__ void sg_ppo_adam_body(float* params, float* m, float* v, const float* grad,
                                                 const float* part, int n_part, int total,
                                                 const SgOptState* st, int k1, float eps, float max_norm,
                                                 float inv_mb, double* loss_acc) {
    __shared__ float s_coef;
    const int t = st->t0 + k1;
    const float s_step_size = st->step_size2[t & 1], s_bc2_sqrt = st->bc2_sqrt2[t & 1];
    __shared__ float s_ws[4];
    {
        float s = 0.f;
        for (int j = threadIdx.x; j < n_part; j += 256) s += part[j];
        s = sg_wave_sum(s);
        if ((threadIdx.x & 63) == 0) s_ws[threadIdx.x >> 6] = s;
    }
    __syncthreads();
    if (threadIdx.x == 0) {
        const float norm = sqrtf((s_ws[0] + s_ws[1]) + (s_ws[2] + s_ws[3]));
        float coef = max_norm / (norm + 1e-6f);
        s_coef = coef > 1.f ? 1.f : coef;
    }
    __syncthreads();
    const int i = blockIdx.x * blockDim.x + threadIdx.x;
    if (i < total) {
        const float g = grad[i] * s_coef;
        float mi = m[i], vi = v[i];
        mi = mi + (g - mi) * (float)(1.0 - 0.9);
        vi = vi * (float)0.999 + (float)(1.0 - 0.999) * g * g;
        const float denom = sqrtf(vi) / s_bc2_sqrt + eps;
        params[i] = params[i] - s_step_size * (mi / denom);
        m[i] = mi;
        v[i] = vi;
    }
    if (blockIdx.x == 0 && threadIdx.x < NL)
        loss_acc[threadIdx.x] += (double)(grad[total + threadIdx.x] * inv_mb);
    if (blockIdx.x == 0 && threadIdx.x == 64) sg_opt_prepare(const_cast<SgOptState*>(st), t + 1);
}
__global__ __launch_bounds__(256) void k_ppo_adam(float* params, float* m, float* v, const float* grad,
                                                  const float* part, int n_part, int total,
                                                  const SgOptState* st, int k1, float eps, float max_norm,
                                                  float inv_mb, double* loss_acc) {
    sg_ppo_adam_body<3>(params, m, v, grad, part, n_part, total, st, k1, eps, max_norm, inv_mb, loss_acc);
}
__global__ __launch_bounds__(256) void k_ppo_adam_sym(float* params, float* m, float* v, const float* grad,
                                                      const float* part, int n_part, int total,
                                                      const SgOptState* st, int k1, float eps, float max_norm,
                                                      float inv_mb, double* loss_acc) {
    sg_ppo_adam_body<4>(params, m, v, grad, part, n_part, total, st, k1, eps, max_norm, inv_mb, loss_acc);
}

__global__ __launch_bounds__(256) void k_a2c_rmsprop(float* params, float* sq, const float* grad, const float* part, int n_part,
                                                     int total, const SgOptState* st, float alpha, float one_m_alpha, float eps,
                                                     float max_norm, float inv_b, double* loss_acc) {
    __shared__ float s_coef;
    __shared__ float s_ws[4];
    {
        float s = 0.f;
        for (int j = threadIdx.x; j < n_part; j += 256) s += part[j];
        s = sg_wave_sum(s);
        if ((threadIdx.x & 63) == 0) s_ws[threadIdx.x >> 6] = s;
    }
    __syncthreads();
    if (threadIdx.x == 0) {
        const float norm = sqrtf((s_ws[0] + s_ws[1]) + (s_ws[2] + s_ws[3]));
        const float coef = max_norm / (norm + 1e-6f);
        s_coef = coef > 1.f ? 1.f : coef;
    }
    __syncthreads();
    const int i = blockIdx.x * blockDim.x + threadIdx.x;
    if (i < total) {
        const float g = grad[i] * s_coef;
        const float s = sq[i] * alpha + one_m_alpha * g * g;
        params[i] = params[i] + (-st->lr) * (g / (sqrtf(s) + eps));
        sq[i] = s;
    }
    if (blockIdx.x == 0 && threadIdx.x < 3) loss_acc[threadIdx.x] += (double)(grad[total + threadIdx.x] * inv_b);
}

__global__ __launch_bounds__(1024) void k_adv_stats(const float* ret, const float* vpred, int64_t n, float* adv,
                                                    double* stats ,
                                                    int pass) {
    __shared__ double ws[16];
    __shared__ double s_mean;
    const int tid = threadIdx.x;
    if (pass == 0) {
        double s = 0.0;
        for (int64_t i = tid; i < n; i += blockDim.x) {
            const float a = ret[i] - vpred[i];
            adv[i] = a;
            s += (double)a;
        }
        s = sg_wave_sum(s);
        if ((tid & 63) == 0) ws[tid >> 6] = s;
        __syncthreads();
        if (tid == 0) {
            double t = 0.0;
            for (int w = 0; w < (int)(blockDim.x >> 6); ++w) t += ws[w];
            stats[0] = t;
            stats[2] = (double)n;
        }
    } else if (pass == 1) {
        if (tid == 0) s_mean = (double)(float)(stats[0] / stats[2]);
        __syncthreads();
        const double mean = s_mean;
        double s = 0.0;
        for (int64_t i = tid; i < n; i += blockDim.x) {
            const double dd = (double)adv[i] - mean;
            s += dd * dd;
        }
        s = sg_wave_sum(s);
        if ((tid & 63) == 0) ws[tid >> 6] = s;
        __syncthreads();
        if (tid == 0) {
            double t = 0.0;
            for (int w = 0; w < (int)(blockDim.x >> 6); ++w) t += ws[w];
            stats[1] = t;
        }
    } else {
        const float mean = (float)(stats[0] / stats[2]);
        const float sd = (float)sqrt(stats[1] / (stats[2] - 1.0));
        for (int64_t i = tid + (int64_t)blockIdx.x * blockDim.x; i < n; i += (int64_t)gridDim.x * blockDim.x)
            adv[i] = (adv[i] - mean) / (sd + 1e-5f);
    }
}
```

### simgan_amd/csrc/sg_test_api.h

```cpp
#pragma once
#include <stdint.h>

#include "../../include/simgan_hip.h"

#ifdef __cplusplus
extern "C" {
#endif
SG_API const char *sg_test_last_error(void);
SG_API int sg_test_gemm(sg_ctx *ctx, int mode, int M, int N, int K, const float *A, const float *B, float *C);
SG_API int sg_test_gemm_bench(sg_ctx *ctx, int mode, int MT, int K, int Np, int threads, int iters, int epi, long long *cycles);
SG_API int sg_test_mfma_probe(sg_ctx *ctx, int abid, const float *a, const float *b, float *d);
SG_API int sg_test_flag_probe(sg_ctx *ctx, int mode, int np, int nc, int words, long long *stamps, float *sums);
SG_API int sg_test_fetch_probe(sg_ctx *ctx, int n_blocks, int waves, int mode, long long *out);
SG_API int sg_test_pstep_probe(sg_ctx *ctx, int mode, int S, int NW, int cyc_phase, int cyc_w, long long *stamps, int *err4);
SG_API int sg_test_pmc_calibrate(sg_ctx *ctx, int64_t mbytes);
SG_API int sg_test_graph_state(sg_ppo *a, sg_disc *d, int out[2]);
SG_API int sg_test_disc_phase_times(sg_disc *d, int enable, long long *out, int n_blocks);
SG_API int sg_test_disc_step4_times(sg_disc *d, int enable, long long *out, int n_blocks);
SG_API int sg_test_ppo_phase_times(sg_ppo *a, int enable, long long *out, int n_blocks);
SG_API int sg_test_disc_gathers(sg_disc *d, long long *out);
SG_API int sg_test_tear_probe(sg_ctx *ctx, int mode, int pairs4, int iters, long long *out4);
SG_API int sg_test_rng(sg_ctx *ctx, int kind, int64_t n, uint64_t seed, void *out);
SG_API int sg_test_raise_handoff_error(sg_disc *d, sg_ppo *a);
SG_API int sg_test_kfac_eig(sg_ctx *ctx, int n, const float *A, float *Q, float *d, int *sweeps);
SG_API int sg_test_acktr_noise(sg_ctx *ctx, int64_t n, uint64_t seed, int64_t update, float *out);
SG_API int sg_test_raise_kfac_error(sg_ppo *a);
#ifdef __cplusplus
}
#endif
```

Measured before the change: 2.496 million env-steps/s.

## Keep PPO policy weights in registers via pre-swizzled MFMA weight images

Adds pre-swizzled weight images in the MFMA fragment layout, including transposed copies for the backward pass. The Adam step writes these images alongside the parameter update, and the fused PPO backward kernel loads them straight into registers instead of staging weights through LDS. This removes the per-block LDS weight staging and the barrier around it, and shrinks the LDS footprint. In exchange the optimizer does extra scattered stores, register pressure rises, and the path only applies to the H64 MLP shapes.

```diff
diff --git a/include/simgan_hip.h b/include/simgan_hip.h
--- a/include/simgan_hip.h
+++ b/include/simgan_hip.h
@@ -99,6 +99,7 @@
 SG_API int sg_results_publish(sg_ctx *ctx, sg_disc *d, sg_ppo *a, int slot);
 SG_API int sg_results_fetch(sg_ctx *ctx, int slot, double out13[13]);
 SG_API int sg_ppo_last_perms(sg_ppo *a, int64_t *perms, int64_t count);
+SG_API int sg_ppo_image_table(int O, int A, int H, int trunk, int image, int64_t *pos, int64_t cap, int64_t dims[4]);
 SG_API int sg_ppo_get_adam(sg_ppo *a, float *m, float *v, int64_t n, int64_t *step);
 SG_API int sg_ppo_set_adam(sg_ppo *a, const float *m, const float *v, int64_t n, int64_t step);
 SG_API int sg_ppo_set_hidden_states(sg_ppo *a, const float *hxs0, int64_t count);
diff --git a/simgan_amd/_lib.py b/simgan_amd/_lib.py
--- a/simgan_amd/_lib.py
+++ b/simgan_amd/_lib.py
@@ -82,6 +82,7 @@
     "sg_ppo_set_lr": (C.c_int, [H, C.c_float]),
     "sg_ppo_update": (C.c_int, [H, H, c_i64_p, C.c_int64, C.c_uint64, c_float_p]),
     "sg_ppo_last_perms": (C.c_int, [H, c_i64_p, C.c_int64]),
+    "sg_ppo_image_table": (C.c_int, [C.c_int, C.c_int, C.c_int, C.c_int, C.c_int, c_i64_p, C.c_int64, c_i64_p]),
     "sg_ppo_set_hidden_states": (C.c_int, [H, c_float_p, C.c_int64]),
     "sg_ppo_get_adam": (C.c_int, [H, c_float_p, c_float_p, C.c_int64, c_i64_p]),
     "sg_ppo_set_adam": (C.c_int, [H, c_float_p, c_float_p, C.c_int64, C.c_int64]),
@@ -145,6 +146,8 @@
     "sg_test_disc_step4_times": (C.c_int, [H, C.c_int, c_ll_p, C.c_int]),
     "sg_test_disc_gathers": (C.c_int, [H, c_ll_p]),
     "sg_test_ppo_phase_times": (C.c_int, [H, C.c_int, c_ll_p, C.c_int]),
+    "sg_test_ppo_wreg": (C.c_int, [H, c_int_p]),
+    "sg_test_ppo_images": (C.c_int, [H, c_float_p, c_float_p, C.c_int64]),
     "sg_test_rng": (C.c_int, [H, C.c_int, C.c_int64, C.c_uint64, C.c_void_p]),
     "sg_test_kfac_eig": (C.c_int, [H, C.c_int, c_float_p, c_float_p, c_float_p, C.POINTER(C.c_int)]),
     "sg_test_acktr_noise": (C.c_int, [H, C.c_int64, C.c_uint64, C.c_int64, c_float_p]),
diff --git a/simgan_amd/csrc/sg_common.h b/simgan_amd/csrc/sg_common.h
--- a/simgan_amd/csrc/sg_common.h
+++ b/simgan_amd/csrc/sg_common.h
@@ -221,6 +221,10 @@
     unsigned* d_pair = nullptr;
     bool self_wait_failed = false;
     bool pair_primed = false;
+    float* d_wimg = nullptr;
+    int32_t* d_wmap = nullptr;
+    int64_t wimg_floats = 0;
+    bool last_wreg = false;
     float sym_coef = 0.f;
     float* d_mobs_mat = nullptr;
     float* d_mact = nullptr;
diff --git a/simgan_amd/csrc/sg_gemm.hpp b/simgan_amd/csrc/sg_gemm.hpp
--- a/simgan_amd/csrc/sg_gemm.hpp
+++ b/simgan_amd/csrc/sg_gemm.hpp
@@ -305,6 +305,65 @@
         sg_acc_zero(acc);
         sg_mma_nn<1, 1>(dY + i * 16 * ldy, ldy, W + tn * 16, ldw, K, acc);
         sg_tile_foreach(acc[0][0], i * 16, tn * 16, ep);
+    }
+}
+
+template <int KC>
+__device__ __forceinline__ void sg_mma_nt_r(const float* A, int lda, const float4 (&w)[KC], f32x4& acc) {
+    const int lane = threadIdx.x & 63, li = lane & 15, lq = lane >> 4;
+    const float* ap = A + li * lda + 2 * lq;
+    f32x4 alt = f32x4{0.f, 0.f, 0.f, 0.f};
+    float2 a[KC][2];
+#pragma unroll
+    for (int c = 0; c < KC; ++c)
+#pragma unroll
+        for (int h = 0; h < 2; ++h) a[c][h] = sg_lds_read_b64(ap + 16 * c + 8 * h);
+#pragma unroll
+    for (int c = 0; c < KC; ++c) {
+        acc = sg_mfma(a[c][0].x, w[c].x, acc);
+        alt = sg_mfma(a[c][0].y, w[c].y, alt);
+        acc = sg_mfma(a[c][1].x, w[c].z, acc);
+        alt = sg_mfma(a[c][1].y, w[c].w, alt);
+    }
+    acc += alt;
+}
+template <int KC>
+__device__ __forceinline__ void sg_mma_nn_r(const float* A, int lda, const float4 (&w)[KC], f32x4& acc) {
+    const int lane = threadIdx.x & 63, li = lane & 15, lq = lane >> 4;
+    const float* ap = A + li * lda + 4 * lq;
+    f32x4 alt = f32x4{0.f, 0.f, 0.f, 0.f};
+    float4 a[KC];
+#pragma unroll
+    for (int c = 0; c < KC; ++c) a[c] = *reinterpret_cast<const float4*>(ap + 16 * c);
+#pragma unroll
+    for (int c = 0; c < KC; ++c) {
+        acc = sg_mfma(a[c].x, w[c].x, acc);
+        alt = sg_mfma(a[c].y, w[c].y, alt);
+        acc = sg_mfma(a[c].z, w[c].z, acc);
+        alt = sg_mfma(a[c].w, w[c].w, alt);
+    }
+    acc += alt;
+}
+template <int MT, int KC, typename EP>
+__device__ __forceinline__ void sg_layer_nt_r(const float* in, int ldi, const float4 (&w)[KC], int Np, EP&& ep) {
+    static_assert(KC >= 1 && KC <= 8, "one K block");
+    const int wave = threadIdx.x >> 6, nw = blockDim.x >> 6, ntl = Np >> 4;
+    for (int u = wave; u < MT * ntl; u += nw) {
+        const int i = u / ntl, tn = u - i * ntl;
+        f32x4 acc = f32x4{0.f, 0.f, 0.f, 0.f};
+        sg_mma_nt_r<KC>(in + i * 16 * ldi, ldi, w, acc);
+        sg_tile_foreach(acc, i * 16, tn * 16, ep);
+    }
+}
+template <int MT, int KC, typename EP>
+__device__ __forceinline__ void sg_layer_nn_r(const float* dY, int ldy, const float4 (&w)[KC], int Np, EP&& ep) {
+    static_assert(KC >= 1 && KC <= 8, "one K block");
+    const int wave = threadIdx.x >> 6, nw = blockDim.x >> 6, ntl = Np >> 4;
+    for (int u = wave; u < MT * ntl; u += nw) {
+        const int i = u / ntl, tn = u - i * ntl;
+        f32x4 acc = f32x4{0.f, 0.f, 0.f, 0.f};
+        sg_mma_nn_r<KC>(dY + i * 16 * ldy, ldy, w, acc);
+        sg_tile_foreach(acc, i * 16, tn * 16, ep);
     }
 }
 
diff --git a/simgan_amd/csrc/sg_layout.cpp b/simgan_amd/csrc/sg_layout.cpp
--- a/simgan_amd/csrc/sg_layout.cpp
+++ b/simgan_amd/csrc/sg_layout.cpp
@@ -3,6 +3,7 @@
 #include <functional>
 
 #include "sg_common.h"
+#include "sg_ppo_images.h"
 
 static SgTrunk make_trunk(int& cursor, int H, int ldO, int P, int EX) {
     SgTrunk t;
@@ -185,3 +186,21 @@
         for (int r = 0; r < rows; ++r) memcpy(flat + fo + (int64_t)r * cols, padded + po + (int64_t)r * ld, sizeof(float) * cols);
     });
 }
+
+void sg_ppo_image_map(const SgPolicyDesc& d, int32_t* map) {
+    for (int64_t i = 0; i < 2 * (int64_t)d.total; ++i) map[i] = -1;
+    for (int t = 0; t < d.n_trunks; ++t) {
+        const SgTrunk& tr = d.trunk[t];
+        const int base = (int)sg_ppo_image_trunk_off(d, t);
+        const int first[3] = {tr.w1, tr.w2, tr.wh}, rows[3] = {tr.Hp, tr.Hp, tr.Pp}, cols[3] = {d.Op, tr.Hp, tr.Hp}, ld[3] = {d.ldO, tr.ldH, tr.ldH};
+        for (int w = 0; w < 3; ++w)
+            for (int r = 0; r < rows[w]; ++r)
+                for (int c = 0; c < cols[w]; ++c) {
+                    int i0, i1;
+                    sg_ppo_img_pos(tr, d.Op, w, r, c, i0, i1);
+                    int32_t* m = map + 2 * (size_t)(tr.off + first[w] + r * ld[w] + c);
+                    m[0] = base + i0;
+                    m[1] = i1 < 0 ? -1 : base + i1;
+                }
+    }
+}
diff --git a/simgan_amd/csrc/sg_ppo.hip b/simgan_amd/csrc/sg_ppo.hip
--- a/simgan_amd/csrc/sg_ppo.hip
+++ b/simgan_amd/csrc/sg_ppo.hip
@@ -8,6 +8,7 @@
 #include "sg_common.h"
 #include "sg_rng.hpp"
 #include "sg_ppo_kernels.hpp"
+#include "sg_ppo_images.h"
 #include "sg_kfac.hpp"
 #include "sg_gru_kernels.hpp"
 
@@ -46,6 +47,17 @@
 static bool ppo_fused(const SgPolicyDesc& d, int MT) {
     const char* e = getenv("SG_PPO_FUSED");
     return d.kind == SG_POLICY_MLP && MT <= 2 && !(e && !strcmp(e, "0"));
+}
+#ifndef SG_PPO_WREG_DEFAULT
+#define SG_PPO_WREG_DEFAULT true
+#endif
+static bool ppo_wreg_shape(const SgPolicyDesc& d) {
+    if (d.kind != SG_POLICY_MLP || d.Hc != d.H || d.Hp != 64 || (d.Op != 48 && d.Op != 112)) return false;
+    for (int t = 0; t < d.n_trunks; ++t) if (d.trunk[t].Pp != 16) return false;
+    return true;
+}
+static bool ppo_wreg_instance(const SgPolicyDesc& d, int MT) {
+    return ppo_wreg_shape(d) && ppo_fused(d, MT) && (MT == 2 || (MT == 1 && d.Op == 48));
 }
 static size_t ppo_bwd_lds(const SgPolicyDesc& d, int MT, bool gw) {
     const int R = 16 * MT;
@@ -105,9 +117,16 @@
     if (MT == 2) SG_LAUNCH(ctx, SG_PROF_PPO_BWD, (k_ppo_pair<2, 0, 0>), grid, block, lds, pa);
     else SG_LAUNCH(ctx, SG_PROF_PPO_BWD, (k_ppo_pair<1, 0, 0>), grid, block, lds, pa);
 }
-static void launch_ppo_bwd(sg_ctx* ctx, int MT, const SgPolicyDesc& d, dim3 grid, size_t lds, const PpoArgs& pa, bool fused, bool gw) {
+static void launch_ppo_bwd(sg_ctx* ctx, int MT, const SgPolicyDesc& d, dim3 grid, size_t lds, const PpoArgs& pa, bool fused, bool gw,
+                           bool wreg = false) {
     const int ko = d.Op / 16, kh = d.Hc == d.H ? d.Hp / 16 : 0;
     const dim3 block(ppo_block_threads(MT));
+    if (wreg) {
+        if (MT == 1 && ko == 3) SG_LAUNCH(ctx, SG_PROF_PPO_BWD, (k_ppo_bwd<1, 3, 4, true, false, false, true>), grid, block, lds, pa);
+        else if (ko == 3) SG_LAUNCH(ctx, SG_PROF_PPO_BWD, (k_ppo_bwd<2, 3, 4, true, false, false, true>), grid, block, lds, pa);
+        else SG_LAUNCH(ctx, SG_PROF_PPO_BWD, (k_ppo_bwd<2, 7, 4, true, false, false, true>), grid, block, lds, pa);
+        return;
+    }
     if (gw) {
         if (fused && MT == 2) SG_LAUNCH(ctx, SG_PROF_PPO_BWD, (k_ppo_bwd<2, 0, 0, true, true>), grid, block, lds, pa);
         else if (fused) SG_LAUNCH(ctx, SG_PROF_PPO_BWD, (k_ppo_bwd<1, 0, 0, true, true>), grid, block, lds, pa);
@@ -318,6 +337,16 @@
     SG_CHECK(hipMemsetAsync(a->d_loss_acc, 0, sizeof(double) * 8, ctx->stream));
     SG_CHECK(sg_dev_malloc((void**)&a->d_pair, SG_PAIR_BYTES));
     SG_CHECK(hipMemsetAsync(a->d_pair, 0, SG_PAIR_BYTES, ctx->stream));
+    if (!p->recurrent && ppo_wreg_shape(p->desc)) {
+        a->wimg_floats = sg_ppo_image_floats(p->desc);
+        std::vector<int32_t> map(2 * (size_t)p->desc.total);
+        sg_ppo_image_map(p->desc, map.data());
+        SG_CHECK(sg_dev_malloc((void**)&a->d_wimg, sizeof(float) * a->wimg_floats));
+        SG_CHECK(sg_dev_malloc((void**)&a->d_wmap, sizeof(int32_t) * map.size()));
+        SG_CHECK(hipMemsetAsync(a->d_wimg, 0, sizeof(float) * a->wimg_floats, ctx->stream));
+        SG_CHECK(hipMemcpyAsync(a->d_wmap, map.data(), sizeof(int32_t) * map.size(), hipMemcpyHostToDevice, ctx->stream));
+        SG_CHECK(hipStreamSynchronize(ctx->stream));
+    }
     SgOptState st;
     memset(&st, 0, sizeof st);
     st.lr = cfg->lr;
@@ -447,11 +476,36 @@
     if (a->d_loss_acc) (void)sg_dev_free(a->d_loss_acc);
     if (a->d_dbg) (void)sg_dev_free(a->d_dbg);
     if (a->d_pair) (void)sg_dev_free(a->d_pair);
+    if (a->d_wimg) (void)sg_dev_free(a->d_wimg);
+    if (a->d_wmap) (void)sg_dev_free(a->d_wmap);
     if (a->h_h0) (void)sg_host_release(a->h_h0);
     for (hipEvent_t ev : a->h0_ev) if (ev) (void)hipEventDestroy(ev);
     if (a->steps_graph) (void)hipGraphExecDestroy(a->steps_graph);
     kfac_free(a);
     delete a;
+    return 0;
+}
+
+extern "C" int sg_ppo_image_table(int O, int A, int H, int trunk, int image, int64_t* pos, int64_t cap, int64_t dims[4]) {
+    SG_REQUIRE(O > 0 && A > 0 && H > 0 && dims, "sg_ppo_image_table: bad argument");
+    const SgPolicyDesc d = sg_make_policy_desc(SG_POLICY_MLP, O, A, H, 0);
+    SG_REQUIRE(trunk >= 0 && trunk < d.n_trunks && image >= 0 && image < SG_PIMG_COUNT, "sg_ppo_image_table: trunk %d / image %d out of range",
+               trunk, image);
+    const SgTrunk& tr = d.trunk[trunk];
+    int N, K;
+    sg_ppo_img_dims(tr, d.Op, image, N, K);
+    const int64_t base = sg_ppo_image_trunk_off(d, trunk);
+    dims[0] = base + sg_ppo_img_off(tr, d.Op, image); dims[1] = (int64_t)N * K; dims[2] = N; dims[3] = K;
+    if (!pos) return 0;
+    SG_REQUIRE(cap >= (int64_t)N * K, "sg_ppo_image_table: pos holds %lld entries, the image has %lld", (long long)cap, (long long)N * K);
+    for (int n = 0; n < N; ++n)
+        for (int k = 0; k < K; ++k) {
+            int i0, i1;
+            const bool transposed = image == SG_PIMG_WHT || image == SG_PIMG_W2T;
+            const int w = image == SG_PIMG_W1 ? 0 : (image == SG_PIMG_W2 || image == SG_PIMG_W2T) ? 1 : 2;
+            sg_ppo_img_pos(tr, d.Op, w, transposed ? k : n, transposed ? n : k, i0, i1);
+            pos[(int64_t)n * K + k] = base + (transposed ? i1 : i0);
+        }
     return 0;
 }
 
@@ -1287,7 +1341,12 @@
                       !a->self_wait_failed && (penv ? strcmp(penv, "0") != 0 : sg_ctx_exclusive(ctx));
     if (pair && !a->pair_primed) SG_CHECK(hipMemsetAsync(a->d_stacks, 0, sizeof(float) * (epoch_f + stack_f), ctx->stream));
     a->pair_primed = pair;
-    const size_t lds_f = ppo_fwd_lds(d, MT, gw), lds_b = sym ? ppo_bwd_sym_lds(d, MT, gw) : ppo_bwd_lds(d, MT, gw);
+    const char* wenv = getenv("SG_PPO_WREG");
+    const bool wreg = fused && !gw && a->d_wimg && ppo_wreg_instance(d, MT) && (wenv ? strcmp(wenv, "0") != 0 : SG_PPO_WREG_DEFAULT);
+    a->last_wreg = wreg;
+    pa.wimg = wreg ? a->d_wimg : nullptr;
+    const size_t lds_f = ppo_fwd_lds(d, MT, gw);
+    const size_t lds_b = sym ? ppo_bwd_sym_lds(d, MT, gw) : ppo_bwd_lds(d, MT, gw) - (wreg ? sizeof(float) * (size_t)wb_f : 0);
     const int nblk = (d.total + 8 + 255) / 256;
     const int nblk_r = (d.total + 8 + SG_PPO_REDUCE_PARAMS - 1) / SG_PPO_REDUCE_PARAMS;
     SgOptState* st = reinterpret_cast<SgOptState*>(a->d_state);
@@ -1323,8 +1382,8 @@
                         pa.wbuf_floats = wb_f;
                         launch_ppo_fwd(ctx, MT, d, dim3(G, d.n_trunks), lds_f, pa, gw);
                     }
-                    pa.wbuf_floats = fused ? wb_f : wb_b;
-                    launch_ppo_bwd(ctx, MT, d, dim3(G, d.n_trunks), lds_b, pa, fused, gw);
+                    pa.wbuf_floats = wreg ? 0 : (fused ? wb_f : wb_b);
+                    launch_ppo_bwd(ctx, MT, d, dim3(G, d.n_trunks), lds_b, pa, fused, gw, wreg);
                 }
                 if (sym) SG_LAUNCH(ctx, SG_PROF_PPO_REDUCE, k_ppo_reduce_sym, dim3(nblk_r), dim3(256), 0, a->d_slabs, G, slab_stride,
                                    d.total, a->d_grad, a->d_part, d.trunk[0].off, d.trunk[0].off + d.trunk[0].ex);
@@ -1334,6 +1393,10 @@
                     SG_TRY(sg_comm_allreduce_f32(ctx, a->d_grad, d.total + 8));
                     hipLaunchKernelGGL(k_sumsq, dim3(nblk), dim3(256), 0, ctx->stream, a->d_grad, d.total, a->d_part);
                 }
+                if (wreg) SG_LAUNCH(ctx, SG_PROF_PPO_ADAM, k_ppo_adam_img, dim3(nblk), dim3(256), 0, a->policy->d_params, a->d_m,
+                                    a->d_v, a->d_grad, a->d_part, ctx->use_comm ? nblk : nblk_r, d.total, st, e * M + k + 1, a->cfg.eps,
+                                    a->cfg.max_grad_norm, pa.inv_B, a->d_loss_acc, reinterpret_cast<const int2*>(a->d_wmap), a->d_wimg);
+                else
                 SG_LAUNCH(ctx, SG_PROF_PPO_ADAM, sym ? k_ppo_adam_sym : k_ppo_adam, dim3(nblk), dim3(256), 0, a->policy->d_params, a->d_m,
                           a->d_v, a->d_grad, a->d_part, ctx->use_comm ? nblk : nblk_r, d.total, st, e * M + k + 1, a->cfg.eps,
                           a->cfg.max_grad_norm, pa.inv_B, a->d_loss_acc);
@@ -1342,6 +1405,11 @@
         hipLaunchKernelGGL(k_opt_commit, dim3(1), dim3(1), 0, ctx->stream, st, E * M);
         return 0;
     };
+    if (wreg) {
+        hipLaunchKernelGGL(k_ppo_build_images, dim3((d.total + 255) / 256), dim3(256), 0, ctx->stream, a->policy->d_params,
+                           reinterpret_cast<const int2*>(a->d_wmap), a->d_wimg, d.total);
+        SG_CHECK(hipGetLastError());
+    }
     const char* genv = getenv("SG_PPO_GRAPH");
     const char* gcenv = getenv("SG_PPO_GRAPH_COMM");
     const bool comm_ok = !a->graph_refused && (!ctx->use_comm || (sg_comm_graph_ok(ctx) && !(gcenv && !strcmp(gcenv, "0"))));
@@ -1358,7 +1426,7 @@
                                   (uint64_t)TN, ((uint64_t)E << 32) | (uint64_t)M, ((uint64_t)MT << 32) | (uint64_t)G,
                                   ((uint64_t)fbits[0] << 32) | fbits[1], ((uint64_t)fbits[2] << 32) | fbits[3],
                                   ((uint64_t)fbits[4] << 32) | fbits[5], (uint64_t)a->cfg.use_clipped_value_loss,
-                                  (uint64_t)(uintptr_t)r->d_field[SG_F_LOGP], 0x50504full + (fused ? 1 : 0) + (ctx->use_comm ? 2 : 0) + (crit_first ? 4 : 0) + (gw ? 8 : 0) + (pair ? 16 : 0) + (sg_comm_peer_on(ctx) ? 32 : 0) + (sym ? 64 : 0) + ((uint64_t)sg_comm_peer_generation(ctx) << 32),
+                                  (uint64_t)(uintptr_t)r->d_field[SG_F_LOGP], 0x50504full + (fused ? 1 : 0) + (ctx->use_comm ? 2 : 0) + (crit_first ? 4 : 0) + (gw ? 8 : 0) + (pair ? 16 : 0) + (sg_comm_peer_on(ctx) ? 32 : 0) + (sym ? 64 : 0) + (wreg ? 128 : 0) + ((uint64_t)sg_comm_peer_generation(ctx) << 32),
                                   sym ? (uint64_t)(uintptr_t)a->d_mrows : 0, sym ? (uint64_t)cbits : 0};
         if (!a->steps_graph || memcmp(key, a->steps_graph_key, sizeof key) != 0) {
             if (a->steps_graph) { SG_CHECK(hipGraphExecDestroy(a->steps_graph)); a->steps_graph = nullptr; }
diff --git a/simgan_amd/csrc/sg_ppo_images.h b/simgan_amd/csrc/sg_ppo_images.h
--- /dev/null
+++ b/simgan_amd/csrc/sg_ppo_images.h
@@ -0,0 +1,43 @@
+#pragma once
+#include "sg_common.h"
+
+enum { SG_PIMG_W1 = 0, SG_PIMG_W2, SG_PIMG_WH, SG_PIMG_WHT, SG_PIMG_W2T, SG_PIMG_COUNT };
+
+__host__ __device__ __forceinline__ int sg16_img_index_nt(int n, int k, int Kp) {
+    const int kk = k & 15, h = kk >> 3, q = (kk & 7) >> 1, s = kk & 1;
+    return ((((n >> 4) * (Kp >> 4) + (k >> 4)) * 64 + 16 * q + (n & 15)) << 2) + 2 * h + s;
+}
+__host__ __device__ __forceinline__ int sg16_img_index_nn(int n, int k, int Kp) {
+    const int kk = k & 15;
+    return ((((n >> 4) * (Kp >> 4) + (k >> 4)) * 64 + 16 * (kk >> 2) + (n & 15)) << 2) + (kk & 3);
+}
+
+__host__ __device__ __forceinline__ void sg_ppo_img_dims(const SgTrunk& tr, int Op, int m, int& N, int& K) {
+    N = m == SG_PIMG_WH ? tr.Pp : tr.Hp;
+    K = m == SG_PIMG_W1 ? Op : (m == SG_PIMG_WHT ? tr.Pp : tr.Hp);
+}
+__host__ __device__ __forceinline__ int sg_ppo_img_off(const SgTrunk& tr, int Op, int m) {
+    int o = 0;
+    for (int j = 0; j < m; ++j) { int N, K; sg_ppo_img_dims(tr, Op, j, N, K); o += N * K; }
+    return o;
+}
+__host__ __device__ __forceinline__ void sg_ppo_img_pos(const SgTrunk& tr, int Op, int w, int row, int col, int& i0, int& i1) {
+    if (w == 0) {
+        i0 = sg_ppo_img_off(tr, Op, SG_PIMG_W1) + sg16_img_index_nt(row, col, Op);
+        i1 = -1;
+    } else if (w == 1) {
+        i0 = sg_ppo_img_off(tr, Op, SG_PIMG_W2) + sg16_img_index_nt(row, col, tr.Hp);
+        i1 = sg_ppo_img_off(tr, Op, SG_PIMG_W2T) + sg16_img_index_nn(col, row, tr.Hp);
+    } else {
+        i0 = sg_ppo_img_off(tr, Op, SG_PIMG_WH) + sg16_img_index_nt(row, col, tr.Hp);
+        i1 = sg_ppo_img_off(tr, Op, SG_PIMG_WHT) + sg16_img_index_nn(col, row, tr.Pp);
+    }
+}
+
+inline int64_t sg_ppo_image_trunk_off(const SgPolicyDesc& d, int t) {
+    int64_t o = 0;
+    for (int j = 0; j < t; ++j) o += sg_ppo_img_off(d.trunk[j], d.Op, SG_PIMG_COUNT);
+    return o;
+}
+inline int64_t sg_ppo_image_floats(const SgPolicyDesc& d) { return sg_ppo_image_trunk_off(d, d.n_trunks); }
+void sg_ppo_image_map(const SgPolicyDesc& d, int32_t* map);
diff --git a/simgan_amd/csrc/sg_ppo_kernels.hpp b/simgan_amd/csrc/sg_ppo_kernels.hpp
--- a/simgan_amd/csrc/sg_ppo_kernels.hpp
+++ b/simgan_amd/csrc/sg_ppo_kernels.hpp
@@ -1,6 +1,7 @@
 #pragma once
 #include "sg_common.h"
 #include "sg_thin.hpp"
+#include "sg_ppo_images.h"
 
 #define HALF_LOG_2PI 0.91893853320467274178f
 
@@ -30,6 +31,7 @@
     const float* MA;
     float sym_c;
     float* DX[2] = {nullptr, nullptr};
+    const float* wimg = nullptr;
 };
 
 #define SG_PAIR_BYTES 64
@@ -185,8 +187,11 @@
     sg_ppo_fwd_body<MT, KO, KH, GW, true>(a, blockIdx.y, blockIdx.x);
 }
 
-template <int MT, int KO, int KH, bool FUSED, bool GW = false, bool PAIR = false, bool SYM = false, bool A2C = false, bool DX = false>
+template <int MT, int KO, int KH, bool FUSED, bool GW = false, bool PAIR = false, bool SYM = false, bool A2C = false, bool DX = false,
+          bool WREG = false>
 __device__ __forceinline__ void sg_ppo_bwd_body(const PpoArgs& a, const int t, const int bx) {
+    static_assert(!WREG || (FUSED && !GW && !PAIR && !SYM && !A2C && !DX && KO > 0 && KO <= 8 && KH == 4),
+                  "register-operand weights: the fused Policy step at compile-time shapes, four hidden column tiles");
     static_assert(!(SYM && (FUSED || PAIR)), "the symmetric step runs the two-launch form");
     static_assert(!DX || ((FUSED || GW) && !PAIR && !SYM && !A2C), "d loss / d X needs w1 at hand: the fused or the global-weight form");
     static_assert(!(A2C && (FUSED || PAIR || SYM)), "the A2C step runs the two-launch form");
@@ -202,7 +207,7 @@
     const int ldO = Op + 4, ldH = Hp + 4, ldP = a.ldP, A = d.A;
     float* Wimg = smem;
     const int w_first = FUSED ? 0 : tr.w2;
-    const float* W = GW ? a.params + tr.off : Wimg - w_first;
+    const float* W = (GW || WREG) ? a.params + tr.off : Wimg - w_first;
     const int wfl = tr.size - w_first;
     float* X = Wimg + a.wbuf_floats;
     float* H1 = X + R * ldO;
@@ -224,7 +229,7 @@
     bool pair_failed = false;
     if (PAIR && !critic) pair_tag = (unsigned)(a.st->t0 + a.k1);
     float4 wv[12];
-    if (!GW) sg_stage_issue<12>(wv, a.params + tr.off + w_first, wfl / 4);
+    if (!GW && !WREG) sg_stage_issue<12>(wv, a.params + tr.off + w_first, wfl / 4);
     constexpr int UX = MT <= 2 ? 4 : 8;
     constexpr int UO = MT <= 2 ? 2 : 4;
     const int ta = critic ? t : (mirror ? 2 : 0);
@@ -259,7 +264,42 @@
             for (int q = 0; q < 4; ++q) scv[q] = a.SC[(size_t)q * a.sc_stride + row0 + r];
         }
     }
-    sg_stage_commit<UX>(X, xv, gX, R * ldO / 4);
+    constexpr int KOr = WREG ? KO : 1, KHr = WREG ? KH : 1;
+    float4 rw1[KOr], rw2[KHr], rwh[KHr], rwhT[1], rw2T[KHr];
+    float rb1 = 0.f, rb2 = 0.f, rbh = 0.f, rls[8] = {0.f, 0.f, 0.f, 0.f, 0.f, 0.f, 0.f, 0.f};
+    const int wtn = (tid >> 6) & 3, wli = tid & 15;
+    constexpr int IMG_W2 = 16 * KH * 16 * KO, IMG_WH = IMG_W2 + 256 * KH * KH, IMG_WHT = IMG_WH + 256 * KH, IMG_W2T = IMG_WHT + 256 * KH,
+                  IMG_TRUNK = IMG_W2T + 256 * KH * KH;
+    const float4* img4 = reinterpret_cast<const float4*>(a.wimg + (size_t)t * IMG_TRUNK) + (tid & 63);
+    if (WREG) {
+        __builtin_amdgcn_sched_barrier(0);
+#pragma unroll
+        for (int c = 0; c < KOr; ++c) rw1[c] = img4[(wtn * KO + c) * 64];
+        rb1 = W[tr.b1 + 16 * wtn + wli];
+        __builtin_amdgcn_sched_barrier(0);
+        __builtin_amdgcn_s_barrier();
+        __builtin_amdgcn_sched_barrier(0);
+#pragma unroll
+        for (int c = 0; c < KHr; ++c) rw2[c] = img4[IMG_W2 / 4 + (wtn * KH + c) * 64];
+        rb2 = W[tr.b2 + 16 * wtn + wli];
+        __builtin_amdgcn_sched_barrier(0);
+#pragma unroll
+        for (int c = 0; c < KHr; ++c) rwh[c] = img4[IMG_WH / 4 + c * 64];
+        rbh = W[tr.bh + wli];
+#pragma unroll
+        for (int j = 0; j < 8; ++j) {
+            const int L = blockDim.x / R, k = tid % L + j * L;
+            if (!critic && j * L < A) rls[j] = W[tr.ex + (k < A ? k : 0)];
+        }
+        __builtin_amdgcn_sched_barrier(0);
+    }
+    if (WREG) {
+#pragma unroll
+        for (int u = 0; u < UX; ++u) {
+            const int i = tid + u * blockDim.x;
+            if (i < R * ldO / 4) reinterpret_cast<float4*>(X)[i] = xv[u];
+        }
+    } else sg_stage_commit<UX>(X, xv, gX, R * ldO / 4);
     if (!FUSED) {
         sg_stage_commit<UX>(H1, h1v, gH1, R * ldH / 4);
         sg_stage_commit<UX>(H2, h2v, gH2, R * ldH / 4);
@@ -273,7 +313,8 @@
     if (!critic && !mirror) {
 #pragma unroll
         for (int u = 0; u < 2; ++u) { const int i = tid + u * 256; if (i < R * A) ACT[i] = actv[u]; }
-        for (int i = tid + 512; i < R * A; i += blockDim.x) ACT[i] = a.ACT[(size_t)row0 * A + i];
+        if (!WREG)
+            for (int i = tid + 512; i < R * A; i += blockDim.x) ACT[i] = a.ACT[(size_t)row0 * A + i];
     }
     if (tid < R) {
         VALID[tid] = row0 + tid < a.mb;
@@ -281,10 +322,25 @@
         for (int q = 0; q < 4; ++q) SC[q * R + tid] = scv[q];
     }
     SG_PPO_STAMP(0);
-    if (!GW) sg_stage_commit<12>(Wimg, wv, a.params + tr.off + w_first, wfl / 4);
-    __syncthreads();
+    if (!GW && !WREG) sg_stage_commit<12>(Wimg, wv, a.params + tr.off + w_first, wfl / 4);
+    if (WREG) SG_LDS_SYNC(); else __syncthreads();
     SG_PPO_STAMP(1);
-    if (FUSED) {
+    if (WREG) {
+        sg_layer_nt_r<MT, KOr>(X, ldO, rw1, Hp, [&](int r, int c, float v) { H1[r * ldH + c] = sg_tanh(v + rb1); });
+        __builtin_amdgcn_sched_barrier(0);
+        rwhT[0] = img4[IMG_WHT / 4 + wtn * 64];
+#pragma unroll
+        for (int c = 0; c < KHr; ++c) rw2T[c] = img4[IMG_W2T / 4 + (wtn * KH + c) * 64];
+        __builtin_amdgcn_sched_barrier(0);
+        SG_LDS_SYNC();
+        SG_PPO_STAMP(2);
+        sg_layer_nt_r<MT, KHr>(H1, ldH, rw2, Hp, [&](int r, int c, float v) { H2[r * ldH + c] = sg_tanh(v + rb2); });
+        SG_LDS_SYNC();
+        SG_PPO_STAMP(3);
+        sg_layer_nt_r<MT, KHr>(H2, ldH, rwh, 16, [&](int r, int c, float v) { O0[r * ldP + c] = v + rbh; });
+        SG_LDS_SYNC();
+        SG_PPO_STAMP(4);
+    } else if (FUSED) {
         const float* b1 = W + tr.b1;
         const float* b2 = W + tr.b2;
         const float* bh = W + tr.bh;
@@ -388,7 +444,7 @@
                 sig[j] = 1.f; dif[j] = 0.f; pmv[j] = nullptr; plv[j] = nullptr;
                 if (k < A) {
                     float mean, ls;
-                    if (mlp) { pmv[j] = o0 + k; plv[j] = o1 + k; mean = *pmv[j]; ls = W[tra.ex + k]; }
+                    if (mlp) { pmv[j] = o0 + k; plv[j] = o1 + k; mean = *pmv[j]; ls = WREG ? rls[j] : W[tra.ex + k]; }
                     else if (k < d.nc) { pmv[j] = o0 + k; plv[j] = o0 + d.nc + k; mean = *pmv[j]; ls = *plv[j]; }
                     else { pmv[j] = o1 + (k - d.nc); plv[j] = o1 + (d.na + k - d.nc); mean = *pmv[j]; ls = *plv[j]; }
                     sig[j] = __expf(ls);
@@ -521,7 +577,8 @@
     SG_PPO_STAMP(11);
     {
         auto dz_u = [&](float* h) { return [=](int r, int c, float v) { float* ph = h + r * ldH + c; const float hv = *ph; *ph = v * (1.f - hv * hv); }; };
-        sg_layer_nn_u<MT>(dout, ldP, W + tr.wh, ldH, tr.Pp, Hp, dz_u(H2));
+        if (WREG) sg_layer_nn_r<MT, 1>(dout, ldP, rwhT, Hp, dz_u(H2));
+        else sg_layer_nn_u<MT>(dout, ldP, W + tr.wh, ldH, tr.Pp, Hp, dz_u(H2));
         SG_LDS_SYNC();
         SG_PPO_STAMP(12);
         sg_grad_tn<MT, (MT >= 2 ? 8 : 0), true>(H2, ldH, H1, ldH, Hp, Hp, g + tr.w2, ldH, false);
@@ -529,7 +586,8 @@
         sg_colsum(H2, ldH, R, Hp, g + tr.b2, false);
         SG_LDS_SYNC();
         SG_PPO_STAMP(13);
-        sg_layer_nn_u<MT>(H2, ldH, W + tr.w2, ldH, Hp, Hp, dz_u(H1));
+        if (WREG) sg_layer_nn_r<MT, KHr>(H2, ldH, rw2T, Hp, dz_u(H1));
+        else sg_layer_nn_u<MT>(H2, ldH, W + tr.w2, ldH, Hp, Hp, dz_u(H1));
         SG_LDS_SYNC();
         SG_PPO_STAMP(14);
         sg_grad_tn<MT, (MT >= 2 ? 8 : 0), true>(H1, ldH, X, ldO, Hp, Op, g + tr.w1, ldO, false);
@@ -548,9 +606,9 @@
     }
 }
 
-template <int MT, int KO, int KH, bool FUSED = false, bool GW = false, bool DX = false>
+template <int MT, int KO, int KH, bool FUSED = false, bool GW = false, bool DX = false, bool WREG = false>
 __global__ __launch_bounds__(512) void k_ppo_bwd(PpoArgs a) {
-    sg_ppo_bwd_body<MT, KO, KH, FUSED, GW, false, false, false, DX>(a, blockIdx.y, blockIdx.x);
+    sg_ppo_bwd_body<MT, KO, KH, FUSED, GW, false, false, false, DX, WREG>(a, blockIdx.y, blockIdx.x);
 }
 template <int MT, int KO, int KH, bool GW = false>
 __global__ __launch_bounds__(512) void k_ppo_bwd_sym(PpoArgs a) {
@@ -631,11 +689,11 @@
     if (threadIdx.x == 0) part[blockIdx.x] = ws[0] + ws[1] + ws[2] + ws[3];
 }
 
-template <int NL>
+template <int NL, bool IMG = false>
 __device__ __forceinline__ void sg_ppo_adam_body(float* params, float* m, float* v, const float* grad,
                                                  const float* part, int n_part, int total,
                                                  const SgOptState* st, int k1, float eps, float max_norm,
-                                                 float inv_mb, double* loss_acc) {
+                                                 float inv_mb, double* loss_acc, const int2* map = nullptr, float* img = nullptr) {
     __shared__ float s_coef;
     const int t = st->t0 + k1;
     const float s_step_size = st->step_size2[t & 1], s_bc2_sqrt = st->bc2_sqrt2[t & 1];
@@ -660,9 +718,15 @@
         mi = mi + (g - mi) * (float)(1.0 - 0.9);
         vi = vi * (float)0.999 + (float)(1.0 - 0.999) * g * g;
         const float denom = sqrtf(vi) / s_bc2_sqrt + eps;
-        params[i] = params[i] - s_step_size * (mi / denom);
+        const float p = params[i] - s_step_size * (mi / denom);
+        params[i] = p;
         m[i] = mi;
         v[i] = vi;
+        if (IMG) {
+            const int2 mp = map[i];
+            if (mp.x >= 0) __builtin_nontemporal_store(p, img + mp.x);
+            if (mp.y >= 0) __builtin_nontemporal_store(p, img + mp.y);
+        }
     }
     if (blockIdx.x == 0 && threadIdx.x < NL)
         loss_acc[threadIdx.x] += (double)(grad[total + threadIdx.x] * inv_mb);
@@ -673,6 +737,20 @@
                                                   const SgOptState* st, int k1, float eps, float max_norm,
                                                   float inv_mb, double* loss_acc) {
     sg_ppo_adam_body<3>(params, m, v, grad, part, n_part, total, st, k1, eps, max_norm, inv_mb, loss_acc);
+}
+__global__ __launch_bounds__(256) void k_ppo_adam_img(float* params, float* m, float* v, const float* grad,
+                                                      const float* part, int n_part, int total,
+                                                      const SgOptState* st, int k1, float eps, float max_norm,
+                                                      float inv_mb, double* loss_acc, const int2* map, float* img) {
+    sg_ppo_adam_body<3, true>(params, m, v, grad, part, n_part, total, st, k1, eps, max_norm, inv_mb, loss_acc, map, img);
+}
+__global__ __launch_bounds__(256) void k_ppo_build_images(const float* params, const int2* map, float* img, int total) {
+    const int i = blockIdx.x * blockDim.x + threadIdx.x;
+    if (i >= total) return;
+    const int2 mp = map[i];
+    const float p = params[i];
+    if (mp.x >= 0) img[mp.x] = p;
+    if (mp.y >= 0) img[mp.y] = p;
 }
 __global__ __launch_bounds__(256) void k_ppo_adam_sym(float* params, float* m, float* v, const float* grad,
                                                       const float* part, int n_part, int total,
diff --git a/simgan_amd/csrc/sg_test_api.h b/simgan_amd/csrc/sg_test_api.h
--- a/simgan_amd/csrc/sg_test_api.h
+++ b/simgan_amd/csrc/sg_test_api.h
@@ -18,6 +18,8 @@
 SG_API int sg_test_disc_phase_times(sg_disc *d, int enable, long long *out, int n_blocks);
 SG_API int sg_test_disc_step4_times(sg_disc *d, int enable, long long *out, int n_blocks);
 SG_API int sg_test_ppo_phase_times(sg_ppo *a, int enable, long long *out, int n_blocks);
+SG_API int sg_test_ppo_wreg(sg_ppo *a, int out[2]);
+SG_API int sg_test_ppo_images(sg_ppo *a, float *dev_img, float *host_img, int64_t n);
 SG_API int sg_test_disc_gathers(sg_disc *d, long long *out);
 SG_API int sg_test_tear_probe(sg_ctx *ctx, int mode, int pairs4, int iters, long long *out4);
 SG_API int sg_test_rng(sg_ctx *ctx, int kind, int64_t n, uint64_t seed, void *out);
```

New measurement: 2.518 million env-steps/s, median of 3. No clear change (+0.9%).
